# syun88/VLA-from-FastVLM

Measured on AMD Instinct MI355X. Metric: policy steps/sec (img+prompt->action) FastVLM-0.5B bs=64, higher is better.
Workload: dtype bf16; 1 GPU; fastvlm-0.5b select_action: letterbox 336^2->1024^2, FastViT-HD, projector, Qwen2 decoder (text-only, reference-literal: 64-token prompt), last-token pool, action head; batch_per_gpu=64, global_batch=64, seq_len=64, image=336, parallelism=replicas x1 (no collective on the inference path), tower_microbatch=0, stream_overlap=True, llm_precision=split-bf16 (hi+lo) operands, fp32 attention

## Files before the change

### include/fastvla_hip_testops.h

```cpp
#ifndef FASTVLA_HIP_TESTOPS_H
#define FASTVLA_HIP_TESTOPS_H

#include "fastvla_hip.h"

#ifdef __cplusplus
extern "C" {
#endif

enum fv_gemm_epilogue {
  FV_EPI_BIAS = 0,
  FV_EPI_BIAS_GELU = 1,
  FV_EPI_LS_RES = 2,
  FV_EPI_RES_F32 = 3,
  FV_EPI_SWIGLU = 4,
  FV_EPI_F32 = 5,
  FV_EPI_SWIGLU_SPLIT = 7,
  FV_EPI_SWIGLU_F16 = 8,
  FV_EPI_GELU_GRAD = 9,
  FV_EPI_MUL_AUX = 10,
  FV_EPI_F16 = 11,
  FV_EPI_MUL_GELUP = 12
};
int fv_op_gemm(const void* A, int lda, const void* W, int M, int N, int K, const float* bias, const float* scale,
               const void* res, int ldr, void* out, int ldo, int epilogue, fv_stream s);
int fv_op_gemm_f16(const void* A, int lda, const void* W, int M, int N, int K, const float* bias, const void* res, int ldr, void* out,
                   int ldo, int epilogue, void* ws, size_t ws_bytes, fv_stream s);
int fv_op_gemm_lo8(const void* A, int lda, const void* W, const void* W8, int M, int N, int K, const float* bias, const void* res, int ldr, void* out,
                   int ldo, int epilogue, void* ws, size_t ws_bytes, fv_stream s);
int fv_op_lo8_pack(const float* x, void* a_out, int lda, const void* W, void* w8_out, int M, int K, int N, fv_stream s);
int fv_op_gemm_ksplit(const void* A, int lda, const void* W, int M, int N, int K, const float* bias, const void* res, int ldr,
                      void* out, int ldo, int epilogue, fv_stream s);
int fv_op_gemm_tn(const void* A, int lda, const void* W, int ldw, int M, int N, int K, int f16, const float* bias, void* out, int ldo, void* ws,
                  size_t ws_bytes, fv_stream s);
int fv_op_gemm_splitk(const void* A, int lda, const void* W, int M, int N, int K, const float* bias, const void* res, int ldr,
                      void* out, int ldo, int epilogue, int ksplit, void* ws, size_t ws_bytes, fv_stream s);
int fv_op_dwconv(const void* x, const float* w, const float* bias, void* y, int B, int H, int W, int C, int k,
                 int stride, int mult, int gelu, fv_stream s);
int fv_op_stem_conv(const void* pix, const float* w, const float* bias, void* y, int B, int S, int Cout, fv_stream s);
int fv_op_stem_mfma(const void* pix, const void* wp, const float* bias, void* y, int B, int S, int Cout, fv_stream s);
int fv_op_stem_fused(const void* pix, const void* wp, const float* b1, const float* w2, const float* b2, void* y, int B,
                     int S, int Cout, fv_stream s);
int fv_op_stem_fused_images(const void* img, int dtype, int B, int C, int Hin, int Win, float pad_value, int resize_with_padding, const void* wp,
                            const float* b1, const float* w2, const float* b2, void* y, int S, int Cout, fv_stream s);
int fv_op_layernorm_rows(const void* x, const float* w, const float* b, void* y, int rows, int C, float eps,
                         fv_stream s);
int fv_op_attention(const void* q, const void* k, const void* v, int ldq, int ldk, int ldv, void* out, int ldo, int B,
                    int T, int heads, int kv_heads, int D, int causal, const int32_t* lens, float scale, fv_stream s);
int fv_op_rmsnorm(const float* x, const float* w, void* y_bf16, int rows, int H, float eps, fv_stream s);
int fv_op_rope(void* qkv, int ld, int rows, int T, int heads, int kv_heads, int D, float theta, fv_stream s);
int fv_op_attention_bwd(const float* qkv, int ld, const float* dO, float* dqkv, void* out_bf16_scratch, float* stat_scratch, int B, int T,
                        int heads, int kv_heads, int D, const int32_t* lens, float theta, fv_stream s);
int fv_op_rmsnorm_bwd(const float* x, const float* w, const float* dy, const float* dres, float* dx, float* dw, float* scratch, int rows,
                      int H, float eps, fv_stream s);

int fv_op_se_gelu(const void* x, const float* w1, const float* b1, const float* w2, const float* b2, void* y,
                  float* scratch, int B, int P, int C, int R, fv_stream s);

int fv_op_dwconv_mfma(const void* x, const void* ttab, const float* bias, void* y, int B, int H, int W, int C, int k, int gelu,
                      fv_stream s);
int fv_op_dwconv_s2_mfma(const void* x, const void* ttab, const float* bias, void* y, int B, int H, int W, int C, int gelu,
                         fv_stream s);
int fv_op_dwconv_pair(const void* x, const void* t3, const float* b3, const void* t7, const float* b7, void* y1, void* y2, int B,
                      int H, int W, int C, fv_stream s);
int fv_op_convffn(const void* x, const void* w1, const float* b1, const void* w2p, const float* b2, const float* ls,
                  const void* res, void* out, int M, int C, fv_stream s);

int fv_op_convffn32(const void* x, const void* wq, const float* b1, const float* b2, const float* ls, const void* res, void* out,
                    int M, int C, fv_stream s);
int fv_op_convffn32_stash(const void* x, const void* wq, const float* b1, const float* b2, const float* ls, const void* res, void* out,
                          int M, int C, void* stash_y, fv_stream s);
int fv_op_gemm_f16_gelup(const void* A, int lda, const void* W, int M, int N, int K, const void* aux, int ldaux, void* out, int ldo, void* h_out, fv_stream s);
int fv_op_dw_wgrad(const void* x, const void* dy, float* dw, float* db, float* scratch, size_t scratch_floats, int B, int H, int W, int C, int k, int stride, int mult, fv_stream s);
int fv_op_convffn32_split(const void* x, const void* wq, const float* b1, const float* b2, const float* ls, const void* res, void* out,
                          int M, int C, float* part, size_t part_bytes, fv_stream s);

int fv_op_lora_direct_scratch_floats(int R, int rank, int max_cols, size_t* out_floats);
int fv_op_lora_direct(int kind, int part_mask, int rank, int Np, int K, int qd, int kd, const int64_t* a_off, const int64_t* b_off, const void* dY, const void* X,
                      int xkind, int ldx, int lo_off, int R, const float* lora, float* lora_grads, float scale, float* scratch, size_t scratch_floats, fv_stream s);

#ifdef __cplusplus
}
#endif
#endif
```

### vla-from-fastvlm_amd/csrc/engine.hip

```cpp
#include <dlfcn.h>

#include <algorithm>
#include <cmath>
#include <cstdarg>
#include <cstdio>
#include <cstdlib>
#include <cstring>
#include <functional>
#include <map>
#include <string>
#include <vector>

#include "kernels.h"

static thread_local char g_err[768] = "";
static thread_local char* g_err_handle = nullptr;
int fv_fail(int code, const char* fmt, ...) {
  va_list ap;
  va_start(ap, fmt);
  vsnprintf(g_err, sizeof(g_err), fmt, ap);
  va_end(ap);
  if (g_err_handle) memcpy(g_err_handle, g_err, sizeof(g_err));
  return code;
}
// ... 202 lines not shown
    const fv_tensor_desc* t = need(name);
    if (t && count(t) != n) {
      if (rc == FV_OK) rc = fv_fail(FV_ERR_ARG, "tensor '%s' has %zu elements, expected %zu", name.c_str(), count(t), n);
      return nullptr;
    }
    return t;
  }
  bool to_f32(const fv_tensor_desc* t, std::vector<float>& out) {
    const size_t n = count(t), esz = t->dtype == FV_F32 ? 4 : 2;
    const void* src = t->data;
    if (t->device) {
      stage.resize(n * esz);
      if (hipMemcpy(stage.data(), t->data, n * esz, hipMemcpyDeviceToHost) != hipSuccess) {
        if (rc == FV_OK) rc = fv_fail(FV_ERR_HIP, "hipMemcpy (device tensor -> host) failed");
        return false;
      }
      src = stage.data();
    }
    out.resize(n);
    if (t->dtype == FV_F32) memcpy(out.data(), src, n * 4);
    else { const bf16_t* b = static_cast<const bf16_t*>(src); for (size_t i = 0; i < n; ++i) out[i] = host_bf2f(b[i]); }
    return true;
  }
  bool get(const std::string& name, std::vector<float>& out, std::vector<int64_t>* shape = nullptr) {
    const fv_tensor_desc* t = need(name);
    if (!t || !to_f32(t, out)) return false;
    if (shape) shape->assign(t->shape, t->shape + t->ndim);
    return true;
  }
  bool expect(const std::string& name, std::vector<float>& v, size_t n) {
    const fv_tensor_desc* t = need_n(name, n);
    return t && to_f32(t, v);
  }
  void* alloc(size_t bytes) {
    void* p = nullptr;
    if (dev_alloc(h, bytes, &p) != FV_OK) { if (rc == FV_OK) rc = FV_ERR_HIP; return nullptr; }
    return p;
  }
  float* up_f32(const std::vector<float>& v) {
    void* p = alloc(v.size() * 4);
    if (p && hipMemcpy(p, v.data(), v.size() * 4, hipMemcpyHostToDevice) != hipSuccess) { if (rc == FV_OK) rc = fv_fail(FV_ERR_HIP, "hipMemcpy failed"); }
    return static_cast<float*>(p);
  }
  bf16_t* up_bf16(const std::vector<float>& v) {
    std::vector<bf16_t> b(v.size());
    for (size_t i = 0; i < v.size(); ++i) b[i] = host_f2bf(v[i]);
    void* p = alloc(b.size() * 2);
    if (p && hipMemcpy(p, b.data(), b.size() * 2, hipMemcpyHostToDevice) != hipSuccess) { if (rc == FV_OK) rc = fv_fail(FV_ERR_HIP, "hipMemcpy failed"); }
    return static_cast<bf16_t*>(p);
  }
  bool put_rows(const fv_tensor_desc* t, bf16_t* dst, size_t dst_pitch, size_t row_elems, size_t rows, size_t src_pitch) {
    std::vector<bf16_t> tmp;
    const void* src = t->data;
    hipMemcpyKind kind = t->device ? hipMemcpyDeviceToDevice : hipMemcpyHostToDevice;
    if (t->dtype == FV_F32) {
      std::vector<float> v;
      if (!to_f32(t, v)) return false;
      tmp.resize(v.size());
      for (size_t i = 0; i < v.size(); ++i) tmp[i] = host_f2bf(v[i]);
      src = tmp.data();
      kind = hipMemcpyHostToDevice;
    }
    if (hipMemcpy2D(dst, dst_pitch * 2, src, src_pitch * 2, row_elems * 2, rows, kind) != hipSuccess) {
      if (rc == FV_OK) rc = fv_fail(FV_ERR_HIP, "hipMemcpy2D (weight packing) failed");
      return false;
    }
    return true;
  }
  float* vec(const std::string& name, size_t n) { std::vector<float> v; return expect(name, v, n) ? up_f32(v) : nullptr; }
  bf16_t* mat(const std::string& name, size_t n, size_t k) {
    const fv_tensor_desc* t = need_n(name, n * k);
    if (!t) return nullptr;
    bf16_t* p = static_cast<bf16_t*>(alloc(n * k * 2));
    return p && put_rows(t, p, n * k, n * k, 1, n * k) ? p : nullptr;
  }
  float* dw(const std::string& name, int cout, int k, const std::vector<float>* scale = nullptr, int map_w = 0, bf16_t** ttab = nullptr,
            int s2_cin = 0, int s2_map = 0, bf16_t** s2_ttab = nullptr) {
    std::vector<float> v;
    if (!expect(name, v, (size_t)cout * k * k)) return nullptr;
    std::vector<float> o((size_t)cout * k * k);
    for (int c = 0; c < cout; ++c)
      for (int t = 0; t < k * k; ++t) o[(size_t)t * cout + c] = v[(size_t)c * k * k + t] * (scale ? (*scale)[c] : 1.0f);
    if (ttab && fv::dwconv_mfma_supported(map_w, cout, k, 1, 1)) {
      std::vector<float> tt(fv::dwconv_toeplitz_elems(cout, k));
      fv::dwconv_toeplitz_pack(o.data(), tt.data(), cout, k);
      *ttab = up_bf16(tt);
    }
    if (s2_ttab && s2_cin > 0 && cout % s2_cin == 0 && fv::dwconv_s2_mfma_supported(s2_map, s2_map, s2_cin, k, 2, cout / s2_cin)) {
      std::vector<float> tt(fv::dwconv_s2_toeplitz_elems(s2_cin));
      fv::dwconv_s2_toeplitz_pack(o.data(), tt.data(), s2_cin);
      *s2_ttab = up_bf16(tt);
    }
    return up_f32(o);
  }
};

int load_ffn(Loader& L, const std::string& pre, int C, int hidden, float bn_eps, FFN& f, const std::string& ls_name, int map_w) {
  std::vector<float> g, b, m, v;
  if (!L.expect(pre + "conv.bn.weight", g, C) || !L.expect(pre + "conv.bn.bias", b, C) ||
      !L.expect(pre + "conv.bn.running_mean", m, C) || !L.expect(pre + "conv.bn.running_var", v, C))
    return L.rc;
  std::vector<float> sc(C), bias(C);
  for (int c = 0; c < C; ++c) {
    sc[c] = g[c] / std::sqrt(v[c] + bn_eps);
    bias[c] = b[c] - m[c] * sc[c];
  }
  f.dw_w = L.dw(pre + "conv.conv.weight", C, 7, &sc, map_w, &f.dw_t);
  f.dw_b = L.up_f32(bias);
  f.fc1_w = L.mat(pre + "fc1.weight", hidden, C);
  f.fc1_b = L.vec(pre + "fc1.bias", hidden);
  f.fc2_w = L.mat(pre + "fc2.weight", C, hidden);
  if (hidden == 4 * C && fv::convffn_supported(C, 4)) {
    std::vector<float> w2, w2p;
    if (L.expect(pre + "fc2.weight", w2, (size_t)C * hidden)) {
      w2p.resize(w2.size());
      fv::convffn_pack_w2(w2.data(), w2p.data(), C, hidden);
      f.w2p = L.up_bf16(w2p);
      std::vector<float> w1;
      if (fv::convffn32_supported(C, 4) && L.expect(pre + "fc1.weight", w1, (size_t)hidden * C)) {
        std::vector<float> wq((size_t)2 * hidden * C);
        fv::convffn32_pack(w1.data(), w2.data(), wq.data(), C);
        f.w2q = L.up_bf16(wq);
      }
    }
  }
  f.fc2_b = L.vec(pre + "fc2.bias", C);
  f.ls = L.vec(ls_name, C);
  return L.rc;
}

WsPlan plan_ws(const fv_handle* h, int B, int T, int splice) {
  const fv_model_desc& d = h->d;
  WsPlan p{};
  const int mb = (d.tower_microbatch > 0 && d.tower_microbatch < B) ? d.tower_microbatch : B;
  const size_t S = d.image_size;
  size_t act = (S / 2) * (S / 2) * (size_t)d.tower_dims[0];
  size_t hid = 0;
  size_t hw = (S / 4) * (S / 4);
  for (int i = 0; i < d.tower_stages; ++i) {
    const size_t C = d.tower_dims[i];
    act = std::max(act, hw * C);
    hid = std::max(hid, hw * C * d.tower_mlp_ratio);
    if (d.tower_is_attn[i]) hid = std::max(hid, hw * C * 3);
    if (i + 1 < d.tower_stages) {
      hw /= 4;
      act = std::max(act, hw * (size_t)d.tower_dims[i + 1]);
    }
  }
  const size_t P = hw;
  act = std::max(act, P * (size_t)d.tower_out_dim);
  hid = std::max(hid, P * (size_t)d.llm_hidden);
  size_t o = 0;
  auto take = [&](size_t bytes) { size_t r = o; o += align_up(bytes); return r; };
  p.bufA = take(act * mb * 2);
  p.bufB = take(act * mb * 2);
  p.bufH = take(hid * mb * 2);
  p.se = take(((size_t)mb * (2 * d.tower_out_dim + d.tower_se_rd)) * 4);
  p.tower_out = take((size_t)B * P * d.tower_out_dim * 2);
  const size_t rows = (size_t)B * (T + (splice ? P : 0));
  const size_t qkvw = (size_t)(d.llm_heads + 2 * d.llm_kv_heads) * d.llm_head_dim;
  p.x = take(rows * d.llm_hidden * 4);
  p.xn = take(rows * d.llm_hidden * 2);
  p.qkv = take(rows * qkvw * 2);
  p.att = take(rows * (size_t)d.llm_heads * d.llm_head_dim * 2);
  p.act = take(rows * d.llm_inter * 2);
  if (d.llm_precision >= 1) {
    p.xn_lo = take(rows * d.llm_hidden * 2 * 2);
    p.att_lo = take(rows * (size_t)d.llm_heads * d.llm_head_dim * 2 * 2);
    p.act_lo = (d.llm_precision == 1 || d.llm_precision == 3 || d.llm_precision == 5) ? take(rows * d.llm_inter * 2 * 2) : 0;
    p.qkvf = take(rows * qkvw * 4);
    p.guf = 0;
  }
  p.splitk_bytes = rows <= 256 || (rows % 256 != 0 && rows <= 1024) ? (size_t)(rows <= 256 ? 40 : 24) * rows * ((std::max((size_t)d.llm_hidden, qkvw) + 255) / 256 * 256) * 4
                               : rows % 256 == 0 ? (size_t)(rows <= 2048 ? 8 : 4) * rows * ((std::max((size_t)d.llm_hidden, qkvw) + 255) / 256 * 256) * 4 : 0;
  p.splitk = take(p.splitk_bytes);
  p.head_scr = take(fv::head_bwd_scratch_bytes(h->hd, B));
  const int Tseq = T + (splice ? (int)P : 0);
  p.attn_scr_bytes = (d.llm_precision != 0 && Tseq >= fv::FV_ATTN_SPLIT_MIN_T && (d.llm_head_dim == 64 || d.llm_head_dim == 128))
                         ? fv::attention_split_scratch_bytes(B, Tseq, d.llm_kv_heads, d.llm_head_dim) : 0;
  p.attn_scr = take(p.attn_scr_bytes);
  p.total = o;
  return p;
}

int check_ready(fv_handle* h, bool need_ws) {
  if (!h) return fv_fail(FV_ERR_ARG, "null handle");
  if (!h->loaded) return fv_fail(FV_ERR_STATE, "weights not loaded: call fv_load_weights first");
  if (need_ws && !h->ws) return fv_fail(FV_ERR_STATE, "workspace not bound: call fv_bind_workspace first");
  return FV_OK;
}

#define FV_TRY(expr)            \
  do {                          \
    int _rc = (expr);           \
    if (_rc != FV_OK) return _rc; \
  } while (0)

void prof_begin(fv_handle* h, int fam, double flops, double bytes, hipStream_t s, int m = 0, int n = 0, int k = 0, int epi = 0) {
  if (!h->prof.on) return;
  ProfRec r{fam, flops, bytes, m, n, k, epi, h->prof.get(), h->prof.get()};
  if (!r.e0 || !r.e1) return;
  (void)hipEventRecord(r.e0, s);
  h->prof.recs.push_back(r);
}
void prof_end(fv_handle* h, hipStream_t s) {
  if (!h->prof.on || h->prof.recs.empty()) return;
  (void)hipEventRecord(h->prof.recs.back().e1, s);
}
#define FV_P(fam, flops, bytes, call)            \
  do {                                           \
    prof_begin(h, fam, flops, bytes, s);         \
    int _rc = (call);                            \
    prof_end(h, s);                              \
    if (_rc != FV_OK) return _rc;                \
  } while (0)

int gemm_p(fv_handle* h, const fv::GemmArgs& g_in, hipStream_t s) {
  fv::GemmArgs g = g_in;
  if (h->train_depth > 0) g.few_rows = 0;
  const double M = g.M, N = g.N, K = g.K;
  const bool f32o = g.epi == FV_EPI_RES_F32 || g.epi == FV_EPI_F32;
  double bytes = (M * K + N * K) * 2 + M * ((g.epi == FV_EPI_SWIGLU || g.epi == FV_EPI_SWIGLU_F16) ? N / 2 : N) * (f32o ? 4 : 2);
  if (g.epi == FV_EPI_LS_RES) bytes += M * N * 2;
  if (g.epi == FV_EPI_RES_F32) bytes += M * N * 4;
  prof_begin(h, FV_FAM_GEMM, 2.0 * M * N * K, bytes + (g.ksplit ? M * K * 2 : 0), s, g.M, g.N, g.ksplit ? -g.K : g.K, g.epi);
  const int rc = fv::launch_gemm(g, s);
  prof_end(h, s);
  return rc;
}
double dw_flops(int B, int Ho, int Wo, int Cout, int k) { return 2.0 * B * Ho * Wo * Cout * k * k; }

int dw_s1(fv_handle* h, const bf16_t* x, const float* w, const bf16_t* ttab, const float* bias, bf16_t* y, int mb, int H, int C,
          int k, hipStream_t s) {
  if (ttab && !h->no_mfma_dw) return fv::launch_dwconv_mfma(x, ttab, bias, y, mb, H, H, C, k, 0, s);
  return fv::launch_dwconv(x, w, bias, y, mb, H, H, C, k, 1, 1, 0, s);
}

bool ffn_stash_ok(const fv_handle* h, const FFN& f, int M, int C) { return f.w2q && !h->no_ffn32 && fv::convffn32_stash_supported(M, C); }
int fused_ffn(fv_handle* h, const FFN& f, const bf16_t* t, const bf16_t* res, bf16_t* out, int M, int C, int hidden, hipStream_t s, bool ranges = true,
              bf16_t* stash_y = nullptr) {
  if (stash_y) return fv::launch_convffn32(t, f.w2q, f.fc1_b, f.fc2_b, f.ls, res, out, M, C, hidden, s, nullptr, 0, stash_y);
  if (f.w2q && !h->no_ffn32 && (size_t)M * C * 2 < ((size_t)1 << 31))
    return fv::launch_convffn32(t, f.w2q, f.fc1_b, f.fc2_b, f.ls, res, out, M, C, hidden, s, ranges && !h->batch_invariant ? h->ffn_part : nullptr,
                                ranges && !h->batch_invariant && h->ffn_part ? FFN_PART_BYTES : 0);
  return fv::launch_convffn(t, f.fc1_w, f.fc1_b, f.w2p, f.fc2_b, f.ls, res, out, M, C, hidden, s);
}

int run_ffn(fv_handle* h, const FFN& f, bf16_t* x_dw_in, bf16_t* dw_out, bf16_t* hid, bf16_t* res_out, int mb, int H, int W, int C,
            int ratio, hipStream_t s) {
  const int M = mb * H * W;
  FV_P(FV_FAM_DWCONV, dw_flops(mb, H, W, C, 7), 4.0 * M * C, dw_s1(h, x_dw_in, f.dw_w, f.dw_t, f.dw_b, dw_out, mb, H, C, 7, s));
  if (f.w2p && !h->no_fused_ffn) {
    prof_begin(h, FV_FAM_GEMM, 4.0 * M * C * (double)(C * ratio), 6.0 * M * C, s, M, C, C * ratio, 6);
    const int rc = fused_ffn(h, f, dw_out, res_out, res_out, M, C, C * ratio, s);
    prof_end(h, s);
    return rc;
  }
  fv::GemmArgs g1{dw_out, C, f.fc1_w, M, C * ratio, C, f.fc1_b, nullptr, nullptr, 0, hid, C * ratio, FV_EPI_BIAS_GELU};
  FV_TRY(gemm_p(h, g1, s));
  fv::GemmArgs g2{hid, C * ratio, f.fc2_w, M, C, C * ratio, f.fc2_b, f.ls, res_out, C, res_out, C, FV_EPI_LS_RES};
  if (!h->batch_invariant) { g2.splitk_ws = h->ffn_part; g2.splitk_bytes = h->ffn_part ? FFN_PART_BYTES : 0; }
  FV_TRY(gemm_p(h, g2, s));
  return FV_OK;
}

int tap_copy(fv_handle* h, int t, const bf16_t* src, int b0, int mb, size_t per_image, hipStream_t s) {
  if (!h->taps || t >= h->n_taps || !h->taps[t]) return FV_OK;
  bf16_t* dst = static_cast<bf16_t*>(h->taps[t]) + (size_t)b0 * per_image;
  FV_HIP_CHECK(hipMemcpyAsync(dst, src, (size_t)mb * per_image * 2, hipMemcpyDeviceToDevice, s));
  return FV_OK;
}

int unit_tap(fv_handle* h, int u, const bf16_t* src, int b0, int mb, size_t per_image, hipStream_t s) {
  if (!h->utaps || u >= h->n_utaps || !h->utaps[u]) return FV_OK;
  bf16_t* dst = static_cast<bf16_t*>(h->utaps[u]) + (size_t)b0 * per_image;
  FV_HIP_CHECK(hipMemcpyAsync(dst, src, (size_t)mb * per_image * 2, hipMemcpyDeviceToDevice, s));
  return FV_OK;
}

struct UnitInfo { int kind, stage, side, channels; };
std::vector<UnitInfo> tower_units(const fv_model_desc& d) {
  std::vector<UnitInfo> u;
  int H = d.image_size / 4;
  u.push_back({0, 0, H, d.tower_dims[0]});
  for (int i = 0; i < d.tower_stages; ++i) {
    if (d.tower_is_attn[i]) u.push_back({1, i, H, d.tower_dims[i]});
    for (int j = 0; j < d.tower_layers[i]; ++j) u.push_back({2, i, H, d.tower_dims[i]});
    if (i + 1 < d.tower_stages) { H /= 2; u.push_back({3, i, H, d.tower_dims[i + 1]}); }
  }
  return u;
}

int tower_pass(fv_handle* h, const bf16_t* pix, int b0, int mb, bf16_t* tower_out, float* img_tokens, const WsPlan& wp,
               hipStream_t s) {
  const fv_model_desc& d = h->d;
  const Tower& tw = h->tw;
  char* ws = static_cast<char*>(h->ws);
  bf16_t* cur = reinterpret_cast<bf16_t*>(ws + wp.bufA);
  bf16_t* oth = reinterpret_cast<bf16_t*>(ws + wp.bufB);
  bf16_t* hid = reinterpret_cast<bf16_t*>(ws + wp.bufH);
  float* se = reinterpret_cast<float*>(ws + wp.se);
  const int S = d.image_size, C0 = d.tower_dims[0];
  static const bool fuse_stem = !fv_ab_env("FASTVLA_NO_FUSED_STEM");
  if (h->lbsrc) {
    const fv_handle::LbSrc& L = *h->lbsrc;
    if (!(tw.stem0_wp && fv::stem_fused_supported(S, C0))) return fv_fail(FV_ERR_UNSUPPORTED, "fv_vision_forward_images needs the fused stem (first stage width 96)");
    const size_t per = (size_t)L.C * L.Hin * L.Win * (L.dtype == FV_U8 ? 1 : 4);
    FV_P(FV_FAM_STEM, 2.0 * mb * (S / 2) * (S / 2) * 27 * C0 + dw_flops(mb, S / 4, S / 4, C0, 3) + 30.0 * mb * S * S,
         (double)mb * per + (double)mb * (S / 4) * (S / 4) * C0 * 2,
         fv::launch_stem_fused_lb(static_cast<const char*>(L.img) + (size_t)b0 * per, L.dtype, mb, L.C, L.Hin, L.Win, L.pad, L.letterbox, tw.stem0_wp,
                                  tw.stem0_b, tw.stem1_w, tw.stem1_b, oth, S, C0, s));
  } else if (fuse_stem && tw.stem0_wp && fv::stem_fused_supported(S, C0)) {
    FV_P(FV_FAM_STEM, 2.0 * mb * (S / 2) * (S / 2) * 27 * C0 + dw_flops(mb, S / 4, S / 4, C0, 3),
         (double)mb * S * S * 8 + (double)mb * (S / 4) * (S / 4) * C0 * 2,
         fv::launch_stem_fused(pix, tw.stem0_wp, tw.stem0_b, tw.stem1_w, tw.stem1_b, oth, mb, S, C0, s));
  } else {
    FV_P(FV_FAM_STEM, 2.0 * mb * (S / 2) * (S / 2) * 27 * C0, (double)mb * S * S * 8 + (double)mb * (S / 2) * (S / 2) * C0 * 2,
         tw.stem0_wp ? fv::launch_stem_mfma(pix, tw.stem0_wp, tw.stem0_b, cur, mb, S, C0, s)
                     : fv::launch_stem_conv(pix, tw.stem0_w, tw.stem0_b, cur, mb, S, C0, s));
    FV_P(FV_FAM_DWCONV, dw_flops(mb, S / 4, S / 4, C0, 3), (double)mb * (S / 2) * (S / 2) * C0 * 2 * 1.25,
         fv::launch_dwconv(cur, tw.stem1_w, tw.stem1_b, oth, mb, S / 2, S / 2, C0, 3, 2, 1, 1, s));
  }
  int H = S / 4;
  {
    fv::GemmArgs g{oth, C0, tw.stem2_w, mb * H * H, C0, C0, tw.stem2_b, nullptr, nullptr, 0, cur, C0, FV_EPI_BIAS_GELU};
    FV_TRY(gemm_p(h, g, s));
  }
  FV_TRY(tap_copy(h, 0, cur, b0, mb, (size_t)H * H * C0, s));
  int unit = 0;
  FV_TRY(unit_tap(h, unit++, cur, b0, mb, (size_t)H * H * C0, s));
  for (int i = 0; i < d.tower_stages; ++i) {
    const int C = d.tower_dims[i];
    const int M = mb * H * H;
    if (d.tower_is_attn[i]) {
      FV_P(FV_FAM_DWCONV, dw_flops(mb, H, H, C, 7), 4.0 * M * C, dw_s1(h, cur, tw.cpes[i].w, tw.cpes[i].t, tw.cpes[i].b, oth, mb, H, C, 7, s));
      std::swap(cur, oth);
      FV_TRY(unit_tap(h, unit++, cur, b0, mb, (size_t)H * H * C, s));
    }
    for (const Block& b : tw.stages[i]) {
      if (!d.tower_is_attn[i]) {
        static const bool pair_ok = !fv_ab_env("FASTVLA_NO_DW_PAIR");
        if (pair_ok && !h->no_mfma_dw && !h->no_fused_ffn && b.mix_t && b.ffn.dw_t && b.ffn.w2p && fv::dwconv_pair_supported(mb, H, H, C)) {
          FV_P(FV_FAM_DWCONV, dw_flops(mb, H, H, C, 3) + dw_flops(mb, H, H, C, 7), 6.0 * M * C,
               fv::launch_dwconv_pair(cur, b.mix_t, b.mix_b, b.ffn.dw_t, b.ffn.dw_b, oth, hid, mb, H, H, C, s));
          prof_begin(h, FV_FAM_GEMM, 4.0 * M * C * (double)(C * d.tower_mlp_ratio), 6.0 * M * C, s, M, C, C * d.tower_mlp_ratio, 6);
          const int rc = fused_ffn(h, b.ffn, hid, oth, oth, M, C, C * d.tower_mlp_ratio, s);
          prof_end(h, s);
          if (rc != FV_OK) return rc;
        } else {
          FV_P(FV_FAM_DWCONV, dw_flops(mb, H, H, C, 3), 4.0 * M * C, dw_s1(h, cur, b.mix_w, b.mix_t, b.mix_b, oth, mb, H, C, 3, s));
          FV_TRY(run_ffn(h, b.ffn, oth, cur, hid, oth, mb, H, H, C, d.tower_mlp_ratio, s));
        }
        std::swap(cur, oth);
      } else {
        FV_P(FV_FAM_NORM, 8.0 * M * C, 4.0 * M * C, fv::launch_layernorm_rows(cur, b.ln_w, b.ln_b, oth, M, C, d.ln_eps, s));
        fv::GemmArgs gq{oth, C, b.qkv_w, M, 3 * C, C, nullptr, nullptr, nullptr, 0, hid, 3 * C, FV_EPI_BIAS};
        FV_TRY(gemm_p(h, gq, s));
        const int nh = C / d.tower_head_dim;
        FV_P(FV_FAM_ATTN, 4.0 * mb * (double)(H * H) * (H * H) * C, 8.0 * M * C,
             fv::launch_attention(hid, hid + C, hid + 2 * C, 3 * C, 3 * C, 3 * C, oth, C, mb, H * H, nh, nh,
                                  d.tower_head_dim, 0, nullptr, 0, 1.0f / std::sqrt((float)d.tower_head_dim), s));
        fv::GemmArgs gp{oth, C, b.proj_w, M, C, C, b.proj_b, b.ls1, cur, C, cur, C, FV_EPI_LS_RES};
        FV_TRY(gemm_p(h, gp, s));
        FV_TRY(run_ffn(h, b.ffn, cur, oth, hid, cur, mb, H, H, C, d.tower_mlp_ratio, s));
      }
      FV_TRY(unit_tap(h, unit++, cur, b0, mb, (size_t)H * H * C, s));
    }
    FV_TRY(tap_copy(h, 1 + i, cur, b0, mb, (size_t)H * H * C, s));
    if (i + 1 < d.tower_stages) {
      const int C2 = d.tower_dims[i + 1];
      FV_P(FV_FAM_DWCONV, dw_flops(mb, H / 2, H / 2, C2, 7), 2.0 * M * C + 2.0 * (M / 4) * C2,
           (tw.downs[i].lk_t && !h->no_mfma_dw)
               ? fv::launch_dwconv_s2_mfma(cur, tw.downs[i].lk_t, tw.downs[i].lk_b, oth, mb, H, H, C, 1, s)
               : fv::launch_dwconv(cur, tw.downs[i].lk_w, tw.downs[i].lk_b, oth, mb, H, H, C, 7, 2, C2 / C, 1, s));
      H /= 2;
      fv::GemmArgs g{oth, C2, tw.downs[i].pw_w, mb * H * H, C2, C2, tw.downs[i].pw_b, nullptr, nullptr, 0, cur, C2, FV_EPI_BIAS_GELU};
      FV_TRY(gemm_p(h, g, s));
      FV_TRY(unit_tap(h, unit++, cur, b0, mb, (size_t)H * H * C2, s));
    }
  }
  const int CL = d.tower_dims[d.tower_stages - 1], CO = d.tower_out_dim, P = H * H;
  FV_P(FV_FAM_DWCONV, dw_flops(mb, H, H, CO, 3), 2.0 * mb * P * (CL + CO), fv::launch_dwconv(cur, tw.exp_w, tw.exp_b, oth, mb, H, H, CL, 3, 1, CO / CL, 0, s));
  FV_P(FV_FAM_ELT, 20.0 * mb * P * CO, 6.0 * mb * P * CO, fv::launch_se_gelu(oth, tw.se_w1, tw.se_b1, tw.se_w2, tw.se_b2, tower_out, se, mb, P, CO, d.tower_se_rd, s));
  fv::GemmArgs p0{tower_out, CO, tw.pj0_w, mb * P, d.llm_hidden, CO, tw.pj0_b, nullptr, nullptr, 0, hid, d.llm_hidden, FV_EPI_BIAS_GELU};
  if (!h->batch_invariant) { p0.splitk_ws = h->ffn_part; p0.splitk_bytes = h->ffn_part ? FFN_PART_BYTES : 0; }
  FV_TRY(gemm_p(h, p0, s));
  fv::GemmArgs p2{hid, d.llm_hidden, tw.pj2_w, mb * P, d.llm_hidden, d.llm_hidden, tw.pj2_b, nullptr, nullptr, 0, img_tokens, d.llm_hidden, FV_EPI_F32};
  FV_TRY(gemm_p(h, p2, s));
  return FV_OK;
}


enum DecMode { DEC_FULL = 0, DEC_PREFIX = 1, DEC_SUFFIX = 2 };
int decoder_layers_split(fv_handle* h, const WsPlan& wp, int B, int Tq, const int32_t* lens, int len_add, float* kv, int Np, int mode,
                         hipStream_t s) {
  const fv_model_desc& d = h->d;
  char* ws = static_cast<char*>(h->ws);
  float* x = reinterpret_cast<float*>(ws + wp.x);
  bf16_t* xn = reinterpret_cast<bf16_t*>(ws + wp.xn);
  bf16_t* act = reinterpret_cast<bf16_t*>(ws + wp.act);
  const int rows = B * Tq, Hd = d.llm_hidden, D = d.llm_head_dim;
  const int qd = d.llm_heads * D, kd = d.llm_kv_heads * D, qkvw = qd + 2 * kd;
  const int Tt = mode == DEC_SUFFIX ? Np + Tq : Tq;
  const float att_scale = 1.0f / std::sqrt((float)D);
  {
    bf16_t* xs = reinterpret_cast<bf16_t*>(ws + wp.xn_lo);
    bf16_t* as = reinterpret_cast<bf16_t*>(ws + wp.att_lo);
    bf16_t* cs = reinterpret_cast<bf16_t*>(ws + wp.act_lo);
    float* qkvf = reinterpret_cast<float*>(ws + wp.qkvf);
    const int I = d.llm_inter, I2 = 2 * I;
    const size_t kv_layer = (size_t)B * Np * 2 * kd;
    for (size_t li = 0; li < h->dec.layers.size(); ++li) {
      const DecLayer& L = h->dec.layers[li];
      const int lo8 = d.llm_precision == 5, KS = lo8 ? 2 : 1;
      if (li == 0) FV_P(FV_FAM_NORM, 4.0 * rows * Hd, 8.0 * rows * Hd, fv::launch_rmsnorm(x, L.ln1, xs, xs + Hd, 2 * Hd, rows, Hd, d.rms_eps, s, 0, nullptr, lo8));
      fv::GemmArgs q1{xs, 2 * Hd, L.qkv_w, rows, qkvw, Hd, L.qkv_b, nullptr, nullptr, 0, qkvf, qkvw, FV_EPI_F32, KS};
      q1.W8 = L.qkv_w8;
      q1.splitk_ws = wp.splitk_bytes ? reinterpret_cast<float*>(ws + wp.splitk) : nullptr;
      q1.splitk_bytes = wp.splitk_bytes;
      FV_TRY(gemm_p(h, q1, s));
      if (mode == DEC_PREFIX) {
        FV_HIP_CHECK(hipMemcpy2DAsync(kv + li * kv_layer, (size_t)2 * kd * 4, qkvf + qd, (size_t)qkvw * 4, (size_t)2 * kd * 4, (size_t)rows,
                                      hipMemcpyDeviceToDevice, s));
        if (li + 1 == h->dec.layers.size()) break;
      }
      FV_P(FV_FAM_ATTN, 2.0 * B * (double)Tq * Tt * qd + 3.0 * rows * (qd + kd), 4.0 * rows * (qkvw + qd),
           fv::launch_attention_f32(qkvf, qkvw, as, as + qd, 2 * qd, B, Tt, d.llm_heads, d.llm_kv_heads, D, lens, len_add, att_scale, s, h->rope,
                                    mode == DEC_SUFFIX ? kv + li * kv_layer : nullptr, 2 * kd, mode == DEC_SUFFIX ? Np : 0, nullptr, lo8,
                                    wp.attn_scr_bytes && mode != DEC_SUFFIX ? ws + wp.attn_scr : nullptr));
      fv::GemmArgs o1{as, 2 * qd, L.o_w, rows, Hd, qd, nullptr, nullptr, x, Hd, x, Hd, FV_EPI_RES_F32, KS};
      o1.W8 = L.o_w8;
      o1.splitk_ws = q1.splitk_ws;
      o1.splitk_bytes = wp.splitk_bytes;
      const bool ln2_fused = d.llm_precision == 1 || d.llm_precision == 5;
      if (ln2_fused) { o1.norm_w = L.ln2; o1.norm_y = xs; o1.norm_ylo = xs + Hd; o1.norm_ld = 2 * Hd; o1.norm_eps = d.rms_eps; }
      FV_TRY(gemm_p(h, o1, s));
      fv::GemmArgs d1{cs, I2, L.down_w, rows, Hd, I, nullptr, nullptr, x, Hd, x, Hd, FV_EPI_RES_F32, KS};
      d1.W8 = L.down_w8;
      if (d.llm_precision == 2) {
        FV_P(FV_FAM_NORM, 4.0 * rows * Hd, 6.0 * rows * Hd, fv::launch_rmsnorm(x, L.ln2, xn, nullptr, Hd, rows, Hd, d.rms_eps, s, 1, h->f16_flags));
        fv::GemmArgs g1{xn, Hd, L.gu_w, rows, I2, Hd, nullptr, nullptr, nullptr, 0, act, I, FV_EPI_SWIGLU_F16, 0};
        g1.f16 = 1; g1.sat = h->f16_flags;
        FV_TRY(gemm_p(h, g1, s));
        d1 = fv::GemmArgs{act, I, L.down_w, rows, Hd, I, nullptr, nullptr, x, Hd, x, Hd, FV_EPI_RES_F32, 0};
        d1.f16 = 1;
      } else if (d.llm_precision == 3) {
        FV_P(FV_FAM_NORM, 4.0 * rows * Hd, 6.0 * rows * Hd, fv::launch_rmsnorm(x, L.ln2, xn, nullptr, Hd, rows, Hd, d.rms_eps, s, 1, h->f16_flags));
        fv::GemmArgs g1{xn, Hd, L.gu_w, rows, I2, Hd, nullptr, nullptr, nullptr, 0, cs, I2, FV_EPI_SWIGLU_SPLIT, 0};
        g1.f16 = 1;
        FV_TRY(gemm_p(h, g1, s));
      } else if (d.llm_precision == 4) {
        FV_P(FV_FAM_NORM, 4.0 * rows * Hd, 8.0 * rows * Hd, fv::launch_rmsnorm(x, L.ln2, xs, xs + Hd, 2 * Hd, rows, Hd, d.rms_eps, s));
        fv::GemmArgs g1{xs, 2 * Hd, L.gu_w, rows, I2, Hd, nullptr, nullptr, nullptr, 0, act, I, FV_EPI_SWIGLU_F16, 1};
        g1.sat = h->f16_flags;
        FV_TRY(gemm_p(h, g1, s));
        d1 = fv::GemmArgs{act, I, L.down_w, rows, Hd, I, nullptr, nullptr, x, Hd, x, Hd, FV_EPI_RES_F32, 0};
        d1.f16 = 1;
      } else {
        fv::GemmArgs g1{xs, 2 * Hd, L.gu_w, rows, I2, Hd, nullptr, nullptr, nullptr, 0, cs, I2, FV_EPI_SWIGLU_SPLIT, KS};
        g1.W8 = L.gu_w8;
        g1.splitk_ws = q1.splitk_ws; g1.splitk_bytes = wp.splitk_bytes;
        FV_TRY(gemm_p(h, g1, s));
      }
      d1.splitk_ws = wp.splitk_bytes ? reinterpret_cast<float*>(ws + wp.splitk) : nullptr;
      d1.splitk_bytes = wp.splitk_bytes;
      if (li + 1 < h->dec.layers.size()) {
        d1.norm_w = h->dec.layers[li + 1].ln1; d1.norm_y = xs; d1.norm_ylo = xs + Hd; d1.norm_ld = 2 * Hd; d1.norm_eps = d.rms_eps;
      }
      FV_TRY(gemm_p(h, d1, s));
    }
  }
  return FV_OK;
}

}

extern "C" {

const char* fv_version(void) { return "fastvla_hip 0.1 (gfx950)"; }
const char* fv_last_error(fv_handle* h) { return h ? h->err : g_err; }

int fv_create(const fv_model_desc* desc, int device, fv_handle** out) {
  if (!desc || !out) return fv_fail(FV_ERR_ARG, "fv_create: null argument");
  const fv_model_desc& d = *desc;
  if (d.tower_stages < 1 || d.tower_stages > FV_MAX_STAGES) return fv_fail(FV_ERR_ARG, "tower_stages out of range");
  if (d.image_size <= 0 || d.image_size % (4 << (d.tower_stages - 1)))
    return fv_fail(FV_ERR_ARG, "image_size %d must be a positive multiple of %d", d.image_size, 4 << (d.tower_stages - 1));
  for (int i = 0; i < d.tower_stages; ++i) {
    if (d.tower_dims[i] % 8 || d.tower_dims[i] <= 0 || d.tower_layers[i] < 0) return fv_fail(FV_ERR_ARG, "tower dims must be positive multiples of 8");
    if (d.tower_is_attn[i] && d.tower_dims[i] % d.tower_head_dim) return fv_fail(FV_ERR_ARG, "attention stage dim %% head_dim != 0");
    if (i > 0 && d.tower_dims[i] != 2 * d.tower_dims[i - 1] && d.tower_dims[i] != d.tower_dims[i - 1]) return fv_fail(FV_ERR_UNSUPPORTED, "stage dims must double or stay (grouped 7x7 multiplier 1 or 2)");
  }
  if (d.tower_head_dim != 32 && d.tower_head_dim != 64 && d.tower_head_dim != 128) return fv_fail(FV_ERR_UNSUPPORTED, "tower head_dim must be 32/64/128");
  if (d.llm_head_dim != 32 && d.llm_head_dim != 64 && d.llm_head_dim != 128) return fv_fail(FV_ERR_UNSUPPORTED, "llm head_dim must be 32/64/128");
  if (d.llm_hidden % 8 || d.llm_inter % 8 || d.llm_heads % d.llm_kv_heads) return fv_fail(FV_ERR_ARG, "llm dims must be multiples of 8 and heads %% kv_heads == 0");
  if (d.tower_out_dim != 2 * d.tower_dims[d.tower_stages - 1] && d.tower_out_dim != d.tower_dims[d.tower_stages - 1]) return fv_fail(FV_ERR_UNSUPPORTED, "tower_out_dim must be 1x or 2x the last stage dim");
  if (d.llm_precision < 0 || d.llm_precision > 5)
    return fv_fail(FV_ERR_ARG, "llm_precision must be 0 (bf16), 1 (split-bf16), 2 (split-bf16 qkv/o + fp16 gate/up/down) or 5 (bf16 hi + fp8 lo)");
#ifndef FASTVLA_AB_SWITCHES
  if (d.llm_precision == 3 || d.llm_precision == 4)
    return fv_fail(FV_ERR_UNSUPPORTED, "llm_precision = %d is a measurement mode of the tools build (make AB=1); the product ships 0, 1, 2 and 5", d.llm_precision);
#endif
  if (d.llm_precision == 5 && (d.llm_hidden % 128 || d.llm_inter % 128 || (d.llm_heads * d.llm_head_dim) % 128))
    return fv_fail(FV_ERR_UNSUPPORTED, "llm_precision = 5 (hi + lo8 operands) needs hidden, inter and heads * head_dim to be multiples of 128");
  if (d.state_dim <= 0 || d.action_dim <= 0 || d.hidden_dim <= 0 || d.fusion_dim <= 0) return fv_fail(FV_ERR_ARG, "head dims must be positive");
  FV_HIP_CHECK(hipSetDevice(device));
  fv_handle* h = new fv_handle();
  h->d = d;
  h->device = device;
  h->hd = fv::HeadDims{d.llm_hidden, d.state_dim, d.action_dim, d.hidden_dim, d.fusion_dim};
  if (const char* e = fv_ab_env("FASTVLA_NO_FUSED_FFN")) h->no_fused_ffn = e[0] == '1';
  if (const char* e = fv_ab_env("FASTVLA_NO_MFMA_DW")) h->no_mfma_dw = e[0] == '1';
  if (const char* e = fv_ab_env("FASTVLA_NO_FFN32")) h->no_ffn32 = e[0] == '1';
  const int P = (d.image_size >> (d.tower_stages + 1)) * (d.image_size >> (d.tower_stages + 1));
  h->rope_rows = d.max_text_tokens + P + 8;
  std::vector<float> cs((size_t)h->rope_rows * d.llm_head_dim);
  fv::rope_table_host(cs.data(), h->rope_rows, d.llm_head_dim, d.rope_theta);
  void* p = nullptr;
  int rc = dev_alloc(h, cs.size() * 4, &p);
  if (rc == FV_OK && hipMemcpy(p, cs.data(), cs.size() * 4, hipMemcpyHostToDevice) != hipSuccess) rc = fv_fail(FV_ERR_HIP, "rope table upload failed");
  h->rope = static_cast<float2*>(p);
  if (rc == FV_OK) { rc = dev_alloc(h, fv::adamw_scratch_bytes(), &p); h->norm_scratch = static_cast<float*>(p); }
  if (rc == FV_OK) {
    rc = dev_alloc(h, 256, &p);
    h->f16_flags = static_cast<unsigned*>(p);
    if (rc == FV_OK && hipMemset(p, 0, 256) != hipSuccess) rc = fv_fail(FV_ERR_HIP, "fp16 flag words: memset failed");
    h->lb_vmax = h->f16_flags + 32;
  }
  if (rc == FV_OK) { rc = dev_alloc(h, FFN_PART_BYTES, &p); h->ffn_part = static_cast<float*>(p); }
  if (rc != FV_OK) { fv_destroy(h); return rc; }
  *out = h;
  return FV_OK;
}

void fv_destroy(fv_handle* h) {
  if (!h) return;
  (void)hipSetDevice(h->device);
  for (void* p : h->allocs) (void)hipFree(p);
  for (hipEvent_t e : h->prof.pool) (void)hipEventDestroy(e);
  delete h;
}

static int load_impl(fv_handle* h, Loader& L);

int fv_load_weights(fv_handle* h, const fv_tensor_desc* tensors, int n) {
  HandleScope _hs(h);
  if (!h || !tensors || n <= 0) return fv_fail(FV_ERR_ARG, "fv_load_weights: null argument");
  if (h->loaded) return fv_fail(FV_ERR_STATE, "weights already loaded");
  Loader L{h};
  for (int i = 0; i < n; ++i) {
    if (!tensors[i].name || !tensors[i].data || tensors[i].ndim < 1 || tensors[i].ndim > 4) return fv_fail(FV_ERR_ARG, "tensor %d: bad descriptor", i);
    L.idx[tensors[i].name] = &tensors[i];
  }
  return load_impl(h, L);
}

int fv_load_weights_cb(fv_handle* h, fv_tensor_provider provider, void* user) {
  HandleScope _hs(h);
  if (!h || !provider) return fv_fail(FV_ERR_ARG, "fv_load_weights_cb: null argument");
  if (h->loaded) return fv_fail(FV_ERR_STATE, "weights already loaded");
  Loader L{h};
  L.prov = provider;
  L.user = user;
  return load_impl(h, L);
}

static int load_impl(fv_handle* h, Loader& L) {
  FV_HIP_CHECK(hipSetDevice(h->device));
  const fv_model_desc& d = h->d;
  Tower& tw = h->tw;
  const std::string vt = VT;
  const int C0 = d.tower_dims[0];
  {
    std::vector<float> v;
    if (L.expect(vt + "patch_embed.0.reparam_conv.weight", v, (size_t)C0 * 27)) {
      std::vector<float> o((size_t)27 * C0);
      for (int co = 0; co < C0; ++co)
        for (int ci = 0; ci < 3; ++ci)
          for (int t = 0; t < 9; ++t) o[(size_t)(t * 3 + ci) * C0 + co] = v[((size_t)co * 3 + ci) * 9 + t];
      tw.stem0_w = L.up_f32(o);
      if (C0 % 16 == 0 && C0 <= 128) {
        std::vector<float> wp((size_t)C0 * 64);
        fv::stem_mfma_pack(o.data(), wp.data(), C0);
        tw.stem0_wp = L.up_bf16(wp);
      }
    }
    tw.stem0_b = L.vec(vt + "patch_embed.0.reparam_conv.bias", C0);
    tw.stem1_w = L.dw(vt + "patch_embed.1.reparam_conv.weight", C0, 3);
    tw.stem1_b = L.vec(vt + "patch_embed.1.reparam_conv.bias", C0);
    tw.stem2_w = L.mat(vt + "patch_embed.2.reparam_conv.weight", C0, C0);
    tw.stem2_b = L.vec(vt + "patch_embed.2.reparam_conv.bias", C0);
  }
  tw.stages.resize(d.tower_stages);
  tw.downs.resize(d.tower_stages);
  tw.cpes.resize(d.tower_stages);
  int idx = 0;
  for (int i = 0; i < d.tower_stages && L.rc == FV_OK; ++i) {
    const int C = d.tower_dims[i];
    const int map_w = d.image_size >> (2 + i);
    if (d.tower_is_attn[i]) {
      const std::string pre = vt + "network." + std::to_string(idx++) + ".";
      tw.cpes[i].w = L.dw(pre + "reparam_conv.weight", C, 7, nullptr, map_w, &tw.cpes[i].t);
      tw.cpes[i].b = L.vec(pre + "reparam_conv.bias", C);
    }
    const int sidx = idx++;
    tw.stages[i].resize(d.tower_layers[i]);
    for (int j = 0; j < d.tower_layers[i] && L.rc == FV_OK; ++j) {
      const std::string pre = vt + "network." + std::to_string(sidx) + "." + std::to_string(j) + ".";
      Block& b = tw.stages[i][j];
      if (d.tower_is_attn[i]) {
        b.ln_w = L.vec(pre + "norm.weight", C);
        b.ln_b = L.vec(pre + "norm.bias", C);
        b.qkv_w = L.mat(pre + "token_mixer.qkv.weight", 3 * (size_t)C, C);
        b.proj_w = L.mat(pre + "token_mixer.proj.weight", C, C);
        b.proj_b = L.vec(pre + "token_mixer.proj.bias", C);
        b.ls1 = L.vec(pre + "layer_scale_1", C);
        load_ffn(L, pre + "convffn.", C, C * d.tower_mlp_ratio, d.bn_eps, b.ffn, pre + "layer_scale_2", map_w);
      } else {
        b.mix_w = L.dw(pre + "token_mixer.reparam_conv.weight", C, 3, nullptr, map_w, &b.mix_t);
        b.mix_b = L.vec(pre + "token_mixer.reparam_conv.bias", C);
        load_ffn(L, pre + "convffn.", C, C * d.tower_mlp_ratio, d.bn_eps, b.ffn, pre + "layer_scale", map_w);
      }
    }
    if (i + 1 < d.tower_stages) {
      const int C2 = d.tower_dims[i + 1];
      const std::string pre = vt + "network." + std::to_string(idx++) + ".proj.";
      tw.downs[i].lk_w = L.dw(pre + "0.lkb_reparam.weight", C2, 7, nullptr, 0, nullptr, C, map_w, &tw.downs[i].lk_t);
// ... 525 lines not shown
```

### vla-from-fastvlm_amd/csrc/kernels.h

```cpp
#pragma once
#include <hip/hip_runtime.h>
#include <stdint.h>

#include "../../include/fastvla_hip.h"
#include "../../include/fastvla_hip_testops.h"
#include "common.h"

namespace fv {

struct GemmArgs {
  const bf16_t* A; int lda;
  const bf16_t* W;
  int M, N, K;
  const float* bias;
  const float* scale;
  const void* res; int ldr;
  void* out; int ldo;
  int epi;
  int ksplit = 0;
  int f16 = 0;
  float* splitk_ws = nullptr;
  size_t splitk_bytes = 0;
  int lo_off = 0;
  int no_tail = 0;
  int few_rows = 1;
  const float* norm_w = nullptr; bf16_t* norm_y = nullptr; bf16_t* norm_ylo = nullptr; int norm_ld = 0; float norm_eps = 0.f;
  const void* W8 = nullptr;
  unsigned* sat = nullptr;
  void* stash = nullptr;
  int stash_f16 = 0;
  int tn = 0, ldw = 0;
};
int launch_gemm(const GemmArgs& a, hipStream_t s);

bool convffn_supported(int C, int ratio);
void convffn_pack_w2(const float* w2, float* out, int C, int hidden);
int launch_convffn(const bf16_t* x, const bf16_t* w1, const float* b1, const bf16_t* w2p, const float* b2, const float* ls,
                   const bf16_t* res, bf16_t* out, int M, int C, int hidden, hipStream_t s);

bool convffn32_supported(int C, int ratio);
void convffn32_pack(const float* w1, const float* w2, float* out, int C);
int launch_convffn32(const bf16_t* x, const bf16_t* wq, const float* b1, const float* b2, const float* ls,
                     const bf16_t* res, bf16_t* out, int M, int C, int hidden, hipStream_t s, float* part = nullptr, size_t part_bytes = 0,
                     bf16_t* stash_y = nullptr);
bool convffn32_stash_supported(int M, int C);

int launch_letterbox(const void* img, int dtype, int B, int C, int Hin, int Win, int S, float pad_value, int letterbox,
                     bf16_t* pix, hipStream_t s);
int launch_letterbox_norm(const void* img, int dtype, int B, int C, int Hin, int Win, int S, float pad_value, int letterbox, const float* mean3,
                          const float* std3, int range_heuristic, unsigned* vmax_scratch, bf16_t* pix, hipStream_t s);
int launch_stem_conv(const bf16_t* pix, const float* w, const float* bias, bf16_t* y, int B, int S, int Cout,
                     hipStream_t s);
void stem_mfma_pack(const float* w27, float* out, int Cout);
int launch_stem_mfma(const bf16_t* pix, const bf16_t* wp, const float* bias, bf16_t* y, int B, int S, int Cout, hipStream_t s);
bool stem_fused_supported(int S, int C0);
int launch_stem_fused(const bf16_t* pix, const bf16_t* wp, const float* b1, const float* w2, const float* b2, bf16_t* y, int B,
                      int S, int C0, hipStream_t s);
int launch_stem_fused_lb(const void* img, int dtype, int B, int C, int Hin, int Win, float pad_value, int letterbox, const bf16_t* wp,
                         const float* b1, const float* w2, const float* b2, bf16_t* y, int S, int C0, hipStream_t s);
int launch_dwconv(const bf16_t* x, const float* w, const float* bias, bf16_t* y, int B, int H, int W, int C, int k,
                  int stride, int mult, int gelu, hipStream_t s);
bool dwconv_mfma_supported(int W, int C, int k, int stride, int mult);
size_t dwconv_toeplitz_elems(int C, int k);
void dwconv_toeplitz_pack(const float* w_tapmajor, float* out, int C, int k);
size_t dwconv_s2_toeplitz_elems(int C);
void dwconv_s2_toeplitz_pack(const float* w_tapmajor, float* out, int C);
bool dwconv_s2_mfma_supported(int H, int W, int C, int k, int stride, int mult);
int launch_dwconv_s2_mfma(const bf16_t* x, const bf16_t* ttab, const float* bias, bf16_t* y, int B, int H, int W, int C, int gelu,
                          hipStream_t s);
bool dwconv_pair_supported(int B, int H, int W, int C);
int launch_dwconv_pair(const bf16_t* x, const bf16_t* t3, const float* b3, const bf16_t* t7, const float* b7, bf16_t* y1, bf16_t* y2,
                       int B, int H, int W, int C, hipStream_t s);
int launch_dwconv_mfma(const bf16_t* x, const bf16_t* ttab, const float* bias, bf16_t* y, int B, int H, int W, int C, int k,
                       int gelu, hipStream_t s);
int launch_layernorm_rows(const bf16_t* x, const float* w, const float* b, bf16_t* y, int rows, int C, float eps,
                          hipStream_t s);
int launch_se_gelu(const bf16_t* x, const float* w1, const float* b1, const float* w2, const float* b2, bf16_t* y,
                   float* scratch, int B, int P, int C, int R, hipStream_t s);
int launch_attention(const bf16_t* q, const bf16_t* k, const bf16_t* v, int ldq, int ldk, int ldv, bf16_t* out,
                     int ldo, int B, int T, int heads, int kv_heads, int D, int causal, const int32_t* lens,
                     int len_add, float scale, hipStream_t s);

int launch_embed_gather(const int32_t* ids, const bf16_t* table, const float* img_tokens, float* x, int B, int T,
                        int Ni, int H, int vocab, hipStream_t s);
int launch_rmsnorm(const float* x, const float* w, bf16_t* y, bf16_t* y_lo, int ldy, int rows, int H, float eps, hipStream_t s,
                   int f16 = 0, unsigned* sat = nullptr,
                   int lo8 = 0);
int launch_bf16_to_f16(bf16_t* p, size_t n, float scale, hipStream_t s, unsigned* maxbits = nullptr);
int launch_bf16_to_w8(const bf16_t* w, void* w8, size_t rows, int K, hipStream_t s, unsigned* maxbits = nullptr);
int launch_rope_f32(float* qkv, const float2* table, int ld, int rows, int T, int heads, int kv_heads, int D, hipStream_t s);
int launch_attention_f32(float* qkv, int ld, bf16_t* out_hi, bf16_t* out_lo, int ldo, int B, int T, int heads,
                         int kv_heads, int D, const int32_t* lens, int len_add, float scale, hipStream_t s, const float2* rope = nullptr,
                         const float* pre = nullptr, int ldp = 0, int Np = 0,
                         float* lse = nullptr,
                         int lo8 = 0,
                         void* split_scratch = nullptr);
constexpr int FV_ATTN_SPLIT_MIN_T = 128;
int launch_rope(bf16_t* qkv, const float2* table, int ld, int rows, int T, int heads, int kv_heads, int D,
                hipStream_t s);
void rope_table_host(float* cos_sin_pairs, int T, int D, float theta);
int launch_pool_norm(const float* x, const int32_t* lens, const float* w, float* pooled, int B, int Ttot, int Ni,
                     int H, float eps, int mode, hipStream_t s);

constexpr int RMS_BWD_RPW = 4;
constexpr int COLSUM_CHUNKS = 64;
int launch_split_rows(const float* in, int ldi, bf16_t* out, int ldo, int lo_off, long R, int C, hipStream_t s);
int launch_lo8_rows(const float* in, int ldi, bf16_t* out, int ldo, long R, int C, hipStream_t s);
int launch_bf16_to_f32(const bf16_t* in, float* out, size_t n, hipStream_t s);
int launch_transpose_to_bf16(const void* in, int in_bf16, int ldi, bf16_t* out, int ldo, int lo_off, int R, int Rp, int C, hipStream_t s);
int launch_transpose_to_f16(const void* in, int in_kind, int ldi, int lo_in, bf16_t* out, int ldo, int R, int Rp, int C, unsigned* sat, hipStream_t s,
                            bf16_t* rows_out = nullptr, int ldro = 0);
int launch_rows_to_f16(const void* in, int in_kind, int ldi, int lo_in, bf16_t* out, int ldo, long R, int C, unsigned* sat, hipStream_t s,
                       long Rp = 0);
int launch_swiglu_bwd(float* gu, const float* dact, long rows, int I, hipStream_t s, bf16_t* out_split = nullptr);
int launch_swiglu_bwd_rows(const void* gu, int gu_f16, const float* dact, long rows, long Rp, int I, bf16_t* dgu_rows, bf16_t* act_rows, unsigned* sat, hipStream_t s);
int launch_swiglu_bwd_f16(const void* gu, int gu_f16, const float* dact, int rows, int Rp, int I, bf16_t* out_rows, bf16_t* outT, unsigned* sat, hipStream_t s,
                          bf16_t* actT = nullptr);
int launch_gelu_fwd(const float* pre, bf16_t* out, int ldo, int lo_off, long R, int C, hipStream_t s);
int launch_gelu_bwd(float* dh, const float* pre, size_t n, hipStream_t s);
size_t rmsnorm_bwd_scratch_floats(long rows, int H);
int launch_colsum(const float* in, int ld, long R, int C, float* out, float* scratch, hipStream_t s);
int launch_rmsnorm_bwd(const float* x, const float* w, const float* dy, const float* dres, float* dx, float* dw, float* scratch, long rows, int H,
                       float eps, hipStream_t s);
int launch_pool_rows(float* stream, float* compact, const int32_t* lens, int B, int Tt, int Ni, int H, int scatter, hipStream_t s);
int launch_image_rows(const float* stream, float* compact, int B, int Tt, int Ni, int H, hipStream_t s);
int launch_embed_bwd(const int32_t* ids, const int32_t* lens, const float* dx, float* dE, int B, int T, int Ni, int H, int vocab, hipStream_t s);
int launch_attention_bwd(const float* qkv, int ld, const bf16_t* o_hi, const bf16_t* o_lo, int ldo, const float* dO, int lddo, const float* lse,
                         float* delta, float* dqkv, int B, int T, int heads, int kv_heads, int D, const int32_t* lens, int len_add, float scale,
                         const float2* rope, hipStream_t s, float* part = nullptr,
                         void* split_scratch = nullptr);

struct CommitDesc {
  long long src_off;
  void* dst;
  void* dstT16;
  void* dstTb;
  int rows, cols;
  int is_mat;
  int tile0;
  void* dst16;
  float scale16;
};
int launch_commit(const CommitDesc* desc_dev, int ndesc, int ntiles, const float* flat, int f16_transposes, unsigned* sat, hipStream_t s);

constexpr int LORA_STRIP_ROWS = 128;
struct LoraMat {
  long long w_off;
  long long a_off, b_off;
  int out, in;
  int row0, blk;
  int strip0;
  long long part_off;
  long long m_off, n_off;
};
struct LoraCommitDesc {
  CommitDesc c;
  int kind;
  int qd, kd;
  int mat[3];
  int band0;
};
int launch_lora_project(const LoraMat* mats_dev, int m0, int m1, int strip_begin, int nstrips, int max_in, const float* grads_full, const float* lora,
                        float* lora_grads, float* scratch, int rank, float scale, hipStream_t s, const float* master = nullptr, const float* norms = nullptr);
int launch_lora_commit(const LoraCommitDesc* desc_dev, int ndesc, int ntiles, const LoraMat* mats_dev, const float* flat, const float* lora, int rank, float scale,
                       int f16_transposes, unsigned* sat, hipStream_t s, const float* norms = nullptr);
int launch_lora_merge(const LoraCommitDesc* desc_dev, int ndesc, int ntiles, const LoraMat* mats_dev, float* flat, const float* lora, int rank, float scale,
                      hipStream_t s, const float* norms = nullptr);
int launch_lora_norms(const LoraCommitDesc* desc_dev, int ndesc, int nbands, const LoraMat* mats_dev, const float* flat, const float* lora, int rank, float scale,
                      float* norms, float* mag, hipStream_t s);

struct LoraDirectPack {
  int kind;
  int nm, r, NCp;
  int Np, K;
  int qd, kd;
  int slot_of_part[3];
  long long a_off[3], b_off[3];
};
size_t lora_direct_scratch_floats(long R, int rank, int max_cols);
int launch_lora_direct(const LoraDirectPack& pk, const bf16_t* dY, const bf16_t* X, int xkind, int ldx, int lo_off, int R, const float* lora, float* lgrads,
                       float scale, float* scratch, size_t scratch_floats, hipStream_t s);

size_t dw_bwd_scratch_floats(int B, int Ho, int Wo, int Co, int k);
int launch_dw_dgrad(const bf16_t* dy, const float* w, const bf16_t* res, bf16_t* dx, int B, int Hi, int Wi, int Ci, int k, int stride, int mult, unsigned* sat,
                    hipStream_t s, int round_w = 0);
bool dw_dgrad_mfma_supported(int H, int W, int C, int k);
int launch_dw_dgrad_mfma(const bf16_t* dy, const bf16_t* ttab16, const bf16_t* res, bf16_t* dx, int B, int H, int W, int C, int k, hipStream_t s);
int launch_dw_wgrad(const bf16_t* x, const bf16_t* dy, float* dw, float* db, float* scratch, int B, int Hi, int Wi, int Ci, int k, int stride, int mult,
                    hipStream_t s);
constexpr int TOWER_COLSUM_CHUNKS = 512;
int launch_colsum16(const bf16_t* in, int ld, long R, int C, float* out, float* scratch, hipStream_t s);
int launch_mul16(const bf16_t* a, const bf16_t* b, bf16_t* out, size_t n, unsigned* sat, hipStream_t s);
int launch_gelu_grad_mul(const bf16_t* dh, const bf16_t* pre, bf16_t* out, size_t n, unsigned* sat, hipStream_t s);
int launch_f16_to_f32(const bf16_t* in, float* out, size_t n, float scale, hipStream_t s);
int launch_scale_to_f16(const float* in, bf16_t* out, size_t n, float scale, unsigned* sat, hipStream_t s);
int launch_rescale_to_f16(const float* in, bf16_t* out, size_t n, float target, unsigned* bits, float* sc, unsigned* sat, hipStream_t s);
int launch_unscale_dev(float* p, size_t n, const float* sc, hipStream_t s);
int launch_ones_col(bf16_t* out, int ld, int C, long R, hipStream_t s);
int launch_ls_grads(const float* dWraw, const float* dbraw, const bf16_t* W, const float* bias, const float* ls, float* dW, float* db, float* dls, int C, int Kd,
                    hipStream_t s);
size_t ln_bwd_scratch_floats(long rows, int C);
int launch_ln_bwd(const bf16_t* x, const bf16_t* dy, const float* w, const bf16_t* res, bf16_t* dx, float* dw, float* db, float* scratch, long rows, int C,
                  float eps, unsigned* sat, hipStream_t s);
int launch_tower_attn_bwd(const bf16_t* qkv, int ld, const bf16_t* dO, int lddo, bf16_t* dqkv, int ldd, float* stats, int B, int T, int heads, float scale,
                          hipStream_t s);
int launch_se_bwd(const bf16_t* e, const bf16_t* dout, const float* se, const float* w1, const float* w2, bf16_t* de, float* dW1, float* db1, float* dW2,
                  float* db2, float* tmp, int B, int P, int C, int R, unsigned* sat, hipStream_t s);
size_t stem0_wgrad_scratch_floats(int B, int S, int C0);
int launch_stem0_wgrad(const bf16_t* pix, const float* w, const float* bias, const bf16_t* dh0, float* dw, float* db, float* scratch, int B, int S, int C0,
                       hipStream_t s, int round_w = 0);
int launch_stem_im2col16(const bf16_t* pix, bf16_t* P, int B, int S, hipStream_t s);
struct TowerCommitOp {
  long long src_off, src2_off, n;
  void* dst;
  const int* idx; const float* coef;
  int kind, rows, cols, blk0;
};
int launch_tower_commit(const TowerCommitOp* ops_dev, int nops, int nblocks, const float* flat, unsigned* sat, hipStream_t s);

size_t attention_split_scratch_bytes(int B, int T, int kv_heads, int D);
int launch_attention_split_fwd(const float* qkv, int ld, bf16_t* out_hi, bf16_t* out_lo, int ldo, int B, int T, int heads, int kv_heads, int D,
                               const int32_t* lens, int len_add, float scale, const float2* rope, float* lse, void* scratch, hipStream_t s);
int launch_attention_split_bwd(const float* qkv, int ld, const bf16_t* o_hi, const bf16_t* o_lo, int ldo, const float* dO, int lddo, const float* lse,
                               float* delta, float* dqkv, int B, int T, int heads, int kv_heads, int D, const int32_t* lens, int len_add, float scale,
                               const float2* rope, hipStream_t s, float* part, long pstride, void* scratch);

struct HeadDims { int feat, ds, da, hid, fus; };
struct HeadOffsets { int64_t o[13]; };
HeadOffsets head_offsets(const HeadDims& d);
size_t head_saved_bytes(const HeadDims& d, int B);
struct HeadIoNorm { const float *state_mean, *state_istd, *action_mean, *action_std; };
int launch_head_forward(const HeadDims& d, const float* P, const float* pooled, const float* states, int B,
                        int training, float drop_p, uint64_t seed, uint64_t offset, float* actions, float* saved,
                        hipStream_t s, const HeadIoNorm* io = nullptr);
int launch_head_backward(const HeadDims& d, const float* P, const float* grad_actions, const float* actions,
                         const float* targets, int B, float drop_p, const float* saved, float* loss, float* G,
                         float* scratch, hipStream_t s, float* d_pooled = nullptr, float loss_scale = 1.0f);
size_t head_bwd_scratch_bytes(const HeadDims& d, int B);
size_t adamw_scratch_bytes();
int launch_axpy(float* y, const float* x, int64_t n, const float* scale_dev, hipStream_t s);
int launch_adamw_clip(float* p, const float* g, float* m, float* v, int64_t n, const fv_adamw_hparams& hp,
                      int64_t step, float* norm_scratch, float* grad_norm_out, hipStream_t s);

}
```

### vla-from-fastvlm_amd/csrc/ops_api.hip

```cpp
#include <cmath>
#include <vector>

#include "kernels.h"

extern "C" {

int fv_op_gemm(const void* A, int lda, const void* W, int M, int N, int K, const float* bias, const float* scale,
               const void* res, int ldr, void* out, int ldo, int epilogue, fv_stream s) {
  fv::GemmArgs g{static_cast<const bf16_t*>(A), lda, static_cast<const bf16_t*>(W), M, N, K, bias, scale, res, ldr, out, ldo, epilogue};
  return fv::launch_gemm(g, static_cast<hipStream_t>(s));
}
int fv_op_gemm_ksplit(const void* A, int lda, const void* W, int M, int N, int K, const float* bias, const void* res, int ldr,
                      void* out, int ldo, int epilogue, fv_stream s) {
  fv::GemmArgs g{static_cast<const bf16_t*>(A), lda, static_cast<const bf16_t*>(W), M, N, K, bias, nullptr, res, ldr, out, ldo, epilogue};
  g.ksplit = true;
  return fv::launch_gemm(g, static_cast<hipStream_t>(s));
}
int fv_op_gemm_splitk(const void* A, int lda, const void* W, int M, int N, int K, const float* bias, const void* res, int ldr,
                      void* out, int ldo, int epilogue, int ksplit, void* ws, size_t ws_bytes, fv_stream s) {
  fv::GemmArgs g{static_cast<const bf16_t*>(A), lda, static_cast<const bf16_t*>(W), M, N, K, bias, nullptr, res, ldr, out, ldo, epilogue};
  g.ksplit = ksplit != 0;
  g.splitk_ws = static_cast<float*>(ws);
  g.splitk_bytes = ws_bytes;
  return fv::launch_gemm(g, static_cast<hipStream_t>(s));
}

int fv_op_gemm_tn(const void* A, int lda, const void* W, int ldw, int M, int N, int K, int f16, const float* bias, void* out, int ldo, void* ws,
                  size_t ws_bytes, fv_stream s) {
  fv::GemmArgs g{static_cast<const bf16_t*>(A), lda, static_cast<const bf16_t*>(W), M, N, K, bias, nullptr, nullptr, 0, out, ldo, FV_EPI_F32};
  g.tn = 1; g.ldw = ldw; g.f16 = f16 != 0;
  g.splitk_ws = static_cast<float*>(ws);
  g.splitk_bytes = ws_bytes;
  return fv::launch_gemm(g, static_cast<hipStream_t>(s));
}

int fv_op_gemm_lo8(const void* A, int lda, const void* W, const void* W8, int M, int N, int K, const float* bias, const void* res, int ldr, void* out,
                   int ldo, int epilogue, void* ws, size_t ws_bytes, fv_stream s) {
  fv::GemmArgs g{static_cast<const bf16_t*>(A), lda, static_cast<const bf16_t*>(W), M, N, K, bias, nullptr, res, ldr, out, ldo, epilogue};
  g.ksplit = 2;
  g.W8 = W8;
  g.splitk_ws = static_cast<float*>(ws);
  g.splitk_bytes = ws_bytes;
  return fv::launch_gemm(g, static_cast<hipStream_t>(s));
}
int fv_op_lo8_pack(const float* x, void* a_out, int lda, const void* W, void* w8_out, int M, int K, int N, fv_stream s) {
  int rc = FV_OK;
  if (x && a_out) {
    rc = fv::launch_split_rows(x, K, static_cast<bf16_t*>(a_out), lda, 0, M, K, static_cast<hipStream_t>(s));
    if (rc == FV_OK) rc = fv::launch_lo8_rows(x, K, static_cast<bf16_t*>(a_out), lda, M, K, static_cast<hipStream_t>(s));
  }
  if (rc == FV_OK && W && w8_out) rc = fv::launch_bf16_to_w8(static_cast<const bf16_t*>(W), w8_out, (size_t)N, K, static_cast<hipStream_t>(s));
  return rc;
}

int fv_op_gemm_f16(const void* A, int lda, const void* W, int M, int N, int K, const float* bias, const void* res, int ldr, void* out,
                   int ldo, int epilogue, void* ws, size_t ws_bytes, fv_stream s) {
  fv::GemmArgs g{static_cast<const bf16_t*>(A), lda, static_cast<const bf16_t*>(W), M, N, K, bias, nullptr, res, ldr, out, ldo, epilogue};
  g.f16 = 1;
  g.splitk_ws = static_cast<float*>(ws);
  g.splitk_bytes = ws_bytes;
  return fv::launch_gemm(g, static_cast<hipStream_t>(s));
}

int fv_op_dwconv(const void* x, const float* w, const float* bias, void* y, int B, int H, int W, int C, int k,
                 int stride, int mult, int gelu, fv_stream s) {
  return fv::launch_dwconv(static_cast<const bf16_t*>(x), w, bias, static_cast<bf16_t*>(y), B, H, W, C, k, stride, mult, gelu, static_cast<hipStream_t>(s));
}

int fv_op_stem_conv(const void* pix, const float* w, const float* bias, void* y, int B, int S, int Cout, fv_stream s) {
  return fv::launch_stem_conv(static_cast<const bf16_t*>(pix), w, bias, static_cast<bf16_t*>(y), B, S, Cout, static_cast<hipStream_t>(s));
}

int fv_op_stem_mfma(const void* pix, const void* wp, const float* bias, void* y, int B, int S, int Cout, fv_stream s) {
  return fv::launch_stem_mfma(static_cast<const bf16_t*>(pix), static_cast<const bf16_t*>(wp), bias, static_cast<bf16_t*>(y), B, S, Cout, static_cast<hipStream_t>(s));
}
int fv_op_stem_fused(const void* pix, const void* wp, const float* b1, const float* w2, const float* b2, void* y, int B, int S, int Cout,
                     fv_stream s) {
  return fv::launch_stem_fused(static_cast<const bf16_t*>(pix), static_cast<const bf16_t*>(wp), b1, w2, b2, static_cast<bf16_t*>(y), B, S, Cout,
                               static_cast<hipStream_t>(s));
}

int fv_op_stem_fused_images(const void* img, int dtype, int B, int C, int Hin, int Win, float pad_value, int resize_with_padding, const void* wp,
                            const float* b1, const float* w2, const float* b2, void* y, int S, int Cout, fv_stream s) {
  return fv::launch_stem_fused_lb(img, dtype, B, C, Hin, Win, pad_value, resize_with_padding, static_cast<const bf16_t*>(wp), b1, w2, b2,
                                  static_cast<bf16_t*>(y), S, Cout, static_cast<hipStream_t>(s));
}

int fv_op_layernorm_rows(const void* x, const float* w, const float* b, void* y, int rows, int C, float eps, fv_stream s) {
  return fv::launch_layernorm_rows(static_cast<const bf16_t*>(x), w, b, static_cast<bf16_t*>(y), rows, C, eps, static_cast<hipStream_t>(s));
}

int fv_op_attention(const void* q, const void* k, const void* v, int ldq, int ldk, int ldv, void* out, int ldo, int B,
                    int T, int heads, int kv_heads, int D, int causal, const int32_t* lens, float scale, fv_stream s) {
  return fv::launch_attention(static_cast<const bf16_t*>(q), static_cast<const bf16_t*>(k), static_cast<const bf16_t*>(v), ldq, ldk,
                              ldv, static_cast<bf16_t*>(out), ldo, B, T, heads, kv_heads, D, causal, lens, 0, scale, static_cast<hipStream_t>(s));
}

int fv_op_rmsnorm(const float* x, const float* w, void* y_bf16, int rows, int H, float eps, fv_stream s) {
  return fv::launch_rmsnorm(x, w, static_cast<bf16_t*>(y_bf16), nullptr, H, rows, H, eps, static_cast<hipStream_t>(s));
}

int fv_op_rope(void* qkv, int ld, int rows, int T, int heads, int kv_heads, int D, float theta, fv_stream s) {
  if (T <= 0 || D <= 0 || D % 16) return fv_fail(FV_ERR_ARG, "rope: bad T/D");
  std::vector<float> cs((size_t)T * D);
  fv::rope_table_host(cs.data(), T, D, theta);
  float2* tab = nullptr;
  FV_HIP_CHECK(hipMalloc(reinterpret_cast<void**>(&tab), cs.size() * 4));
  hipError_t e = hipMemcpy(tab, cs.data(), cs.size() * 4, hipMemcpyHostToDevice);
  int rc = e == hipSuccess ? fv::launch_rope(static_cast<bf16_t*>(qkv), tab, ld, rows, T, heads, kv_heads, D, static_cast<hipStream_t>(s))
                           : fv_hip_fail(e, "hipMemcpy(rope table)");
  (void)hipStreamSynchronize(static_cast<hipStream_t>(s));
  (void)hipFree(tab);
  return rc;
}

int fv_op_attention_bwd(const float* qkv, int ld, const float* dO, float* dqkv, void* out_bf16_scratch, float* stat_scratch, int B, int T,
                        int heads, int kv_heads, int D, const int32_t* lens, float theta, fv_stream st) {
  if (!qkv || !dO || !dqkv || !out_bf16_scratch || !stat_scratch) return fv_fail(FV_ERR_ARG, "attention_bwd: null pointer");
  if (T <= 0 || (D != 64 && D != 128)) return fv_fail(FV_ERR_UNSUPPORTED, "attention_bwd: head_dim must be 64 or 128");
  hipStream_t s = static_cast<hipStream_t>(st);
  std::vector<float> cs((size_t)T * D);
  fv::rope_table_host(cs.data(), T, D, theta);
  float2* tab = nullptr;
  FV_HIP_CHECK(hipMalloc(reinterpret_cast<void**>(&tab), cs.size() * 4));
  hipError_t e = hipMemcpy(tab, cs.data(), cs.size() * 4, hipMemcpyHostToDevice);
  int rc = e == hipSuccess ? FV_OK : fv_hip_fail(e, "hipMemcpy(rope table)");
  const int qd = heads * D;
  bf16_t* o = static_cast<bf16_t*>(out_bf16_scratch);
  float* lse = stat_scratch;
  float* delta = stat_scratch + (size_t)B * heads * T;
  const float scale = 1.0f / sqrtf((float)D);
  void* scr = nullptr;
  if (rc == FV_OK) { e = hipMalloc(&scr, fv::attention_split_scratch_bytes(B, T, kv_heads, D)); if (e != hipSuccess) rc = fv_hip_fail(e, "hipMalloc(attention scratch)"); }
  if (rc == FV_OK) rc = fv::launch_attention_f32(const_cast<float*>(qkv), ld, o, o + qd, 2 * qd, B, T, heads, kv_heads, D, lens, 0, scale, s, tab, nullptr, 0, 0, lse, 0, scr);
  if (rc == FV_OK) rc = fv::launch_attention_bwd(qkv, ld, o, o + qd, 2 * qd, dO, qd, lse, delta, dqkv, B, T, heads, kv_heads, D, lens, 0, scale, tab, s, nullptr, scr);
  (void)hipStreamSynchronize(s);
  (void)hipFree(tab);
  if (scr) (void)hipFree(scr);
  return rc;
}

int fv_op_rmsnorm_bwd(const float* x, const float* w, const float* dy, const float* dres, float* dx, float* dw, float* scratch, int rows,
                      int H, float eps, fv_stream s) {
  return fv::launch_rmsnorm_bwd(x, w, dy, dres, dx, dw, scratch, rows, H, eps, static_cast<hipStream_t>(s));
}

int fv_op_se_gelu(const void* x, const float* w1, const float* b1, const float* w2, const float* b2, void* y,
                  float* scratch, int B, int P, int C, int R, fv_stream s) {
  return fv::launch_se_gelu(static_cast<const bf16_t*>(x), w1, b1, w2, b2, static_cast<bf16_t*>(y), scratch, B, P, C, R, static_cast<hipStream_t>(s));
}

int fv_op_dwconv_mfma(const void* x, const void* ttab, const float* bias, void* y, int B, int H, int W, int C, int k, int gelu,
                      fv_stream s) {
  return fv::launch_dwconv_mfma(static_cast<const bf16_t*>(x), static_cast<const bf16_t*>(ttab), bias, static_cast<bf16_t*>(y), B, H, W, C, k,
                                gelu, static_cast<hipStream_t>(s));
}
int fv_op_dwconv_s2_mfma(const void* x, const void* ttab, const float* bias, void* y, int B, int H, int W, int C, int gelu, fv_stream s) {
  return fv::launch_dwconv_s2_mfma(static_cast<const bf16_t*>(x), static_cast<const bf16_t*>(ttab), bias, static_cast<bf16_t*>(y), B, H, W, C,
                                   gelu, static_cast<hipStream_t>(s));
}
int fv_op_dwconv_pair(const void* x, const void* t3, const float* b3, const void* t7, const float* b7, void* y1, void* y2, int B,
                      int H, int W, int C, fv_stream s) {
  return fv::launch_dwconv_pair(static_cast<const bf16_t*>(x), static_cast<const bf16_t*>(t3), b3, static_cast<const bf16_t*>(t7), b7,
                                static_cast<bf16_t*>(y1), static_cast<bf16_t*>(y2), B, H, W, C, static_cast<hipStream_t>(s));
}

int fv_op_convffn(const void* x, const void* w1, const float* b1, const void* w2p, const float* b2, const float* ls,
                  const void* res, void* out, int M, int C, fv_stream s) {
  return fv::launch_convffn(static_cast<const bf16_t*>(x), static_cast<const bf16_t*>(w1), b1, static_cast<const bf16_t*>(w2p), b2, ls,
                            static_cast<const bf16_t*>(res), static_cast<bf16_t*>(out), M, C, 4 * C, static_cast<hipStream_t>(s));
}

int fv_op_convffn32(const void* x, const void* wq, const float* b1, const float* b2, const float* ls, const void* res, void* out,
                    int M, int C, fv_stream s) {
  return fv::launch_convffn32(static_cast<const bf16_t*>(x), static_cast<const bf16_t*>(wq), b1, b2, ls, static_cast<const bf16_t*>(res),
                              static_cast<bf16_t*>(out), M, C, 4 * C, static_cast<hipStream_t>(s));
}

int fv_op_convffn32_stash(const void* x, const void* wq, const float* b1, const float* b2, const float* ls, const void* res, void* out,
                          int M, int C, void* stash_y, fv_stream s) {
  if (!stash_y) return fv_fail(FV_ERR_ARG, "fv_op_convffn32_stash: null stash");
  return fv::launch_convffn32(static_cast<const bf16_t*>(x), static_cast<const bf16_t*>(wq), b1, b2, ls, static_cast<const bf16_t*>(res),
                              static_cast<bf16_t*>(out), M, C, 4 * C, static_cast<hipStream_t>(s), nullptr, 0, static_cast<bf16_t*>(stash_y));
}
int fv_op_gemm_f16_gelup(const void* A, int lda, const void* W, int M, int N, int K, const void* aux, int ldaux, void* out, int ldo, void* h_out, fv_stream s) {
  fv::GemmArgs g{static_cast<const bf16_t*>(A), lda, static_cast<const bf16_t*>(W), M, N, K, nullptr, nullptr, aux, ldaux, out, ldo, FV_EPI_MUL_GELUP};
  g.f16 = 1;
  g.stash = h_out;
  return fv::launch_gemm(g, static_cast<hipStream_t>(s));
}

int fv_op_dw_wgrad(const void* x, const void* dy, float* dw, float* db, float* scratch, size_t scratch_floats, int B, int H, int W, int C, int k, int stride, int mult, fv_stream s) {
  const int pad = k / 2, Ho = (H + 2 * pad - k) / stride + 1, Wo = (W + 2 * pad - k) / stride + 1;
  if (scratch_floats < fv::dw_bwd_scratch_floats(B, Ho, Wo, C * mult, k)) return fv_fail(FV_ERR_ARG, "fv_op_dw_wgrad: scratch too small (%zu floats needed)", fv::dw_bwd_scratch_floats(B, Ho, Wo, C * mult, k));
  return fv::launch_dw_wgrad(static_cast<const bf16_t*>(x), static_cast<const bf16_t*>(dy), dw, db, scratch, B, H, W, C, k, stride, mult, static_cast<hipStream_t>(s));
}

int fv_op_convffn32_split(const void* x, const void* wq, const float* b1, const float* b2, const float* ls, const void* res, void* out,
                          int M, int C, float* part, size_t part_bytes, fv_stream s) {
  return fv::launch_convffn32(static_cast<const bf16_t*>(x), static_cast<const bf16_t*>(wq), b1, b2, ls, static_cast<const bf16_t*>(res),
                              static_cast<bf16_t*>(out), M, C, 4 * C, static_cast<hipStream_t>(s), part, part_bytes);
}

int fv_op_lora_direct_scratch_floats(int R, int rank, int max_cols, size_t* out_floats) {
  if (!out_floats || R <= 0 || rank < 1 || rank > 64 || max_cols <= 0) return fv_fail(FV_ERR_ARG, "fv_op_lora_direct_scratch_floats: bad arguments");
  *out_floats = fv::lora_direct_scratch_floats(R, rank, max_cols);
  return FV_OK;
}
int fv_op_lora_direct(int kind, int part_mask, int rank, int Np, int K, int qd, int kd, const int64_t* a_off, const int64_t* b_off, const void* dY, const void* X,
                      int xkind, int ldx, int lo_off, int R, const float* lora, float* lora_grads, float scale, float* scratch, size_t scratch_floats, fv_stream s) {
  if (!a_off || !b_off) return fv_fail(FV_ERR_ARG, "fv_op_lora_direct: null offsets");
  const int nparts = kind == 1 ? 3 : (kind == 2 ? 2 : 1);
  if (kind < 0 || kind > 2 || part_mask <= 0 || part_mask >= (1 << nparts)) return fv_fail(FV_ERR_ARG, "fv_op_lora_direct: kind %d, part mask 0x%x", kind, part_mask);
  fv::LoraDirectPack pk{};
  pk.kind = kind; pk.r = rank; pk.Np = Np; pk.K = K; pk.qd = qd; pk.kd = kd;
  for (int p = 0; p < 3; ++p) {
    pk.slot_of_part[p] = -1;
    if (p < nparts && (part_mask >> p & 1)) { pk.slot_of_part[p] = pk.nm; pk.a_off[pk.nm] = a_off[p]; pk.b_off[pk.nm] = b_off[p]; ++pk.nm; }
  }
  pk.NCp = (pk.nm * rank + 31) / 32 * 32;
  return fv::launch_lora_direct(pk, static_cast<const bf16_t*>(dY), static_cast<const bf16_t*>(X), xkind, ldx, lo_off, R, lora, lora_grads, scale, scratch,
                                scratch_floats, static_cast<hipStream_t>(s));
}

}
```

### vla-from-fastvlm_amd/csrc/tower_kernels.hip

```cpp
#include "kernels.h"
#include <cstdlib>

namespace fv {
namespace {

struct LbParams {
  const void* img; bf16_t* pix; int dtype, B, C, Hin, Win, S, rh, rw, pt, pl; float pad, sh, sw;
};

__device__ __forceinline__ float lb_fetch(const LbParams& p, size_t plane, int y, int x) {
  const size_t i = plane + (size_t)y * p.Win + x;
  return p.dtype == FV_U8 ? (float)static_cast<const uint8_t*>(p.img)[i] : static_cast<const float*>(p.img)[i];
}

__device__ __forceinline__ float lb_lerp(float a, float b, float w) {
#pragma clang fp contract(off)
  return (1.0f - w) * a + w * b;
}
__device__ __forceinline__ float lb_src(int d, float scale) {
#pragma clang fp contract(off)
  return fmaxf(((float)d + 0.5f) * scale - 0.5f, 0.0f);
}
__device__ __forceinline__ float lb_frac(float s, int i) {
#pragma clang fp contract(off)
  return s - (float)i;
}

__device__ __forceinline__ uint2 lb_pixel(const LbParams& p, int b, int y, int x) {
  float v[3] = {p.pad, p.pad, p.pad};
  const int dx = x - p.pl, dy = y - p.pt;
  if (dx >= 0 && dx < p.rw && dy >= 0 && dy < p.rh) {
    const float sx = lb_src(dx, p.sw);
    const int x0 = min((int)sx, p.Win - 1), x1 = min(x0 + 1, p.Win - 1);
    const float wx = lb_frac(sx, x0);
    const float sy = lb_src(dy, p.sh);
    const int y0 = min((int)sy, p.Hin - 1), y1 = min(y0 + 1, p.Hin - 1);
    const float wy = lb_frac(sy, y0);
    const int nc = p.C >= 3 ? 3 : 1;
    for (int c = 0; c < nc; ++c) {
      const size_t plane = ((size_t)b * p.C + c) * p.Hin * p.Win;
      const float t0 = lb_lerp(lb_fetch(p, plane, y0, x0), lb_fetch(p, plane, y0, x1), wx);
      const float t1 = lb_lerp(lb_fetch(p, plane, y1, x0), lb_fetch(p, plane, y1, x1), wx);
      v[c] = lb_lerp(t0, t1, wy);
    }
    if (nc == 1) v[1] = v[2] = v[0];
  }
  uint2 o;
  o.x = pack_bf2(v[0], v[1]);
  o.y = pack_bf2(v[2], 0.0f);
  return o;
}

constexpr int LB_R = 4;
struct LbNorm { float mean[3], std[3]; unsigned* vmax; int heuristic; };
__device__ __forceinline__ unsigned lb_ord(float f) { const unsigned u = __float_as_uint(f); return (u & 0x80000000u) ? ~u : (u | 0x80000000u); }
__device__ __forceinline__ float lb_unord(unsigned k) { return __uint_as_float((k & 0x80000000u) ? (k & 0x7fffffffu) : ~k); }
template <int MODE>
__global__ __launch_bounds__(256) void letterbox_kernel(LbParams p, LbNorm nrm) {
  bool by255 = false;
  if constexpr (MODE == 2) by255 = nrm.heuristic && lb_unord(*nrm.vmax) > 1.5f;
  float vmax = -INFINITY;
  const int x = blockIdx.x * 256 + threadIdx.x, yb = blockIdx.y * LB_R, b = blockIdx.z;
  if (MODE != 1 && x >= p.S) return;
  const int dx = x - p.pl;
  const bool xin = dx >= 0 && dx < p.rw;
  const float sx = lb_src(dx, p.sw);
  const int x0 = min((int)sx, p.Win - 1), x1 = min(x0 + 1, p.Win - 1);
  const float wx = lb_frac(sx, x0);
  const int nc = p.C >= 3 ? 3 : 1;
  float t0[3] = {0.f, 0.f, 0.f}, t1[3] = {0.f, 0.f, 0.f};
  int have = -1;
#pragma unroll
  for (int r = 0; r < LB_R; ++r) {
    const int y = yb + r;
    if (y >= p.S || x >= p.S) break;
    float v[3] = {p.pad, p.pad, p.pad};
    const int dy = y - p.pt;
    if (xin && dy >= 0 && dy < p.rh) {
      const float sy = lb_src(dy, p.sh);
      const int y0 = min((int)sy, p.Hin - 1), y1 = min(y0 + 1, p.Hin - 1);
      const float wy = lb_frac(sy, y0);
      if (y0 != have) {
        have = y0;
        for (int c = 0; c < nc; ++c) {
          const size_t plane = ((size_t)b * p.C + c) * p.Hin * p.Win;
          const float p00 = lb_fetch(p, plane, y0, x0), p01 = lb_fetch(p, plane, y0, x1);
          const float p10 = lb_fetch(p, plane, y1, x0), p11 = lb_fetch(p, plane, y1, x1);
          t0[c] = lb_lerp(p00, p01, wx);
          t1[c] = lb_lerp(p10, p11, wx);
        }
      }
      for (int c = 0; c < nc; ++c) v[c] = lb_lerp(t0[c], t1[c], wy);
      if (nc == 1) v[1] = v[2] = v[0];
    }
    if constexpr (MODE == 1) { vmax = fmaxf(vmax, fmaxf(v[0], fmaxf(v[1], v[2]))); continue; }
    if constexpr (MODE == 2) {
#pragma unroll
      for (int c = 0; c < 3; ++c) {
        float t = v[c];
        if (by255) t = __fdiv_rn(t, 255.0f);
        v[c] = __fdiv_rn(__fsub_rn(t, nrm.mean[c]), nrm.std[c]);
      }
    }
    uint2 o;
    o.x = pack_bf2(v[0], v[1]);
    o.y = pack_bf2(v[2], 0.0f);
    *reinterpret_cast<uint2*>(p.pix + (((size_t)b * p.S + y) * p.S + x) * 4) = o;
  }
  if constexpr (MODE == 1) {
#pragma unroll
    for (int off = 32; off > 0; off >>= 1) vmax = fmaxf(vmax, __shfl_xor(vmax, off, 64));
    if ((threadIdx.x & 63) == 0 && vmax > -INFINITY) atomicMax(nrm.vmax, lb_ord(vmax));
  }
}

__global__ __launch_bounds__(256) void stem_conv_kernel(const bf16_t* __restrict__ pix, const float* __restrict__ w,
                                                         const float* __restrict__ bias, bf16_t* __restrict__ y, int B,
                                                         int S, int Cout) {
  extern __shared__ __attribute__((aligned(16))) float sw[];
  for (int i = threadIdx.x; i < 27 * Cout; i += 256) sw[i] = w[i];
  __syncthreads();
  const int So = S >> 1, G = Cout >> 3, WQ = (So + 3) >> 2;
  const int per_block = 256 / G;
  const int g = threadIdx.x % G, ql = threadIdx.x / G;
  if (ql >= per_block) return;
  long q = (long)blockIdx.x * per_block + ql;
  const int xq = (int)(q % WQ); q /= WQ;
  const int oy = (int)(q % So);
  const int b = (int)(q / So);
  if (b >= B) return;
  const int ox0 = xq * 4, co0 = g * 8;
  float acc[4][8];
#pragma unroll
  for (int r = 0; r < 4; ++r)
#pragma unroll
    for (int e = 0; e < 8; ++e) acc[r][e] = bias[co0 + e];
#pragma unroll
  for (int ky = 0; ky < 3; ++ky) {
    const int iy = oy * 2 - 1 + ky;
    if (iy < 0 || iy >= S) continue;
    float xin[9][3];
#pragma unroll
    for (int c = 0; c < 9; ++c) {
      const int ix = ox0 * 2 - 1 + c;
      if (ix >= 0 && ix < S) {
        const uint2 u = *reinterpret_cast<const uint2*>(pix + (((size_t)b * S + iy) * S + ix) * 4);
        xin[c][0] = bf_lo(u.x); xin[c][1] = bf_hi(u.x); xin[c][2] = bf_lo(u.y);
      } else {
        xin[c][0] = xin[c][1] = xin[c][2] = 0.0f;
      }
    }
#pragma unroll
    for (int kx = 0; kx < 3; ++kx)
#pragma unroll
      for (int ci = 0; ci < 3; ++ci) {
        const float* wp = sw + ((ky * 3 + kx) * 3 + ci) * Cout + co0;
        const float4 w0 = *reinterpret_cast<const float4*>(wp), w1 = *reinterpret_cast<const float4*>(wp + 4);
        const float wv[8] = {w0.x, w0.y, w0.z, w0.w, w1.x, w1.y, w1.z, w1.w};
#pragma unroll
        for (int r = 0; r < 4; ++r)
#pragma unroll
          for (int e = 0; e < 8; ++e) acc[r][e] += xin[2 * r + kx][ci] * wv[e];
      }
  }
#pragma unroll
  for (int r = 0; r < 4; ++r) {
    if (ox0 + r >= So) break;
#pragma unroll
    for (int e = 0; e < 8; ++e) acc[r][e] = gelu_f(acc[r][e]);
    *reinterpret_cast<uint4*>(y + (((size_t)b * So + oy) * So + ox0 + r) * Cout + co0) = pack8(acc[r]);
  }
}

template <int TPW>
__global__ __launch_bounds__(256) void stem_mfma_kernel(const bf16_t* __restrict__ pix, const bf16_t* __restrict__ wp,
                                                         const float* __restrict__ bias, bf16_t* __restrict__ y, int B,
                                                         int S, int Cout, long ntiles) {
  const int lane = threadIdx.x & 63, fr = lane & 15, fg = lane >> 4;
  const int So = S >> 1, tiles_per_row = (So + 15) >> 4;
  const int NTn = Cout >> 4;
  bf16x8 wf[8][2];
#pragma unroll
  for (int nt = 0; nt < 8; ++nt)
#pragma unroll
    for (int ks = 0; ks < 2; ++ks)
      wf[nt][ks] = nt < NTn ? __builtin_bit_cast(bf16x8, *reinterpret_cast<const uint4*>(wp + ((size_t)(nt * 16 + fr) * 64 + ks * 32 + fg * 8)))
                            : __builtin_bit_cast(bf16x8, make_uint4(0, 0, 0, 0));
  const long wave = (long)blockIdx.x * 4 + (threadIdx.x >> 6);
  for (int t = 0; t < TPW; ++t) {
    const long tile = wave * TPW + t;
    if (tile >= ntiles) break;
    const int tx = (int)(tile % tiles_per_row);
    const int oy = (int)((tile / tiles_per_row) % So);
    const long b = tile / ((long)tiles_per_row * So);
    const int ox = tx * 16 + fr;
    bf16x8 xf[2];
#pragma unroll
    for (int ks = 0; ks < 2; ++ks) {
      const int ky = 2 * ks + (fg >> 1), pp = fg & 1;
      const int iy = 2 * oy - 1 + ky, ix = 2 * ox - 1 + 2 * pp;
      uint2 lo = make_uint2(0, 0), hi = make_uint2(0, 0);
      if (ky < 3 && iy >= 0 && iy < S && ox < So) {
        const bf16_t* rp = pix + (((size_t)b * S + iy) * S) * 4;
        if (ix >= 0 && ix < S) lo = *reinterpret_cast<const uint2*>(rp + (size_t)ix * 4);
        if (ix + 1 >= 0 && ix + 1 < S) hi = *reinterpret_cast<const uint2*>(rp + (size_t)(ix + 1) * 4);
      }
      xf[ks] = __builtin_bit_cast(bf16x8, make_uint4(lo.x, lo.y, hi.x, hi.y));
    }
#pragma unroll
    for (int nt = 0; nt < 8; ++nt) {
      if (nt >= NTn) break;
      f32x4 acc = f32x4{0.f, 0.f, 0.f, 0.f};
      acc = __builtin_amdgcn_mfma_f32_16x16x32_bf16(wf[nt][0], xf[0], acc, 0, 0, 0);
      acc = __builtin_amdgcn_mfma_f32_16x16x32_bf16(wf[nt][1], xf[1], acc, 0, 0, 0);
      if (ox < So) {
        const float4 bv = *reinterpret_cast<const float4*>(bias + nt * 16 + fg * 4);
        uint2 o;
        o.x = pack_bf2(gelu_f(acc[0] + bv.x), gelu_f(acc[1] + bv.y));
        o.y = pack_bf2(gelu_f(acc[2] + bv.z), gelu_f(acc[3] + bv.w));
        *reinterpret_cast<uint2*>(y + (((size_t)b * So + oy) * So + ox) * Cout + nt * 16 + fg * 4) = o;
      }
    }
  }
}

template <int K, int S, int MULT>
__global__ __launch_bounds__(256) void dwconv_kernel(const bf16_t* __restrict__ x, const float* __restrict__ w,
                                                      const float* __restrict__ bias, bf16_t* __restrict__ y, int B,
                                                      int H, int W, int C, int Ho, int Wo, int gelu, int GS,
                                                      int nslices, long nquads) {
  constexpr int R = 4, NCOL = (R - 1) * S + K, CI = 8 / MULT, PAD = K / 2;
  __shared__ __attribute__((aligned(16))) float sw[K * K * 16 * 8];
  const int Cout = C * MULT, WQ = (Wo + R - 1) / R;
  const int slice = blockIdx.x % nslices;
  const long qblock = blockIdx.x / nslices;
  const int sc = GS * 8;
  for (int i = threadIdx.x; i < K * K * sc; i += 256) sw[i] = w[(size_t)(i / sc) * Cout + slice * sc + (i % sc)];
  __syncthreads();
  const int qpb = 256 / GS;
  const int g = threadIdx.x % GS, ql = threadIdx.x / GS;
  long q = qblock * qpb + ql;
  if (ql >= qpb || q >= nquads) return;
  const int xq = (int)(q % WQ); q /= WQ;
  const int oy = (int)(q % Ho);
  const long b = q / Ho;
  const int ox0 = xq * R, co0 = slice * sc + g * 8, ci0 = co0 / MULT;
  float acc[R][8];
  {
    const float4 b0 = *reinterpret_cast<const float4*>(bias + co0), b1 = *reinterpret_cast<const float4*>(bias + co0 + 4);
#pragma unroll
    for (int r = 0; r < R; ++r) {
      acc[r][0] = b0.x; acc[r][1] = b0.y; acc[r][2] = b0.z; acc[r][3] = b0.w;
      acc[r][4] = b1.x; acc[r][5] = b1.y; acc[r][6] = b1.z; acc[r][7] = b1.w;
    }
  }
#pragma unroll 1
  for (int ky = 0; ky < K; ++ky) {
    const int iy = oy * S - PAD + ky;
    if (iy < 0 || iy >= H) continue;
    float wr[K][8];
#pragma unroll
    for (int kx = 0; kx < K; ++kx) {
      const float* wp = sw + (ky * K + kx) * sc + g * 8;
      const float4 w0 = *reinterpret_cast<const float4*>(wp), w1 = *reinterpret_cast<const float4*>(wp + 4);
      wr[kx][0] = w0.x; wr[kx][1] = w0.y; wr[kx][2] = w0.z; wr[kx][3] = w0.w;
      wr[kx][4] = w1.x; wr[kx][5] = w1.y; wr[kx][6] = w1.z; wr[kx][7] = w1.w;
    }
    const bf16_t* rowp = x + ((size_t)b * H + iy) * W * C + ci0;
#pragma unroll
    for (int c = 0; c < NCOL; ++c) {
      const int ix = ox0 * S - PAD + c;
      const bool ok = ix >= 0 && ix < W;
      float xv[CI];
      if (MULT == 1) {
        const uint4 u = ok ? *reinterpret_cast<const uint4*>(rowp + (size_t)ix * C) : make_uint4(0, 0, 0, 0);
        unpack8(u, xv);
      } else {
        const uint2 u = ok ? *reinterpret_cast<const uint2*>(rowp + (size_t)ix * C) : make_uint2(0, 0);
        xv[0] = bf_lo(u.x); xv[1] = bf_hi(u.x); xv[2] = bf_lo(u.y); xv[3] = bf_hi(u.y);
      }
#pragma unroll
      for (int r = 0; r < R; ++r) {
        const int kx = c - r * S;
        if (kx >= 0 && kx < K) {
#pragma unroll
          for (int e = 0; e < 8; ++e) acc[r][e] += xv[e / MULT] * wr[kx][e];
        }
      }
    }
  }
#pragma unroll
  for (int r = 0; r < R; ++r) {
    if (ox0 + r >= Wo) break;
    if (gelu) {
#pragma unroll
      for (int e = 0; e < 8; ++e) acc[r][e] = gelu_f(acc[r][e]);
    }
    *reinterpret_cast<uint4*>(y + (((size_t)b * Ho + oy) * Wo + ox0 + r) * Cout + co0) = pack8(acc[r]);
  }
}

template <int K>
__global__ __launch_bounds__(256, 3) void dwconv_tile_kernel(const bf16_t* __restrict__ x, const float* __restrict__ w,
                                                           const float* __restrict__ bias, bf16_t* __restrict__ y,
                                                           int H, int W, int C, int gelu, int tiles_x, int tiles_y,
                                                           int nslices) {
  constexpr int TH = 8, TW = 32, CS = 32, PAD = K / 2, IH = TH + K - 1, IW = TW + K - 1;
  constexpr int ROWB = IW * 64 + ((IW + 3) / 4) * 64;
  __shared__ __attribute__((aligned(16))) char smem[IH * ROWB + K * K * CS * 4];
  float* sw = reinterpret_cast<float*>(smem + IH * ROWB);
  const int tid = threadIdx.x;
  int bid = blockIdx.x;
  const int slice = bid % nslices; bid /= nslices;
  const int tx = bid % tiles_x; bid /= tiles_x;
  const int tyb = bid % tiles_y;
  const long b = bid / tiles_y;
  const int c0 = slice * CS;
  for (int i = tid; i < K * K * CS; i += 256) sw[i] = w[(size_t)(i / CS) * C + c0 + (i % CS)];
  for (int i = tid; i < IH * IW * 4; i += 256) {
    const int chunk = i & 3, pc = i >> 2;
    const int col = pc % IW, row = pc / IW;
    const int iy = tyb * TH - PAD + row, ix = tx * TW - PAD + col;
    uint4 v = make_uint4(0, 0, 0, 0);
    if (iy >= 0 && iy < H && ix >= 0 && ix < W) v = *reinterpret_cast<const uint4*>(x + (((size_t)b * H + iy) * W + ix) * C + c0 + chunk * 8);
    *reinterpret_cast<uint4*>(smem + row * ROWB + col * 64 + (col >> 2) * 64 + chunk * 16) = v;
  }
  __syncthreads();
  const int g = tid & 3, qx = (tid >> 2) & 7, r_ = tid >> 5;
  const int oy = tyb * TH + r_, ox0 = tx * TW + qx * 4;
  float acc[4][8];
  {
    const float4 b0 = *reinterpret_cast<const float4*>(bias + c0 + g * 8), b1 = *reinterpret_cast<const float4*>(bias + c0 + g * 8 + 4);
#pragma unroll
    for (int r = 0; r < 4; ++r) {
      acc[r][0] = b0.x; acc[r][1] = b0.y; acc[r][2] = b0.z; acc[r][3] = b0.w;
      acc[r][4] = b1.x; acc[r][5] = b1.y; acc[r][6] = b1.z; acc[r][7] = b1.w;
    }
  }
#pragma unroll 1
  for (int ky = 0; ky < K; ++ky) {
    float wr[K][8];
#pragma unroll
    for (int kx = 0; kx < K; ++kx) {
      const float* wp = sw + (ky * K + kx) * CS + g * 8;
      const float4 w0 = *reinterpret_cast<const float4*>(wp), w1 = *reinterpret_cast<const float4*>(wp + 4);
      wr[kx][0] = w0.x; wr[kx][1] = w0.y; wr[kx][2] = w0.z; wr[kx][3] = w0.w;
      wr[kx][4] = w1.x; wr[kx][5] = w1.y; wr[kx][6] = w1.z; wr[kx][7] = w1.w;
    }
    const char* rowp = smem + (r_ + ky) * ROWB + g * 16;
#pragma unroll
    for (int c = 0; c < K + 3; ++c) {
      const int col = qx * 4 + c;
      float xv[8];
      unpack8(*reinterpret_cast<const uint4*>(rowp + col * 64 + (col >> 2) * 64), xv);
#pragma unroll
      for (int r = 0; r < 4; ++r) {
        const int kx = c - r;
        if (kx >= 0 && kx < K) {
#pragma unroll
          for (int e = 0; e < 8; ++e) acc[r][e] += xv[e] * wr[kx][e];
        }
      }
    }
  }
  if (oy >= H) return;
#pragma unroll
  for (int r = 0; r < 4; ++r) {
    if (ox0 + r >= W) break;
    if (gelu) {
#pragma unroll
      for (int e = 0; e < 8; ++e) acc[r][e] = gelu_f(acc[r][e]);
    }
    *reinterpret_cast<uint4*>(y + (((size_t)b * H + oy) * W + ox0 + r) * C + c0 + g * 8) = pack8(acc[r]);
  }
}

constexpr int SF_C = 96, SF_TR = 4, SF_TC = 32, SF_R1 = 2 * SF_TR + 1, SF_C1 = 2 * SF_TC + 1;
constexpr int SF_NSEG = (SF_R1 * SF_C1 + 15) / 16;
constexpr int SF_PS = SF_C * 2 + 16;
constexpr int SF_S1 = SF_R1 * SF_C1 * SF_PS;
constexpr int SF_PR = 4 * SF_TR + 3, SF_PCH = (4 * SF_TC + 4) / 2;
constexpr int SF_PATCH = SF_PR * SF_PCH * 16 + 16;
constexpr int SF_LDS = SF_S1 + 10 * SF_C * 4 + SF_PATCH;
constexpr int SF_PLD = (SF_PR * SF_PCH + 511) / 512;
template <bool LB>
__global__ __launch_bounds__(512, 1) void stem_fused_kernel(const bf16_t* __restrict__ pix, const bf16_t* __restrict__ wp,
                                                             const float* __restrict__ b1, const float* __restrict__ w2,
                                                             const float* __restrict__ b2, bf16_t* __restrict__ y, int B, int S,
                                                             long ntiles, LbParams lb) {
  extern __shared__ __attribute__((aligned(16))) char sf_smem[];
  char* s1 = sf_smem;
  float* sw2 = reinterpret_cast<float*>(sf_smem + SF_S1);
  char* spx = sf_smem + SF_S1 + 10 * SF_C * 4;
  const int tid = threadIdx.x, lane = tid & 63, wid = tid >> 6, fr = lane & 15, fg = lane >> 4;
  const int S1 = S >> 1, S2 = S >> 2;
  const int tiles_x = (S2 + SF_TC - 1) / SF_TC, tiles_y = (S2 + SF_TR - 1) / SF_TR;
  for (int i = tid; i < 10 * SF_C; i += 512) sw2[i] = i < 9 * SF_C ? w2[i] : b2[i - 9 * SF_C];
  bf16x8 wf[6][2];
#pragma unroll
  for (int nt = 0; nt < 6; ++nt)
#pragma unroll
    for (int ks = 0; ks < 2; ++ks)
      wf[nt][ks] = __builtin_bit_cast(bf16x8, *reinterpret_cast<const uint4*>(wp + ((size_t)(nt * 16 + fr) * 64 + ks * 32 + fg * 8)));
  float4 bv1[6];
#pragma unroll
  for (int nt = 0; nt < 6; ++nt) bv1[nt] = *reinterpret_cast<const float4*>(b1 + nt * 16 + fg * 4);

  uint4 pre[SF_PLD];
  auto patch_fetch = [&](unsigned tile) {
    const unsigned r_ = tile / (unsigned)tiles_x;
    const int tx = (int)(tile - r_ * (unsigned)tiles_x), ty = (int)(r_ % (unsigned)tiles_y);
    const long b = r_ / (unsigned)tiles_y;
    const int iy0 = 4 * ty * SF_TR - 3, ix0 = 4 * tx * SF_TC - 4;
#pragma unroll
    for (int j = 0; j < SF_PLD; ++j) {
      const int c = tid + 512 * j, r = c / SF_PCH, cc = c % SF_PCH;
      const int iy = iy0 + r, ix = ix0 + 2 * cc;
      const bool in_ = c < SF_PR * SF_PCH && iy >= 0 && iy < S && ix >= 0 && ix < S;
      if constexpr (LB) {
        pre[j] = make_uint4(0, 0, 0, 0);
        if (in_) {
          const uint2 p0 = lb_pixel(lb, (int)b, iy, ix), p1 = lb_pixel(lb, (int)b, iy, ix + 1);
          pre[j] = make_uint4(p0.x, p0.y, p1.x, p1.y);
        }
      } else {
        pre[j] = in_ ? *reinterpret_cast<const uint4*>(pix + (((size_t)b * S + iy) * S + ix) * 4) : make_uint4(0, 0, 0, 0);
      }
    }
  };
  auto patch_store = [&]() {
#pragma unroll
    for (int j = 0; j < SF_PLD; ++j) {
      const int c = tid + 512 * j;
      if (c < SF_PR * SF_PCH) *reinterpret_cast<uint4*>(spx + c * 16) = pre[j];
    }
  };
  if (tid == 0) *reinterpret_cast<uint4*>(spx + SF_PR * SF_PCH * 16) = make_uint4(0, 0, 0, 0);
  if ((long)blockIdx.x < ntiles) { patch_fetch(blockIdx.x); patch_store(); }

  for (unsigned tile = blockIdx.x; tile < (unsigned)ntiles; tile += gridDim.x) {
    const unsigned r_ = tile / (unsigned)tiles_x;
    const int tx = (int)(tile - r_ * (unsigned)tiles_x), ty = (int)(r_ % (unsigned)tiles_y);
    const long b = r_ / (unsigned)tiles_y;
    const int y1_0 = 2 * ty * SF_TR - 1, x1_0 = 2 * tx * SF_TC - 1;
    __syncthreads();
#define SF_FETCH(SEG, XF, LIVE)                                                                                  \
  {                                                                                                              \
    const int f_ = min((SEG) * 16 + fr, SF_R1 * SF_C1 - 1), r1_ = f_ / SF_C1, cs_ = f_ - r1_ * SF_C1;            \
    const int oy_ = y1_0 + r1_, ox_ = x1_0 + cs_;                                                                \
    LIVE = oy_ >= 0 && oy_ < S1 && ox_ >= 0 && ox_ < S1;                                                         \
    const char* pp_ = spx + ((2 * r1_ + (fg >> 1)) * SF_PCH * 2 + 2 * cs_ + 2 * (fg & 1) + 1) * 8;               \
    const uint2 l0_ = *reinterpret_cast<const uint2*>(pp_), h0_ = *reinterpret_cast<const uint2*>(pp_ + 8);      \
    uint2 l1_ = make_uint2(0, 0), h1_ = make_uint2(0, 0);                                                        \
    if (fg < 2) {                                                                                                \
      l1_ = *reinterpret_cast<const uint2*>(pp_ + 2 * SF_PCH * 16);                                              \
      h1_ = *reinterpret_cast<const uint2*>(pp_ + 2 * SF_PCH * 16 + 8);                                          \
    }                                                                                                            \
    XF[0] = __builtin_bit_cast(bf16x8, make_uint4(l0_.x, l0_.y, h0_.x, h0_.y));                                  \
    XF[1] = __builtin_bit_cast(bf16x8, make_uint4(l1_.x, l1_.y, h1_.x, h1_.y));                                  \
  }
    bf16x8 xf[2], xn[2];
    bool live, live_n;
    SF_FETCH(wid, xf, live)
    for (int seg = wid; seg < SF_NSEG; seg += 8) {
      SF_FETCH(seg + 8, xn, live_n)
      const int f = seg * 16 + fr;
      char* dst = s1 + f * SF_PS + fg * 8;
      f32x4 acc[6];
#pragma unroll
      for (int nt = 0; nt < 6; ++nt) {
        acc[nt] = __builtin_amdgcn_mfma_f32_16x16x32_bf16(wf[nt][0], xf[0], f32x4{0.f, 0.f, 0.f, 0.f}, 0, 0, 0);
        acc[nt] = __builtin_amdgcn_mfma_f32_16x16x32_bf16(wf[nt][1], xf[1], acc[nt], 0, 0, 0);
      }
#pragma unroll
      for (int np = 0; np < 3; ++np) {
        const int n0 = 2 * np, n1 = 2 * np + 1;
        f32x2 g[4] = {{acc[n0][0] + bv1[n0].x, acc[n0][1] + bv1[n0].y}, {acc[n0][2] + bv1[n0].z, acc[n0][3] + bv1[n0].w},
                      {acc[n1][0] + bv1[n1].x, acc[n1][1] + bv1[n1].y}, {acc[n1][2] + bv1[n1].z, acc[n1][3] + bv1[n1].w}};
        gelu2_n<4>(g);
        uint2 o0, o1;
        o0.x = live ? pack_bf2(g[0].x, g[0].y) : 0u;
        o0.y = live ? pack_bf2(g[1].x, g[1].y) : 0u;
        o1.x = live ? pack_bf2(g[2].x, g[2].y) : 0u;
        o1.y = live ? pack_bf2(g[3].x, g[3].y) : 0u;
        if (f < SF_R1 * SF_C1) {
          *reinterpret_cast<uint2*>(dst + n0 * 32) = o0;
          *reinterpret_cast<uint2*>(dst + n1 * 32) = o1;
        }
      }
      xf[0] = xn[0]; xf[1] = xn[1]; live = live_n;
    }
#undef SF_FETCH
    __syncthreads();
    const unsigned tile_n = tile + gridDim.x;
    if (tile_n < (unsigned)ntiles) patch_fetch(tile_n);
#pragma unroll 1
    for (int it = 0; it < SF_TR * SF_TC * (SF_C / 8) / 512; ++it) {
      const int item = tid + 512 * it;
      const int cg = item % (SF_C / 8), p = item / (SF_C / 8), pr = p / SF_TC, pc = p % SF_TC;
      float acc[8];
      {
        const float4 a0 = *reinterpret_cast<const float4*>(sw2 + 9 * SF_C + cg * 8), a1 = *reinterpret_cast<const float4*>(sw2 + 9 * SF_C + cg * 8 + 4);
        acc[0] = a0.x; acc[1] = a0.y; acc[2] = a0.z; acc[3] = a0.w; acc[4] = a1.x; acc[5] = a1.y; acc[6] = a1.z; acc[7] = a1.w;
      }
#pragma unroll
      for (int ky = 0; ky < 3; ++ky)
#pragma unroll
        for (int kx = 0; kx < 3; ++kx) {
          float xv[8];
          unpack8(*reinterpret_cast<const uint4*>(s1 + ((2 * pr + ky) * SF_C1 + 2 * pc + kx) * SF_PS + cg * 16), xv);
          const float* wt = sw2 + (ky * 3 + kx) * SF_C + cg * 8;
          const float4 w0 = *reinterpret_cast<const float4*>(wt), w1 = *reinterpret_cast<const float4*>(wt + 4);
          acc[0] += xv[0] * w0.x; acc[1] += xv[1] * w0.y; acc[2] += xv[2] * w0.z; acc[3] += xv[3] * w0.w;
          acc[4] += xv[4] * w1.x; acc[5] += xv[5] * w1.y; acc[6] += xv[6] * w1.z; acc[7] += xv[7] * w1.w;
        }
      f32x2 g[4] = {{acc[0], acc[1]}, {acc[2], acc[3]}, {acc[4], acc[5]}, {acc[6], acc[7]}};
      gelu2_n<4>(g);
      const int oy = ty * SF_TR + pr, ox = tx * SF_TC + pc;
      if (oy < S2 && ox < S2) {
        uint4 o;
        o.x = pack_bf2(g[0].x, g[0].y); o.y = pack_bf2(g[1].x, g[1].y); o.z = pack_bf2(g[2].x, g[2].y); o.w = pack_bf2(g[3].x, g[3].y);
        *reinterpret_cast<uint4*>(y + (((size_t)b * S2 + oy) * S2 + ox) * SF_C + cg * 8) = o;
      }
    }
    if (tile_n < (unsigned)ntiles) patch_store();
  }
}

typedef __attribute__((ext_vector_type(4))) short s16x4;

template <int K, int TH>
__global__ __launch_bounds__(256, TH == 8 ? 3 : 2) void dwconv_mfma_kernel(const bf16_t* __restrict__ x, const bf16_t* __restrict__ ttab,
                                                              const float* __restrict__ bias, bf16_t* __restrict__ y,
                                                              int H, int W, int C, int gelu, int tiles_x, int tiles_y,
                                                              int nslices) {
  constexpr int TW = 32, NP = TH / 8, PAD = K / 2, IH = TH + K - 1, IW = TW + K - 1;
  constexpr int NQ = (IW + 3) / 4, NM = (K + 3 + 3) / 4;
  constexpr int RS = NQ * 256 + 64;
  constexpr int T_BYTES = 2 * K * NM * 512, X_BYTES = IH * RS;
  __shared__ __attribute__((aligned(16))) char smem[X_BYTES];
  char* sX = smem;

  const int tid = threadIdx.x, lane = tid & 63, wid = tid >> 6;
#ifdef DW_NO_XCD
  int bid = blockIdx.x;
#else
  int bid = xcd_remap(blockIdx.x, gridDim.x);
#endif
  const int slice = bid % nslices; bid /= nslices;
  const int tx = bid % tiles_x; bid /= tiles_x;
  const int tyb = bid % tiles_y;
  const long b = bid / tiles_y;
  const int c0 = slice * 32;
  const int gg = wid & 1, rg = wid >> 1;
  const int bch = lane >> 2, jr = lane & 3;

  s16x4 afr[K][NM];
  {
    const char* tsrc = reinterpret_cast<const char*>(ttab) + (size_t)slice * T_BYTES + (size_t)gg * K * NM * 512 + lane * 8;
#pragma unroll
    for (int ky = 0; ky < K; ++ky)
#pragma unroll
      for (int m = 0; m < NM; ++m) afr[ky][m] = __builtin_bit_cast(s16x4, *reinterpret_cast<const uint2*>(tsrc + (ky * NM + m) * 512));
  }
  constexpr int NTASK = IH * NQ * 4, TPT = (NTASK + 255) / 256;
  uint4 px[TPT][4];
#pragma unroll
  for (int tt = 0; tt < TPT; ++tt) {
    const int task = tid + 256 * tt;
    const int cg = task & 3, quad = (task >> 2) % NQ, row = (task >> 2) / NQ;
    const int iy = tyb * TH - PAD + row, ix0 = tx * TW - PAD + quad * 4;
#pragma unroll
    for (int j = 0; j < 4; ++j) {
      const int ix = ix0 + j;
      px[tt][j] = (task < NTASK && iy >= 0 && iy < H && ix >= 0 && ix < W && quad * 4 + j < IW)
                      ? *reinterpret_cast<const uint4*>(x + (((size_t)b * H + iy) * W + ix) * C + c0 + cg * 8)
                      : make_uint4(0, 0, 0, 0);
    }
  }
#pragma unroll
  for (int tt = 0; tt < TPT; ++tt) {
    const int task = tid + 256 * tt;
    if (task < NTASK) {
      const int cg = task & 3, quad = (task >> 2) % NQ, row = (task >> 2) / NQ;
      const uint32_t d[4][4] = {{px[tt][0].x, px[tt][0].y, px[tt][0].z, px[tt][0].w}, {px[tt][1].x, px[tt][1].y, px[tt][1].z, px[tt][1].w},
                                {px[tt][2].x, px[tt][2].y, px[tt][2].z, px[tt][2].w}, {px[tt][3].x, px[tt][3].y, px[tt][3].z, px[tt][3].w}};
      const uint32_t dst = (uint32_t)(row * RS + quad * 256 + cg * 64) | (uint32_t)((((quad & 3) << 1) | (cg >> 1)) << 3);
#pragma unroll
      for (int dd = 0; dd < 4; ++dd) {
        uint2 ev, od;
        ev.x = __builtin_amdgcn_perm(d[1][dd], d[0][dd], 0x05040100u);
        ev.y = __builtin_amdgcn_perm(d[3][dd], d[2][dd], 0x05040100u);
        od.x = __builtin_amdgcn_perm(d[1][dd], d[0][dd], 0x07060302u);
        od.y = __builtin_amdgcn_perm(d[3][dd], d[2][dd], 0x07060302u);
        *reinterpret_cast<uint2*>(sX + (dst ^ (uint32_t)((2 * dd) * 8))) = ev;
        *reinterpret_cast<uint2*>(sX + (dst ^ (uint32_t)((2 * dd + 1) * 8))) = od;
      }
    }
  }
  __syncthreads();

  const char* lrow[4];
#pragma unroll
  for (int v = 0; v < 4; ++v) lrow[v] = sX + (rg * 4 * NP + jr) * RS + (((gg * 16 + bch) ^ ((v << 1) | gg)) << 3);
  f32x4 acc[NP][8];
#pragma unroll
  for (int pp = 0; pp < NP; ++pp)
#pragma unroll
    for (int q = 0; q < 8; ++q) acc[pp][q] = f32x4{0.f, 0.f, 0.f, 0.f};
#pragma unroll
  for (int pp = 0; pp < NP; ++pp)
#pragma unroll
    for (int ky = 0; ky < K; ++ky) {
      s16x4 xq[NQ];
#pragma unroll
      for (int t = 0; t < NQ; ++t)
        xq[t] = __builtin_bit_cast(s16x4, *reinterpret_cast<const uint2*>(lrow[t & 3] + (pp * 4 + ky) * RS + t * 256));
#pragma unroll
      for (int q = 0; q < 8; ++q)
#pragma unroll
        for (int m = 0; m < NM; ++m)
#ifdef DW_ABL_MFMA
          if (q + m < NQ && m == 0) acc[pp][q] = __builtin_amdgcn_mfma_f32_4x4x4bf16_1k(afr[ky][m], xq[q + m], acc[pp][q], 0, 0, 0);
#else
          if (q + m < NQ) acc[pp][q] = __builtin_amdgcn_mfma_f32_4x4x4bf16_1k(afr[ky][m], xq[q + m], acc[pp][q], 0, 0, 0);
#endif
    }
  __syncthreads();

  {
    const float bv = bias[c0 + gg * 16 + bch];
#pragma unroll
    for (int pp = 0; pp < NP; ++pp)
#pragma unroll
      for (int q = 0; q < 8; ++q) {
        float v[4];
#pragma unroll
        for (int i = 0; i < 4; ++i) {
          v[i] = acc[pp][q][i] + bv;
          if (gelu) v[i] = gelu_f(v[i]);
        }
        uint2 u;
        u.x = pack_bf2(v[0], v[1]);
        u.y = pack_bf2(v[2], v[3]);
        *reinterpret_cast<uint2*>(const_cast<char*>(lrow[q & 3]) + pp * 4 * RS + q * 256) = u;
      }
  }
  __syncthreads();
#pragma unroll
  for (int ot = 0; ot < NP; ++ot) {
    const int task = tid + 256 * ot;
    const int cg = task & 3, quad = (task >> 2) & 7, row = task >> 5;
    const uint32_t src = (uint32_t)(row * RS + quad * 256 + cg * 64) | (uint32_t)((((quad & 3) << 1) | (cg >> 1)) << 3);
    uint2 r[8];
#pragma unroll
    for (int e = 0; e < 8; ++e) r[e] = *reinterpret_cast<const uint2*>(sX + (src ^ (uint32_t)(e * 8)));
    const int oy = tyb * TH + row, ox0 = tx * TW + quad * 4;
    if (oy < H) {
      bf16_t* yp = y + (((size_t)b * H + oy) * W + ox0) * C + c0 + cg * 8;
#pragma unroll
      for (int j = 0; j < 4; ++j) {
        if (ox0 + j < W) {
          uint4 o;
          const uint32_t sel = (j & 1) ? 0x07060302u : 0x05040100u;
#define FV_PX(A, B) __builtin_amdgcn_perm((j & 2) ? r[B].y : r[B].x, (j & 2) ? r[A].y : r[A].x, sel)
          o.x = FV_PX(0, 1); o.y = FV_PX(2, 3); o.z = FV_PX(4, 5); o.w = FV_PX(6, 7);
#undef FV_PX
          *reinterpret_cast<uint4*>(yp + (size_t)j * C) = o;
        }
      }
    }
  }
}

__global__ __launch_bounds__(256, 2) void dwconv_s2_mfma_kernel(const bf16_t* __restrict__ x, const bf16_t* __restrict__ ttab,
                                                                 const float* __restrict__ bias, bf16_t* __restrict__ y, int H,
                                                                 int W, int C, int Ho, int Wo, int gelu, int tiles_x, int tiles_y,
                                                                 int nslices, int nimg) {
  constexpr int K = 7, TH = 8, TW = 16, PAD = 3, IH = 2 * TH + K - 2, IW = 2 * TW + K - 2;
  constexpr int NQ = (IW + 3) / 4, NM = 4;
  constexpr int RS = NQ * 256 + 64;
  constexpr int X_BYTES = IH * RS;
  constexpr int OC = 512 + 16;
  static_assert(TH * 4 * OC <= X_BYTES, "the output tile reuses the halo tile's LDS");
  __shared__ __attribute__((aligned(16))) char smem[X_BYTES];
  char* sX = smem;
  const int tid = threadIdx.x, lane = tid & 63, wid = tid >> 6;
  const int xcd = blockIdx.x & 7, lb = blockIdx.x >> 3;
  const int slice = lb % nslices, chain = lb / nslices, chains = (int)(gridDim.x >> 3) / nslices;
  const int ntiles = nimg * tiles_x * tiles_y;
  const int tpx = (ntiles + 7) >> 3, t_end = min((xcd + 1) * tpx, ntiles), per_slice = chains;
  const int c0 = slice * 32;
  const int gg = wid & 1, eo = wid >> 1;
  const int bch = lane >> 2, jr = lane & 3;

  s16x4 afr[K][NM];
  {
    const char* tsrc = reinterpret_cast<const char*>(ttab) + (size_t)(slice * 2 + gg) * (2 * K * NM * 512) + (size_t)eo * (K * NM * 512) + lane * 8;
#pragma unroll
    for (int ky = 0; ky < K; ++ky)
#pragma unroll
      for (int m = 0; m < NM; ++m) afr[ky][m] = __builtin_bit_cast(s16x4, *reinterpret_cast<const uint2*>(tsrc + (ky * NM + m) * 512));
  }
  constexpr int NTASK = IH * NQ * 4, TPT = (NTASK + 255) / 256;
  uint4 px[TPT][4];
  int trow[TPT], tcol[TPT], toff[TPT];
  uint32_t tdst[TPT];
#pragma unroll
  for (int tt = 0; tt < TPT; ++tt) {
    const int task = min(tid + 256 * tt, NTASK - 1);
    const int cg = task & 3, quad = (task >> 2) % NQ, row = (task >> 2) / NQ;
    trow[tt] = row;
    tcol[tt] = quad * 4;
    toff[tt] = (row * W + quad * 4) * C + cg * 8;
    tdst[tt] = (uint32_t)(row * RS + quad * 256 + cg * 64) | (uint32_t)((((quad & 3) << 1) | (cg >> 1)) << 3);
  }
  auto fetch = [&](int tx, int tyb, int b) {
    const int iy0 = 2 * tyb * TH - PAD, ix0 = 2 * tx * TW - PAD;
    const bf16_t* org = x + ((long)b * H * W + (long)iy0 * W + ix0) * C + c0;
#pragma unroll
    for (int tt = 0; tt < TPT; ++tt) {
      const bool rok = (unsigned)(iy0 + trow[tt]) < (unsigned)H;
#pragma unroll
      for (int j = 0; j < 4; ++j)
        px[tt][j] = (rok && (unsigned)(ix0 + tcol[tt] + j) < (unsigned)W) ? *reinterpret_cast<const uint4*>(org + toff[tt] + j * C)
                                                                         : make_uint4(0, 0, 0, 0);
    }
  };
  auto decode = [&](int tile, int& tx, int& tyb, int& b) {
    const unsigned t = (unsigned)tile, r = t / (unsigned)tiles_x;
    tx = (int)(t - r * (unsigned)tiles_x);
    b = (int)(r / (unsigned)tiles_y);
    tyb = (int)(r - (unsigned)b * (unsigned)tiles_y);
  };
  int tile = xcd * tpx + chain, tx = 0, tyb = 0, b = 0, txn = 0, tybn = 0, bn = 0;
  if (tile < t_end) { decode(tile, tx, tyb, b); fetch(tx, tyb, b); }
  for (; tile < t_end; tile += per_slice) {
#pragma unroll
  for (int tt = 0; tt < TPT; ++tt) {
    if (tid + 256 * tt < NTASK) {
      const uint32_t d[4][4] = {{px[tt][0].x, px[tt][0].y, px[tt][0].z, px[tt][0].w}, {px[tt][1].x, px[tt][1].y, px[tt][1].z, px[tt][1].w},
                                {px[tt][2].x, px[tt][2].y, px[tt][2].z, px[tt][2].w}, {px[tt][3].x, px[tt][3].y, px[tt][3].z, px[tt][3].w}};
      const uint32_t dst = tdst[tt];
#pragma unroll
      for (int dd = 0; dd < 4; ++dd) {
        uint2 ev, od;
        ev.x = __builtin_amdgcn_perm(d[1][dd], d[0][dd], 0x05040100u);
        ev.y = __builtin_amdgcn_perm(d[3][dd], d[2][dd], 0x05040100u);
        od.x = __builtin_amdgcn_perm(d[1][dd], d[0][dd], 0x07060302u);
        od.y = __builtin_amdgcn_perm(d[3][dd], d[2][dd], 0x07060302u);
        *reinterpret_cast<uint2*>(sX + (dst ^ (uint32_t)((2 * dd) * 8))) = ev;
        *reinterpret_cast<uint2*>(sX + (dst ^ (uint32_t)((2 * dd + 1) * 8))) = od;
      }
    }
  }
  __syncthreads();
  if (tile + per_slice < t_end) { decode(tile + per_slice, txn, tybn, bn); fetch(txn, tybn, bn); }

  const char* lrow[4];
#pragma unroll
  for (int v = 0; v < 4; ++v) lrow[v] = sX + (2 * jr) * RS + (((gg * 16 + bch) ^ ((v << 1) | gg)) << 3);
  f32x4 acc[2][4];
#pragma unroll
  for (int rg = 0; rg < 2; ++rg)
#pragma unroll
    for (int q = 0; q < 4; ++q) acc[rg][q] = f32x4{0.f, 0.f, 0.f, 0.f};
#pragma unroll
  for (int ky = 0; ky < K; ++ky)
#pragma unroll
    for (int rg = 0; rg < 2; ++rg) {
      s16x4 xq[NQ];
#pragma unroll
      for (int t = 0; t < NQ; ++t) xq[t] = __builtin_bit_cast(s16x4, *reinterpret_cast<const uint2*>(lrow[t & 3] + (rg * 8 + ky) * RS + t * 256));
#pragma unroll
      for (int m = 0; m < NM; ++m)
#pragma unroll
        for (int q = 0; q < 4; ++q) acc[rg][q] = __builtin_amdgcn_mfma_f32_4x4x4bf16_1k(afr[ky][m], xq[2 * q + m], acc[rg][q], 0, 0, 0);
    }
  __syncthreads();

  {
    const int co = 2 * (gg * 16 + bch) + eo, sig = (jr >> 1) & 1;
    const float bv = bias[2 * c0 + co];
#pragma unroll
    for (int rg = 0; rg < 2; ++rg)
#pragma unroll
      for (int q = 0; q < 4; ++q) {
        f32x2 g[2] = {{acc[rg][q][0] + bv, acc[rg][q][1] + bv}, {acc[rg][q][2] + bv, acc[rg][q][3] + bv}};
        if (gelu) gelu2_n<2>(g);
        uint2 u;
        u.x = pack_bf2(g[0].x, g[0].y);
        u.y = pack_bf2(g[1].x, g[1].y);
        *reinterpret_cast<uint2*>(sX + ((rg * 4 + jr) * 4 + q) * OC + ((co ^ sig) << 3)) = u;
      }
  }
  __syncthreads();
  {
    const int cg = tid & 7, quad = (tid >> 3) & 3, row = tid >> 5;
    const int sig = (row >> 1) & 1;
    uint2 r[8];
#pragma unroll
    for (int e = 0; e < 8; ++e) r[e] = *reinterpret_cast<const uint2*>(sX + (row * 4 + quad) * OC + (((cg * 8 + e) ^ sig) << 3));
    const int oy = tyb * TH + row, ox0 = tx * TW + quad * 4;
    if (oy < Ho) {
      bf16_t* yp = y + (((size_t)b * Ho + oy) * Wo + ox0) * (2 * C) + 2 * c0 + cg * 8;
#pragma unroll
      for (int j = 0; j < 4; ++j) {
        if (ox0 + j < Wo) {
          uint4 o;
          const uint32_t sel = (j & 1) ? 0x07060302u : 0x05040100u;
#define FV_PX(A, B) __builtin_amdgcn_perm((j & 2) ? r[B].y : r[B].x, (j & 2) ? r[A].y : r[A].x, sel)
          o.x = FV_PX(0, 1); o.y = FV_PX(2, 3); o.z = FV_PX(4, 5); o.w = FV_PX(6, 7);
#undef FV_PX
          *reinterpret_cast<uint4*>(yp + (size_t)j * (2 * C)) = o;
        }
      }
    }
  }
  __syncthreads();
  tx = txn; tyb = tybn; b = bn;
  }
}

#ifndef DW_MARCH_OCC
#define DW_MARCH_OCC 2
#endif
typedef __attribute__((ext_vector_type(4))) _Float16 f16x4_t;
template <int K, bool GRAD = false>
// ... 554 lines not shown
    }
  }
  const float rstd = rsqrtf(wave_sum(q) / (float)C + eps);
#pragma unroll
  for (int i = 0; i < 4; ++i) {
    const int ch = lane + 64 * i;
    if (ch < nch) {
      float o[8];
#pragma unroll
      for (int e = 0; e < 8; ++e) o[e] = (v[i][e] - mean) * rstd * w[ch * 8 + e] + bb[ch * 8 + e];
      *reinterpret_cast<uint4*>(y + row * C + ch * 8) = pack8(o);
    }
  }
}

__global__ __launch_bounds__(256) void se_pool_kernel(const bf16_t* __restrict__ x, float* __restrict__ pooled, int P,
                                                       int C) {
  __shared__ float part[16][16][8];
  const int cgl = threadIdx.x & 15, pr = threadIdx.x >> 4;
  const int ch = blockIdx.x * 16 + cgl, b = blockIdx.y;
  float a[8] = {0, 0, 0, 0, 0, 0, 0, 0};
  if (ch < (C >> 3)) {
    for (int p = pr; p < P; p += 16) {
      float v[8];
      unpack8(*reinterpret_cast<const uint4*>(x + ((size_t)b * P + p) * C + ch * 8), v);
#pragma unroll
      for (int e = 0; e < 8; ++e) a[e] += v[e];
    }
  }
#pragma unroll
  for (int e = 0; e < 8; ++e) part[pr][cgl][e] = a[e];
  __syncthreads();
  if (threadIdx.x < 128) {
    const int c = threadIdx.x >> 3, e = threadIdx.x & 7, chn = blockIdx.x * 16 + c;
    if (chn < (C >> 3)) {
      float t = 0.f;
#pragma unroll
      for (int q = 0; q < 16; ++q) t += part[q][c][e];
      pooled[(size_t)b * C + chn * 8 + e] = t / (float)P;
    }
  }
}

__global__ __launch_bounds__(256) void se_fc_kernel(const float* __restrict__ x, const float* __restrict__ W,
                                                     const float* __restrict__ bias, float* __restrict__ y, int N,
                                                     int K, int act) {
  const int lane = threadIdx.x & 63;
  const int n = blockIdx.x * 4 + (threadIdx.x >> 6), b = blockIdx.y;
  if (n >= N) return;
  float s = 0.f;
  for (int k = lane; k < K; k += 64) s += x[(size_t)b * K + k] * W[(size_t)n * K + k];
  s = wave_sum(s) + bias[n];
  if (lane == 0) y[(size_t)b * N + n] = act == 0 ? fmaxf(s, 0.f) : sigmoid_f(s);
}

__global__ __launch_bounds__(256) void se_apply_gelu_kernel(const bf16_t* __restrict__ x, const float* __restrict__ sc,
                                                             bf16_t* __restrict__ y, int P, int C, long total_chunks) {
  const long i = (long)blockIdx.x * 256 + threadIdx.x;
  if (i >= total_chunks) return;
  const int nch = C >> 3;
  const int ch = (int)(i % nch);
  const long b = i / ((long)nch * P);
  float v[8];
  unpack8(*reinterpret_cast<const uint4*>(x + i * 8), v);
  const float* s = sc + b * C + ch * 8;
#pragma unroll
  for (int e = 0; e < 8; ++e) v[e] = gelu_f(v[e] * s[e]);
  *reinterpret_cast<uint4*>(y + i * 8) = pack8(v);
}

}

#ifndef FV_TRY_RC
#define FV_TRY_RC(expr) do { const int rc_ = (expr); if (rc_ != FV_OK) return rc_; } while (0)
#endif
namespace {
int lb_params(const void* img, int dtype, int B, int C, int Hin, int Win, int S, float pad_value, int letterbox, bf16_t* pix, LbParams& p) {
  if (B <= 0 || Hin <= 0 || Win <= 0 || S <= 0) return fv_fail(FV_ERR_ARG, "letterbox: empty shape");
  if (C != 1 && C != 3 && C != 4) return fv_fail(FV_ERR_ARG, "letterbox: C must be 1, 3 or 4 (got %d)", C);
  if (dtype != FV_F32 && dtype != FV_U8) return fv_fail(FV_ERR_ARG, "letterbox: dtype must be f32 or u8");
  p.img = img; p.pix = pix; p.dtype = dtype; p.B = B; p.C = C; p.Hin = Hin; p.Win = Win; p.S = S; p.pad = pad_value;
  if (letterbox) {
    const double ratio = ((double)Win / S > (double)Hin / S) ? (double)Win / S : (double)Hin / S;
    p.rh = (int)((double)Hin / ratio);
    p.rw = (int)((double)Win / ratio);
    if (p.rh > S || p.rw > S || p.rh < 1 || p.rw < 1) return fv_fail(FV_ERR_ARG, "letterbox: degenerate resize %dx%d", p.rh, p.rw);
  } else {
    p.rh = S; p.rw = S;
  }
  p.pt = S - p.rh; p.pl = S - p.rw;
  p.sh = (float)Hin / (float)p.rh;
  p.sw = (float)Win / (float)p.rw;
  return FV_OK;
}
}

int launch_letterbox(const void* img, int dtype, int B, int C, int Hin, int Win, int S, float pad_value, int letterbox,
                     bf16_t* pix, hipStream_t s) {
  if (!img || !pix) return fv_fail(FV_ERR_ARG, "letterbox: null pointer");
  LbParams p;
  FV_TRY_RC(lb_params(img, dtype, B, C, Hin, Win, S, pad_value, letterbox, pix, p));
  hipLaunchKernelGGL(letterbox_kernel<0>, dim3((S + 255) / 256, (S + LB_R - 1) / LB_R, B), dim3(256), 0, s, p, LbNorm{});
  FV_HIP_CHECK(hipGetLastError());
  return FV_OK;
}

int launch_letterbox_norm(const void* img, int dtype, int B, int C, int Hin, int Win, int S, float pad_value, int letterbox, const float* mean3,
                          const float* std3, int range_heuristic, unsigned* vmax_scratch, bf16_t* pix, hipStream_t s) {
  if (!img || !pix || !mean3 || !std3 || (range_heuristic && !vmax_scratch)) return fv_fail(FV_ERR_ARG, "letterbox_norm: null pointer");
  LbParams p;
  FV_TRY_RC(lb_params(img, dtype, B, C, Hin, Win, S, pad_value, letterbox, pix, p));
  LbNorm n{};
  for (int c = 0; c < 3; ++c) {
    if (!(std3[c] != 0.0f)) return fv_fail(FV_ERR_ARG, "letterbox_norm: std[%d] must be non-zero", c);
    n.mean[c] = mean3[c]; n.std[c] = std3[c];
  }
  n.vmax = vmax_scratch; n.heuristic = range_heuristic ? 1 : 0;
  const dim3 grid((S + 255) / 256, (S + LB_R - 1) / LB_R, B);
  if (range_heuristic) {
    FV_HIP_CHECK(hipMemsetAsync(vmax_scratch, 0, 4, s));
    hipLaunchKernelGGL(letterbox_kernel<1>, grid, dim3(256), 0, s, p, n);
  }
  hipLaunchKernelGGL(letterbox_kernel<2>, grid, dim3(256), 0, s, p, n);
  FV_HIP_CHECK(hipGetLastError());
  return FV_OK;
}

int launch_stem_conv(const bf16_t* pix, const float* w, const float* bias, bf16_t* y, int B, int S, int Cout,
                     hipStream_t s) {
  if (!pix || !w || !bias || !y) return fv_fail(FV_ERR_ARG, "stem_conv: null pointer");
  if (B <= 0 || S < 2 || (S & 1) || Cout % 8 || Cout < 8 || Cout > 2048) return fv_fail(FV_ERR_ARG, "stem_conv: bad shape S=%d Cout=%d", S, Cout);
  const int So = S / 2, G = Cout / 8, WQ = (So + 3) / 4, per_block = 256 / G;
  const long quads = (long)B * So * WQ;
  const long blocks = (quads + per_block - 1) / per_block;
  hipLaunchKernelGGL(stem_conv_kernel, dim3((unsigned)blocks), dim3(256), 27 * Cout * sizeof(float), s, pix, w, bias, y, B, S, Cout);
  FV_HIP_CHECK(hipGetLastError());
  return FV_OK;
}

void stem_mfma_pack(const float* w27, float* out, int Cout) {
  for (int co = 0; co < Cout; ++co)
    for (int ks = 0; ks < 2; ++ks)
      for (int g = 0; g < 4; ++g)
        for (int e = 0; e < 8; ++e) {
          const int ky = 2 * ks + (g >> 1), kx = 2 * (g & 1) + (e >> 2), ch = e & 3;
          out[(size_t)co * 64 + ks * 32 + g * 8 + e] = (ky < 3 && kx < 3 && ch < 3) ? w27[(size_t)((ky * 3 + kx) * 3 + ch) * Cout + co] : 0.0f;
        }
}

int launch_stem_mfma(const bf16_t* pix, const bf16_t* wp, const float* bias, bf16_t* y, int B, int S, int Cout, hipStream_t s) {
  if (!pix || !wp || !bias || !y) return fv_fail(FV_ERR_ARG, "stem_mfma: null pointer");
  if (B <= 0 || S < 2 || (S & 1) || Cout % 16 || Cout > 128) return fv_fail(FV_ERR_UNSUPPORTED, "stem_mfma: bad shape S=%d Cout=%d", S, Cout);
  const int So = S / 2;
  const long ntiles = (long)B * So * ((So + 15) / 16);
  constexpr int TPW = 8;
  const long blocks = (ntiles + 4 * TPW - 1) / (4 * TPW);
  hipLaunchKernelGGL(stem_mfma_kernel<TPW>, dim3((unsigned)blocks), dim3(256), 0, s, pix, wp, bias, y, B, S, Cout, ntiles);
  FV_HIP_CHECK(hipGetLastError());
  return FV_OK;
}

int launch_dwconv(const bf16_t* x, const float* w, const float* bias, bf16_t* y, int B, int H, int W, int C, int k,
                  int stride, int mult, int gelu, hipStream_t s) {
  if (!x || !w || !bias || !y) return fv_fail(FV_ERR_ARG, "dwconv: null pointer");
  if (B <= 0 || H <= 0 || W <= 0 || C <= 0 || (C * mult) % 8) return fv_fail(FV_ERR_ARG, "dwconv: bad shape C=%d mult=%d", C, mult);
  const int pad = k / 2;
  const int Ho = (H + 2 * pad - k) / stride + 1, Wo = (W + 2 * pad - k) / stride + 1;
  if (stride == 1 && mult == 1 && (k == 3 || k == 7) && W >= 32 && C % 32 == 0) {
    const int tiles_x = (W + 31) / 32, tiles_y = (H + 7) / 8, nsl = C / 32;
    const long nblk = (long)B * tiles_x * tiles_y * nsl;
    if (nblk > 0x7fffffffL) return fv_fail(FV_ERR_ARG, "dwconv: grid too large");
    if (k == 7) hipLaunchKernelGGL(dwconv_tile_kernel<7>, dim3((unsigned)nblk), dim3(256), 0, s, x, w, bias, y, H, W, C, gelu, tiles_x, tiles_y, nsl);
    else hipLaunchKernelGGL(dwconv_tile_kernel<3>, dim3((unsigned)nblk), dim3(256), 0, s, x, w, bias, y, H, W, C, gelu, tiles_x, tiles_y, nsl);
    FV_HIP_CHECK(hipGetLastError());
    return FV_OK;
  }
  const int G = C * mult / 8, WQ = (Wo + 3) / 4;
  int GS = 1;
  for (int d = 1; d <= 16; ++d)
    if (G % d == 0) GS = d;
  const int nslices = G / GS, qpb = 256 / GS;
  const long nquads = (long)B * Ho * WQ;
  const long blocks = (nquads + qpb - 1) / qpb * nslices;
  if (blocks > 0x7fffffffL) return fv_fail(FV_ERR_ARG, "dwconv: grid too large");
  const dim3 grid((unsigned)blocks);
#define FV_DW(K_, S_, M_)                                                                                        \
  if (k == K_ && stride == S_ && mult == M_) {                                                                   \
    hipLaunchKernelGGL((dwconv_kernel<K_, S_, M_>), grid, dim3(256), 0, s, x, w, bias, y, B, H, W, C, Ho, Wo, gelu, \
                       GS, nslices, nquads);                                                                     \
    FV_HIP_CHECK(hipGetLastError());                                                                             \
    return FV_OK;                                                                                                \
  }
  FV_DW(3, 1, 1) FV_DW(7, 1, 1) FV_DW(3, 2, 1) FV_DW(7, 2, 2) FV_DW(3, 1, 2)
#undef FV_DW
  return fv_fail(FV_ERR_UNSUPPORTED, "dwconv: unsupported k=%d stride=%d mult=%d", k, stride, mult);
}

size_t dwconv_toeplitz_elems(int C, int k) { return (size_t)(C / 16) * k * ((k + 6) / 4) * 256; }
void dwconv_toeplitz_pack(const float* w_tapmajor, float* out, int C, int k) {
  const int NM = (k + 6) / 4;
  for (int g = 0; g < C / 16; ++g)
    for (int ky = 0; ky < k; ++ky)
      for (int m = 0; m < NM; ++m)
        for (int bch = 0; bch < 16; ++bch)
          for (int i = 0; i < 4; ++i)
            for (int kk = 0; kk < 4; ++kk) {
              const int kx = 4 * m + kk - i;
              out[((((size_t)(g * k + ky) * NM + m) * 16 + bch) * 4 + i) * 4 + kk] =
                  (kx >= 0 && kx < k) ? w_tapmajor[(size_t)(ky * k + kx) * C + g * 16 + bch] : 0.0f;
            }
}
size_t dwconv_s2_toeplitz_elems(int C) { return (size_t)(C / 16) * 2 * 7 * 4 * 256; }
void dwconv_s2_toeplitz_pack(const float* w_tapmajor, float* out, int C) {
  for (int g = 0; g < C / 16; ++g)
    for (int e = 0; e < 2; ++e)
      for (int ky = 0; ky < 7; ++ky)
        for (int m = 0; m < 4; ++m)
          for (int bch = 0; bch < 16; ++bch)
            for (int i = 0; i < 4; ++i)
              for (int kk = 0; kk < 4; ++kk) {
                const int kx = 4 * m + kk - 2 * i;
                out[(((((size_t)(g * 2 + e) * 7 + ky) * 4 + m) * 16 + bch) * 4 + i) * 4 + kk] =
                    (kx >= 0 && kx < 7) ? w_tapmajor[(size_t)(ky * 7 + kx) * (2 * C) + 2 * (g * 16 + bch) + e] : 0.0f;
              }
}
bool dwconv_s2_mfma_supported(int H, int W, int C, int k, int stride, int mult) {
  return k == 7 && stride == 2 && mult == 2 && C % 32 == 0 && H % 2 == 0 && W % 2 == 0 && W >= 16;
}
int launch_dwconv_s2_mfma(const bf16_t* x, const bf16_t* ttab, const float* bias, bf16_t* y, int B, int H, int W, int C, int gelu,
                          hipStream_t s) {
  if (!x || !ttab || !bias || !y) return fv_fail(FV_ERR_ARG, "dwconv_s2_mfma: null pointer");
  if (B <= 0 || H <= 0 || !dwconv_s2_mfma_supported(H, W, C, 7, 2, 2)) return fv_fail(FV_ERR_UNSUPPORTED, "dwconv_s2_mfma: unsupported shape H=%d W=%d C=%d", H, W, C);
  const int Ho = H / 2, Wo = W / 2;
  const int tiles_x = (Wo + 15) / 16, tiles_y = (Ho + 7) / 8, nsl = C / 32;
  const long nblk = (long)B * tiles_x * tiles_y * nsl;
  if (nblk > 0x7fffffffL) return fv_fail(FV_ERR_ARG, "dwconv_s2_mfma: grid too large");
  static int cus = 0;
  if (!cus) {
    int dev = 0;
    hipDeviceProp_t prop;
    cus = (hipGetDevice(&dev) == hipSuccess && hipGetDeviceProperties(&prop, dev) == hipSuccess && prop.multiProcessorCount > 0) ? prop.multiProcessorCount : 256;
  }
  const long tiles = nblk / nsl, tpx = (tiles + 7) / 8;
  long chains = (2L * cus / 8) / nsl;
  if (chains < 1) chains = 1;
  if (chains > tpx) chains = tpx;
  hipLaunchKernelGGL(dwconv_s2_mfma_kernel, dim3((unsigned)(8 * chains * nsl)), dim3(256), 0, s, x, ttab, bias, y, H, W, C, Ho, Wo, gelu, tiles_x, tiles_y, nsl, B);
  FV_HIP_CHECK(hipGetLastError());
  return FV_OK;
}

bool dwconv_mfma_supported(int W, int C, int k, int stride, int mult) {
  return stride == 1 && mult == 1 && (k == 3 || k == 7) && W >= 16 && C % 32 == 0;
}

int launch_dwconv_mfma(const bf16_t* x, const bf16_t* ttab, const float* bias, bf16_t* y, int B, int H, int W, int C, int k,
                       int gelu, hipStream_t s) {
  if (!x || !ttab || !bias || !y) return fv_fail(FV_ERR_ARG, "dwconv_mfma: null pointer");
  if (B <= 0 || H <= 0 || !dwconv_mfma_supported(W, C, k, 1, 1)) return fv_fail(FV_ERR_UNSUPPORTED, "dwconv_mfma: unsupported shape W=%d C=%d k=%d", W, C, k);
#ifndef DW_TH7
#define DW_TH7 8
#endif
  const int th = (k == 7 && H >= 32) ? DW_TH7 : 8;
  const int tiles_x = (W + 31) / 32, tiles_y = (H + th - 1) / th, nsl = C / 32;
  const long nblk = (long)B * tiles_x * tiles_y * nsl;
  if (nblk > 0x7fffffffL) return fv_fail(FV_ERR_ARG, "dwconv_mfma: grid too large");
#ifndef DW_NO_MARCH
  if (k == 7 && H >= 16) {
    const long nstrips = (long)B * tiles_x * nsl;
    hipLaunchKernelGGL((dwconv_march_kernel<7>), dim3((unsigned)nstrips), dim3(256), 0, s, x, ttab, bias, y, H, W, C, gelu, tiles_x, nsl);
    FV_HIP_CHECK(hipGetLastError());
    return FV_OK;
  }
#ifdef DW_MARCH3
  if (k == 3 && H >= 16) {
    const long nstrips = (long)B * tiles_x * nsl;
    hipLaunchKernelGGL((dwconv_march_kernel<3>), dim3((unsigned)nstrips), dim3(256), 0, s, x, ttab, bias, y, H, W, C, gelu, tiles_x, nsl);
    FV_HIP_CHECK(hipGetLastError());
    return FV_OK;
  }
#endif
#endif
  if (k == 7 && th == 16) hipLaunchKernelGGL((dwconv_mfma_kernel<7, 16>), dim3((unsigned)nblk), dim3(256), 0, s, x, ttab, bias, y, H, W, C, gelu, tiles_x, tiles_y, nsl);
  else if (k == 7) hipLaunchKernelGGL((dwconv_mfma_kernel<7, 8>), dim3((unsigned)nblk), dim3(256), 0, s, x, ttab, bias, y, H, W, C, gelu, tiles_x, tiles_y, nsl);
  else hipLaunchKernelGGL((dwconv_mfma_kernel<3, 8>), dim3((unsigned)nblk), dim3(256), 0, s, x, ttab, bias, y, H, W, C, gelu, tiles_x, tiles_y, nsl);
  FV_HIP_CHECK(hipGetLastError());
  return FV_OK;
}

bool dw_dgrad_mfma_supported(int H, int W, int C, int k) { return dwconv_mfma_supported(W, C, k, 1, 1) && H >= 16; }
int launch_dw_dgrad_mfma(const bf16_t* dy, const bf16_t* ttab16, const bf16_t* res, bf16_t* dx, int B, int H, int W, int C, int k, hipStream_t s) {
  if (!dy || !ttab16 || !dx) return fv_fail(FV_ERR_ARG, "dw_dgrad_mfma: null pointer");
  if (B <= 0 || !dw_dgrad_mfma_supported(H, W, C, k)) return fv_fail(FV_ERR_UNSUPPORTED, "dw_dgrad_mfma: unsupported shape H=%d W=%d C=%d k=%d", H, W, C, k);
  const int tiles_x = (W + 31) / 32, nsl = C / 32;
  const long nstrips = (long)B * tiles_x * nsl;
  if (nstrips > 0x7fffffffL) return fv_fail(FV_ERR_ARG, "dw_dgrad_mfma: grid too large");
  if (k == 7) hipLaunchKernelGGL((dwconv_march_kernel<7, true>), dim3((unsigned)nstrips), dim3(256), 0, s, dy, ttab16, static_cast<const float*>(nullptr), dx, H, W, C, 0, tiles_x, nsl, res);
  else hipLaunchKernelGGL((dwconv_march_kernel<3, true>), dim3((unsigned)nstrips), dim3(256), 0, s, dy, ttab16, static_cast<const float*>(nullptr), dx, H, W, C, 0, tiles_x, nsl, res);
  FV_HIP_CHECK(hipGetLastError());
  return FV_OK;
}

bool stem_fused_supported(int S, int C0) { return C0 == SF_C && S >= 8 && S % 4 == 0; }
int launch_stem_fused(const bf16_t* pix, const bf16_t* wp, const float* b1, const float* w2, const float* b2, bf16_t* y, int B,
                      int S, int C0, hipStream_t s) {
  if (!pix || !wp || !b1 || !w2 || !b2 || !y) return fv_fail(FV_ERR_ARG, "stem_fused: null pointer");
  if (B <= 0 || !stem_fused_supported(S, C0)) return fv_fail(FV_ERR_UNSUPPORTED, "stem_fused: bad shape S=%d C0=%d", S, C0);
  static bool attr_set = false;
  if (!attr_set) {
    FV_HIP_CHECK(hipFuncSetAttribute(reinterpret_cast<const void*>(&stem_fused_kernel<false>), hipFuncAttributeMaxDynamicSharedMemorySize, SF_LDS));
    attr_set = true;
  }
  const int S2 = S / 4;
  const long ntiles = (long)B * ((S2 + SF_TC - 1) / SF_TC) * ((S2 + SF_TR - 1) / SF_TR);
  if (ntiles > 0x3fffffffL) return fv_fail(FV_ERR_ARG, "stem_fused: too many tiles");
  int dev = 0, cus = 256;
  hipDeviceProp_t prop;
  if (hipGetDevice(&dev) == hipSuccess && hipGetDeviceProperties(&prop, dev) == hipSuccess && prop.multiProcessorCount > 0) cus = prop.multiProcessorCount;
  const long blocks = ntiles < cus ? ntiles : cus;
  hipLaunchKernelGGL(stem_fused_kernel<false>, dim3((unsigned)blocks), dim3(512), SF_LDS, s, pix, wp, b1, w2, b2, y, B, S, ntiles, LbParams{});
  FV_HIP_CHECK(hipGetLastError());
  return FV_OK;
}

int launch_stem_fused_lb(const void* img, int dtype, int B, int C, int Hin, int Win, float pad_value, int letterbox, const bf16_t* wp,
                         const float* b1, const float* w2, const float* b2, bf16_t* y, int S, int C0, hipStream_t s) {
  if (!img || !wp || !b1 || !w2 || !b2 || !y) return fv_fail(FV_ERR_ARG, "stem_fused_lb: null pointer");
  if (B <= 0 || !stem_fused_supported(S, C0)) return fv_fail(FV_ERR_UNSUPPORTED, "stem_fused_lb: bad shape S=%d C0=%d", S, C0);
  LbParams p;
  FV_TRY_RC(lb_params(img, dtype, B, C, Hin, Win, S, pad_value, letterbox, nullptr, p));
  static bool attr_set = false;
  if (!attr_set) {
    FV_HIP_CHECK(hipFuncSetAttribute(reinterpret_cast<const void*>(&stem_fused_kernel<true>), hipFuncAttributeMaxDynamicSharedMemorySize, SF_LDS));
    attr_set = true;
  }
  const int S2 = S / 4;
  const long ntiles = (long)B * ((S2 + SF_TC - 1) / SF_TC) * ((S2 + SF_TR - 1) / SF_TR);
  if (ntiles > 0x3fffffffL) return fv_fail(FV_ERR_ARG, "stem_fused_lb: too many tiles");
  int dev = 0, cus = 256;
  hipDeviceProp_t prop;
  if (hipGetDevice(&dev) == hipSuccess && hipGetDeviceProperties(&prop, dev) == hipSuccess && prop.multiProcessorCount > 0) cus = prop.multiProcessorCount;
  const long blocks = ntiles < cus ? ntiles : cus;
  hipLaunchKernelGGL(stem_fused_kernel<true>, dim3((unsigned)blocks), dim3(512), SF_LDS, s, nullptr, wp, b1, w2, b2, y, B, S, ntiles, p);
  FV_HIP_CHECK(hipGetLastError());
  return FV_OK;
}

bool dwconv_pair_supported(int B, int H, int W, int C) {
  return H >= 16 && W >= 32 && C % 32 == 0 && ((long)B * H + 16) * W * C * 2 <= 0x7FFFFFF0L;
}
int launch_dwconv_pair(const bf16_t* x, const bf16_t* t3, const float* b3, const bf16_t* t7, const float* b7, bf16_t* y1, bf16_t* y2,
                       int B, int H, int W, int C, hipStream_t s) {
  if (!x || !t3 || !b3 || !t7 || !b7 || !y1 || !y2) return fv_fail(FV_ERR_ARG, "dwconv_pair: null pointer");
  if (B <= 0 || !dwconv_pair_supported(B, H, W, C)) return fv_fail(FV_ERR_UNSUPPORTED, "dwconv_pair: unsupported shape H=%d W=%d C=%d", H, W, C);
  if (x == y1 || x == y2 || y1 == y2) return fv_fail(FV_ERR_ARG, "dwconv_pair: buffers must be distinct");
  static bool attr_set = false;
  if (!attr_set) {
    FV_HIP_CHECK(hipFuncSetAttribute(reinterpret_cast<const void*>(&dwpair_march_kernel<32, 32>), hipFuncAttributeMaxDynamicSharedMemorySize, DpGeo<32, 32>::LDS));
    FV_HIP_CHECK(hipFuncSetAttribute(reinterpret_cast<const void*>(&dwpair_march_kernel<64, 16>), hipFuncAttributeMaxDynamicSharedMemorySize, DpGeo<64, 16>::LDS));
    FV_HIP_CHECK(hipFuncSetAttribute(reinterpret_cast<const void*>(&dwpair_march_kernel<32, 16>), hipFuncAttributeMaxDynamicSharedMemorySize, DpGeo<32, 16>::LDS));
#if DP_DEFAULT_GEO == 3
    FV_HIP_CHECK(hipFuncSetAttribute(reinterpret_cast<const void*>(&dwpair_march_kernel<64, 8>), hipFuncAttributeMaxDynamicSharedMemorySize, DpGeo<64, 8>::LDS));
#endif
    attr_set = true;
  }
  int geo = DP_DEFAULT_GEO;
  if ((geo == 1 || geo == 3) && C % 64) geo = 0;
  const int chb = (geo == 1 || geo == 3) ? 64 : 32, tw = geo == 0 ? 32 : geo == 3 ? 8 : 16;
  const int tiles_x = (W + tw - 1) / tw, nsl = C / chb;
  long nstrips = (long)B * tiles_x * nsl;
  if (nstrips > 0x7fffffffL) return fv_fail(FV_ERR_ARG, "dwconv_pair: grid too large");
  int nseg = 1;
  if (nstrips < 256) {
    const int ng = (H + 7) / 8;
    nseg = (int)((512 + nstrips - 1) / nstrips);
    if (nseg > ng / 2) nseg = ng / 2;
    if (nseg < 1) nseg = 1;
  }
  nstrips *= nseg;
#if DP_DEFAULT_GEO == 3
  if (geo == 3)
    hipLaunchKernelGGL((dwpair_march_kernel<64, 8>), dim3((unsigned)nstrips), dim3(256), (DpGeo<64, 8>::LDS), s, x, t3, b3, t7, b7, y1, y2, H, W, C, tiles_x, nsl, nseg);
  else
#endif
  if (geo == 1)
    hipLaunchKernelGGL((dwpair_march_kernel<64, 16>), dim3((unsigned)nstrips), dim3(256), (DpGeo<64, 16>::LDS), s, x, t3, b3, t7, b7, y1, y2, H, W, C, tiles_x, nsl, nseg);
  else if (geo == 2)
    hipLaunchKernelGGL((dwpair_march_kernel<32, 16>), dim3((unsigned)nstrips), dim3(256), (DpGeo<32, 16>::LDS), s, x, t3, b3, t7, b7, y1, y2, H, W, C, tiles_x, nsl, nseg);
  else
    hipLaunchKernelGGL((dwpair_march_kernel<32, 32>), dim3((unsigned)nstrips), dim3(256), (DpGeo<32, 32>::LDS), s, x, t3, b3, t7, b7, y1, y2, H, W, C, tiles_x, nsl, nseg);
  FV_HIP_CHECK(hipGetLastError());
  return FV_OK;
}

int launch_layernorm_rows(const bf16_t* x, const float* w, const float* b, bf16_t* y, int rows, int C, float eps,
                          hipStream_t s) {
  if (!x || !w || !b || !y) return fv_fail(FV_ERR_ARG, "layernorm_rows: null pointer");
  if (rows <= 0 || C % 8 || C > 2048 || C <= 0) return fv_fail(FV_ERR_ARG, "layernorm_rows: bad shape rows=%d C=%d", rows, C);
  hipLaunchKernelGGL(layernorm_rows_kernel, dim3((rows + 3) / 4), dim3(256), 0, s, x, w, b, y, rows, C, eps);
  FV_HIP_CHECK(hipGetLastError());
  return FV_OK;
}

int launch_se_gelu(const bf16_t* x, const float* w1, const float* b1, const float* w2, const float* b2, bf16_t* y,
                   float* scratch, int B, int P, int C, int R, hipStream_t s) {
  if (!x || !w1 || !b1 || !w2 || !b2 || !y || !scratch) return fv_fail(FV_ERR_ARG, "se_gelu: null pointer");
  if (B <= 0 || P <= 0 || C % 8 || R <= 0) return fv_fail(FV_ERR_ARG, "se_gelu: bad shape");
  float* pooled = scratch;
  float* hid = pooled + (size_t)B * C;
  float* sc = hid + (size_t)B * R;
  hipLaunchKernelGGL(se_pool_kernel, dim3((C / 8 + 15) / 16, B), dim3(256), 0, s, x, pooled, P, C);
  hipLaunchKernelGGL(se_fc_kernel, dim3((R + 3) / 4, B), dim3(256), 0, s, pooled, w1, b1, hid, R, C, 0);
  hipLaunchKernelGGL(se_fc_kernel, dim3((C + 3) / 4, B), dim3(256), 0, s, hid, w2, b2, sc, C, R, 1);
  const long chunks = (long)B * P * (C / 8);
  hipLaunchKernelGGL(se_apply_gelu_kernel, dim3((unsigned)((chunks + 255) / 256)), dim3(256), 0, s, x, sc, y, P, C, chunks);
  FV_HIP_CHECK(hipGetLastError());
  return FV_OK;
}

}

#ifdef DP_STAMPS
extern "C" int fv_dbg_dp_stamps(unsigned long long* out) { return (int)hipMemcpyFromSymbol(out, HIP_SYMBOL(fv::g_dp_stamps), 512 * 16 * 8); }
#endif
```

### vla-from-fastvlm_amd/fastvla_hip/_lib.py

```python
from __future__ import annotations

import ctypes as C
import os
from pathlib import Path

FV_MAX_STAGES = 8
FV_F32, FV_BF16, FV_U8, FV_I32 = 0, 1, 2, 3
EPI_BIAS, EPI_BIAS_GELU, EPI_LS_RES, EPI_RES_F32, EPI_SWIGLU, EPI_F32 = range(6)
EPI_SWIGLU_SPLIT = 7
EPI_SWIGLU_F16 = 8


class FastVLAHipError(RuntimeError):
    status = 0


class ModelDesc(C.Structure):
    _fields_ = [
        ("llm_hidden", C.c_int32), ("llm_layers", C.c_int32), ("llm_heads", C.c_int32), ("llm_kv_heads", C.c_int32),
        ("llm_head_dim", C.c_int32), ("llm_inter", C.c_int32), ("llm_vocab", C.c_int32),
        ("rope_theta", C.c_float), ("rms_eps", C.c_float),
        ("tower_stages", C.c_int32),
        ("tower_layers", C.c_int32 * FV_MAX_STAGES), ("tower_dims", C.c_int32 * FV_MAX_STAGES),
        ("tower_is_attn", C.c_int32 * FV_MAX_STAGES),
        ("tower_mlp_ratio", C.c_int32), ("tower_head_dim", C.c_int32), ("tower_se_rd", C.c_int32),
        ("tower_out_dim", C.c_int32),
        ("ln_eps", C.c_float), ("bn_eps", C.c_float),
        ("image_size", C.c_int32),
        ("state_dim", C.c_int32), ("action_dim", C.c_int32), ("hidden_dim", C.c_int32), ("fusion_dim", C.c_int32),
        ("max_batch", C.c_int32), ("max_text_tokens", C.c_int32), ("tower_microbatch", C.c_int32),
        ("llm_precision", C.c_int32),
    ]


class TensorDesc(C.Structure):
    _fields_ = [("name", C.c_char_p), ("data", C.c_void_p), ("dtype", C.c_int32), ("ndim", C.c_int32),
                ("shape", C.c_int64 * 4), ("device", C.c_int32), ("reserved", C.c_int32)]


class RcclId(C.Structure):
    _fields_ = [("internal", C.c_char * 128)]


TENSOR_PROVIDER = C.CFUNCTYPE(C.c_int, C.c_void_p, C.c_char_p, C.POINTER(TensorDesc))


class AdamWHParams(C.Structure):
    _fields_ = [("lr", C.c_float), ("beta1", C.c_float), ("beta2", C.c_float), ("eps", C.c_float),
                ("weight_decay", C.c_float), ("max_grad_norm", C.c_float), ("grad_scale", C.c_float)]


class ProfileEntry(C.Structure):
    _fields_ = [("ms", C.c_double), ("flops", C.c_double), ("bytes", C.c_double), ("launches", C.c_int64)]


class GemmProfile(C.Structure):
    _fields_ = [("m", C.c_int32), ("n", C.c_int32), ("k", C.c_int32), ("epi", C.c_int32), ("ms", C.c_double),
                ("launches", C.c_int64)]


class TrainTensor(C.Structure):
    _fields_ = [("name", C.c_char * 104), ("offset", C.c_int64), ("numel", C.c_int64), ("rows", C.c_int32), ("cols", C.c_int32),
                ("bucket", C.c_int32), ("packing", C.c_int32)]


BUCKET_CB = C.CFUNCTYPE(None, C.c_void_p, C.c_int, C.c_int64, C.c_int64)

FAMILIES = ("gemm", "dwconv", "stem", "attention", "norm", "elementwise", "head")

_vp, _i, _f, _u64, _i64 = C.c_void_p, C.c_int, C.c_float, C.c_uint64, C.c_int64

SIGNATURES = {
    "fv_create": (_i, [C.POINTER(ModelDesc), _i, C.POINTER(_vp)]),
    "fv_load_weights": (_i, [_vp, C.POINTER(TensorDesc), _i]),
    "fv_load_weights_cb": (_i, [_vp, TENSOR_PROVIDER, _vp]),
    "fv_destroy": (None, [_vp]),
    "fv_last_error": (C.c_char_p, [_vp]),
    "fv_version": (C.c_char_p, []),
    "fv_workspace_bytes": (_i, [_vp, _i, _i, _i, C.POINTER(C.c_size_t)]),
    "fv_bind_workspace": (_i, [_vp, _vp, C.c_size_t]),
    "fv_preprocess": (_i, [_vp, _vp, _i, _i, _i, _i, _i, _f, _i, _vp, _vp]),
    "fv_preprocess_normalized": (_i, [_vp, _vp, _i, _i, _i, _i, _i, _f, _i, _vp, _vp, _i, _vp, _vp]),
    "fv_vision_forward": (_i, [_vp, _vp, _i, _vp, _vp, _vp]),
    "fv_vision_forward_images": (_i, [_vp, _vp, _i, _i, _i, _i, _i, _f, _i, _vp, _vp, _vp]),
    "fv_vision_forward_taps": (_i, [_vp, _vp, _i, _vp, _vp, C.POINTER(_vp), _i, _vp]),
    "fv_vision_unit_info": (_i, [_vp, _i, C.POINTER(C.c_int32), C.POINTER(C.c_int32), C.POINTER(C.c_int32), C.POINTER(C.c_int32)]),
    "fv_vision_forward_unit_taps": (_i, [_vp, _vp, _i, _vp, _vp, C.POINTER(_vp), _i, _vp]),
    "fv_llm_forward_pooled": (_i, [_vp, _vp, _vp, _vp, _i, _i, _i, _i, _vp, _vp]),
    "fv_llm_fp16_saturations": (_i, [_vp, C.POINTER(_u64), _i]),
    "fv_set_batch_invariant": (_i, [_vp, _i]),
    "fv_llm_prefix_bytes": (_i, [_vp, _i, _i, C.POINTER(C.c_size_t)]),
    "fv_llm_prefix": (_i, [_vp, _vp, _i, _i, _vp, _vp]),
    "fv_llm_forward_pooled_prefixed": (_i, [_vp, _vp, _vp, _vp, _i, _i, _i, _i, _vp, _vp]),
    "fv_head_layout": (_i, [_vp, C.POINTER(_i64 * 13)]),
    "fv_head_saved_bytes": (_i, [_vp, _i, C.POINTER(C.c_size_t)]),
    "fv_head_forward": (_i, [_vp, _vp, _vp, _vp, _i, _i, _f, _u64, _u64, _vp, _vp, _vp]),
    "fv_head_set_io_norm": (_i, [_vp, _vp, _vp, _vp, _vp, _f]),
    "fv_head_mse_backward": (_i, [_vp, _vp, _vp, _vp, _i, _f, _vp, _vp, _vp, _vp]),
    "fv_head_backward": (_i, [_vp, _vp, _vp, _i, _f, _vp, _vp, _vp]),
    "fv_grad_accumulate": (_i, [_vp, _vp, _vp, _i64, _vp]),
    "fv_grad_scale": (_i, [_vp, _vp, _i64, _vp, _vp]),
    "fv_comm_unique_id": (_i, [_vp, C.POINTER(RcclId)]),
    "fv_comm_init": (_i, [_vp, C.POINTER(RcclId), _i, _i, C.POINTER(_vp)]),
    "fv_comm_destroy": (_i, [_vp, _vp]),
    "fv_allreduce_grads": (_i, [_vp, _vp, _vp, _i64, _vp]),
    "fv_train_layout": (_i, [_vp, C.POINTER(TrainTensor), _i, C.POINTER(_i), C.POINTER(_i64), C.POINTER(_i)]),
    "fv_train_begin": (_i, [_vp]),
    "fv_train_export_params": (_i, [_vp, _vp, _vp]),
    "fv_train_commit": (_i, [_vp, _vp, _vp]),
    "fv_train_set_options": (_i, [_vp, _i, _i, _i]),
    "fv_train_loss_scale": (_i, [_vp, C.POINTER(_f)]),
    "fv_train_set_forward_f16": (_i, [_vp, _i]),
    "fv_train_workspace_bytes": (_i, [_vp, _i, _i, C.POINTER(C.c_size_t)]),
    "fv_train_forward_backward": (_i, [_vp, _vp, _vp, _vp, _vp, _vp, _vp, _i, _i, _i, _f, _u64, _u64, _vp, C.c_size_t, _vp, _vp, _vp, BUCKET_CB, _vp, _vp]),
    "fv_train_lora_begin": (_i, [_vp, _i, _f, _i]),
    "fv_train_lora_begin_ex": (_i, [_vp, _i, _f, _i, _i]),
    "fv_train_lora_init_magnitude": (_i, [_vp, _vp, _vp, _vp]),
    "fv_train_lora_layout": (_i, [_vp, C.POINTER(TrainTensor), _i, C.POINTER(_i), C.POINTER(_i64)]),
    "fv_train_lora_project": (_i, [_vp, _vp, _vp, _vp, _vp]),
    "fv_train_lora_commit": (_i, [_vp, _vp, _vp, _vp]),
    "fv_train_lora_merge": (_i, [_vp, _vp, _vp, _vp]),
    "fv_train_lora_forward_backward": (_i, [_vp, _vp, _vp, _vp, _vp, _vp, _vp, _vp, _i, _i, _i, _f, _u64, _u64, _vp, C.c_size_t, _vp, _vp, _vp, _vp]),
    "fv_train_tower_begin": (_i, [_vp]),
    "fv_train_tower_workspace_bytes": (_i, [_vp, _i, C.POINTER(C.c_size_t)]),
    "fv_train_tower_forward": (_i, [_vp, _vp, _i, _vp, C.c_size_t, _vp, _vp]),
    "fv_train_set_tower_grad": (_i, [_vp, _vp]),
    "fv_train_tower_backward": (_i, [_vp, _vp, _vp, _i, _vp, C.c_size_t, _vp, BUCKET_CB, _vp, _vp]),
    "fv_train_tower_read_unit": (_i, [_vp, _i, _i, _vp, C.c_size_t, _vp, _vp]),
    "fv_train_tower_unit": (_i, [_vp, _i, _vp, _vp, _f, _i, _vp, C.c_size_t, _vp, _vp, _vp, _vp]),
    "fv_profile": (_i, [_vp, _i]),
    "fv_profile_read": (_i, [_vp, C.POINTER(ProfileEntry), C.POINTER(GemmProfile), _i, C.POINTER(_i)]),
    "fv_adamw_clip_step": (_i, [_vp, _vp, _vp, _vp, _vp, _i64, C.POINTER(AdamWHParams), _i64, _vp, _vp]),
}

OPS_SIGNATURES = {
    "fv_op_gemm": (_i, [_vp, _i, _vp, _i, _i, _i, _vp, _vp, _vp, _i, _vp, _i, _i, _vp]),
    "fv_op_gemm_f16": (_i, [_vp, _i, _vp, _i, _i, _i, _vp, _vp, _i, _vp, _i, _i, _vp, C.c_size_t, _vp]),
    "fv_op_gemm_lo8": (_i, [_vp, _i, _vp, _vp, _i, _i, _i, _vp, _vp, _i, _vp, _i, _i, _vp, C.c_size_t, _vp]),
    "fv_op_lo8_pack": (_i, [_vp, _vp, _i, _vp, _vp, _i, _i, _i, _vp]),
    "fv_op_gemm_ksplit": (_i, [_vp, _i, _vp, _i, _i, _i, _vp, _vp, _i, _vp, _i, _i, _vp]),
    "fv_op_gemm_tn": (_i, [_vp, _i, _vp, _i, _i, _i, _i, _i, _vp, _vp, _i, _vp, C.c_size_t, _vp]),
    "fv_op_gemm_splitk": (_i, [_vp, _i, _vp, _i, _i, _i, _vp, _vp, _i, _vp, _i, _i, _i, _vp, C.c_size_t, _vp]),
    "fv_op_dwconv": (_i, [_vp, _vp, _vp, _vp, _i, _i, _i, _i, _i, _i, _i, _i, _vp]),
    "fv_op_stem_conv": (_i, [_vp, _vp, _vp, _vp, _i, _i, _i, _vp]),
    "fv_op_stem_mfma": (_i, [_vp, _vp, _vp, _vp, _i, _i, _i, _vp]),
    "fv_op_stem_fused": (_i, [_vp, _vp, _vp, _vp, _vp, _vp, _i, _i, _i, _vp]),
    "fv_op_stem_fused_images": (_i, [_vp, _i, _i, _i, _i, _i, _f, _i, _vp, _vp, _vp, _vp, _vp, _i, _i, _vp]),
    "fv_op_layernorm_rows": (_i, [_vp, _vp, _vp, _vp, _i, _i, _f, _vp]),
    "fv_op_attention": (_i, [_vp, _vp, _vp, _i, _i, _i, _vp, _i, _i, _i, _i, _i, _i, _i, _vp, _f, _vp]),
    "fv_op_rmsnorm": (_i, [_vp, _vp, _vp, _i, _i, _f, _vp]),
    "fv_op_rope": (_i, [_vp, _i, _i, _i, _i, _i, _i, _f, _vp]),
    "fv_op_dwconv_mfma": (_i, [_vp, _vp, _vp, _vp, _i, _i, _i, _i, _i, _i, _vp]),
    "fv_op_dwconv_s2_mfma": (_i, [_vp, _vp, _vp, _vp, _i, _i, _i, _i, _i, _vp]),
    "fv_op_dwconv_pair": (_i, [_vp, _vp, _vp, _vp, _vp, _vp, _vp, _i, _i, _i, _i, _vp]),
    "fv_op_convffn": (_i, [_vp, _vp, _vp, _vp, _vp, _vp, _vp, _vp, _i, _i, _vp]),
    "fv_op_convffn32": (_i, [_vp, _vp, _vp, _vp, _vp, _vp, _vp, _i, _i, _vp]),
    "fv_op_convffn32_stash": (_i, [_vp, _vp, _vp, _vp, _vp, _vp, _vp, _i, _i, _vp, _vp]),
    "fv_op_gemm_f16_gelup": (_i, [_vp, _i, _vp, _i, _i, _i, _vp, _i, _vp, _i, _vp, _vp]),
    "fv_op_dw_wgrad": (_i, [_vp, _vp, _vp, _vp, _vp, C.c_size_t, _i, _i, _i, _i, _i, _i, _i, _vp]),
    "fv_op_convffn32_split": (_i, [_vp, _vp, _vp, _vp, _vp, _vp, _vp, _i, _i, _vp, C.c_size_t, _vp]),
    "fv_op_lora_direct_scratch_floats": (_i, [_i, _i, _i, C.POINTER(C.c_size_t)]),
    "fv_op_lora_direct": (_i, [_i, _i, _i, _i, _i, _i, _i, _vp, _vp, _vp, _vp, _i, _i, _i, _i, _vp, _vp, _f, _vp, C.c_size_t, _vp]),
    "fv_op_attention_bwd": (_i, [_vp, _i, _vp, _vp, _vp, _vp, _i, _i, _i, _i, _i, _vp, _f, _vp]),
    "fv_op_rmsnorm_bwd": (_i, [_vp, _vp, _vp, _vp, _vp, _vp, _vp, _i, _i, _f, _vp]),
    "fv_op_se_gelu": (_i, [_vp, _vp, _vp, _vp, _vp, _vp, _vp, _i, _i, _i, _i, _vp]),
}

_LIB = None
_OPS = None


def library_path() -> Path:
    env = os.environ.get("FASTVLA_HIP_LIB")
    return Path(env) if env else Path(__file__).resolve().parent / "libfastvla_hip.so"


def load():
    global _LIB
    if _LIB is not None:
        return _LIB
    path = library_path()
    if not path.is_file():
        raise FastVLAHipError(f"{path} not found: build it with `python -c 'import __graft_entry__ as g; g.build()'` "
                              "(make -C vla-from-fastvlm_amd/csrc).  There is no CPU fallback.")
    try:
        lib = C.CDLL(str(path))
    except OSError as exc:
        raise FastVLAHipError(f"cannot load {path}: {exc}") from exc
    for name, (res, args) in SIGNATURES.items():
        fn = getattr(lib, name)
        fn.restype = res
        fn.argtypes = args
    _LIB = lib
    return lib


def testops_path() -> Path:
    env = os.environ.get("FASTVLA_HIP_TESTOPS_LIB")
    if env:
        return Path(env)
    if os.environ.get("FASTVLA_HIP_LIB"):
        lp = library_path()
        return lp.with_name(lp.stem + "_testops.so")
    return Path(__file__).resolve().parents[2] / "tests" / "_native" / "libfastvla_hip_testops.so"


class _WithTestOps:

    def __init__(self, product, ops):
        self._product, self._ops = product, ops

    def __getattr__(self, name):
        try:
            return getattr(self._product, name)
        except AttributeError:
            return getattr(self._ops, name)


def load_testops():
    global _OPS
    if _OPS is not None:
        return _OPS
    product = load()
    if hasattr(product, "fv_op_gemm"):
        for name, (res, args) in OPS_SIGNATURES.items():
            fn = getattr(product, name)
            fn.restype = res
            fn.argtypes = args
        _OPS = product
        return _OPS
    path = testops_path()
    if not path.is_file():
        raise FastVLAHipError(f"{path} not found: `make -C vla-from-fastvlm_amd/csrc` builds it beside the product library (test-only entry points)")
    try:
        C.CDLL(str(library_path()), mode=C.RTLD_GLOBAL)
        ops = C.CDLL(str(path))
    except OSError as exc:
        raise FastVLAHipError(f"cannot load {path}: {exc}") from exc
    for name, (res, args) in OPS_SIGNATURES.items():
        fn = getattr(ops, name)
        fn.restype = res
        fn.argtypes = args
    _OPS = _WithTestOps(product, ops)
    return _OPS


def check(rc: int, what: str = "", handle=None) -> None:
    if rc != 0:
        msg = load().fv_last_error(handle)
        err = FastVLAHipError(f"{what or 'libfastvla_hip'} failed (status {rc}): {msg.decode() if msg else '?'}")
        err.status = int(rc)
        raise err
```

Before: 18.99 steps/s.

## Stage letterbox source window in LDS and optionally fuse stem 1x1 conv

The fused stem kernel gains a mode that loads the small source-image window each tile needs into LDS, along with per-axis interpolation tables. Letterbox resampling then reads from shared memory instead of doing repeated bilinear global gathers. An opt-in path also fuses the following 1x1 conv with bias and GELU into the stem kernel via MFMA, skipping a separate GEMM and one intermediate round trip. The cost is more LDS, more template variants and extra sync points in the tile loop.

```diff
diff --git a/include/fastvla_hip_testops.h b/include/fastvla_hip_testops.h
--- a/include/fastvla_hip_testops.h
+++ b/include/fastvla_hip_testops.h
@@ -42,6 +42,11 @@
                      int S, int Cout, fv_stream s);
 int fv_op_stem_fused_images(const void* img, int dtype, int B, int C, int Hin, int Win, float pad_value, int resize_with_padding, const void* wp,
                             const float* b1, const float* w2, const float* b2, void* y, int S, int Cout, fv_stream s);
+int fv_op_stem_fused_pw(const void* pix, const void* wp, const float* b1, const float* w2, const float* b2, const void* w3, const float* b3, void* y,
+                        int B, int S, int Cout, fv_stream s);
+int fv_op_stem_fused_images_pw(const void* img, int dtype, int B, int C, int Hin, int Win, float pad_value, int resize_with_padding, const void* wp,
+                               const float* b1, const float* w2, const float* b2, const void* w3, const float* b3, void* y, int S, int Cout,
+                               fv_stream s);
 int fv_op_layernorm_rows(const void* x, const float* w, const float* b, void* y, int rows, int C, float eps,
                          fv_stream s);
 int fv_op_attention(const void* q, const void* k, const void* v, int ldq, int ldk, int ldv, void* out, int ldo, int B,
diff --git a/vla-from-fastvlm_amd/csrc/engine.hip b/vla-from-fastvlm_amd/csrc/engine.hip
--- a/vla-from-fastvlm_amd/csrc/engine.hip
+++ b/vla-from-fastvlm_amd/csrc/engine.hip
@@ -528,18 +528,27 @@
   float* se = reinterpret_cast<float*>(ws + wp.se);
   const int S = d.image_size, C0 = d.tower_dims[0];
   static const bool fuse_stem = !fv_ab_env("FASTVLA_NO_FUSED_STEM");
+  bool stem2_done = false;
+  static const bool stem_pw = fv_ab_env("FASTVLA_STEM_PW") != nullptr;
+  const bool pw_in = stem_pw && tw.stem2_w && tw.stem2_b;
+  const bf16_t* w3 = pw_in ? tw.stem2_w : nullptr;
+  const float* b3 = pw_in ? tw.stem2_b : nullptr;
+  bf16_t* stem_out = pw_in ? cur : oth;
+  const double pw_flops = pw_in ? 2.0 * mb * (S / 4) * (S / 4) * (double)C0 * C0 : 0.0;
   if (h->lbsrc) {
     const fv_handle::LbSrc& L = *h->lbsrc;
     if (!(tw.stem0_wp && fv::stem_fused_supported(S, C0))) return fv_fail(FV_ERR_UNSUPPORTED, "fv_vision_forward_images needs the fused stem (first stage width 96)");
     const size_t per = (size_t)L.C * L.Hin * L.Win * (L.dtype == FV_U8 ? 1 : 4);
-    FV_P(FV_FAM_STEM, 2.0 * mb * (S / 2) * (S / 2) * 27 * C0 + dw_flops(mb, S / 4, S / 4, C0, 3) + 30.0 * mb * S * S,
+    FV_P(FV_FAM_STEM, 2.0 * mb * (S / 2) * (S / 2) * 27 * C0 + dw_flops(mb, S / 4, S / 4, C0, 3) + 30.0 * mb * S * S + pw_flops,
          (double)mb * per + (double)mb * (S / 4) * (S / 4) * C0 * 2,
          fv::launch_stem_fused_lb(static_cast<const char*>(L.img) + (size_t)b0 * per, L.dtype, mb, L.C, L.Hin, L.Win, L.pad, L.letterbox, tw.stem0_wp,
-                                  tw.stem0_b, tw.stem1_w, tw.stem1_b, oth, S, C0, s));
+                                  tw.stem0_b, tw.stem1_w, tw.stem1_b, w3, b3, stem_out, S, C0, s));
+    stem2_done = pw_in;
   } else if (fuse_stem && tw.stem0_wp && fv::stem_fused_supported(S, C0)) {
-    FV_P(FV_FAM_STEM, 2.0 * mb * (S / 2) * (S / 2) * 27 * C0 + dw_flops(mb, S / 4, S / 4, C0, 3),
+    FV_P(FV_FAM_STEM, 2.0 * mb * (S / 2) * (S / 2) * 27 * C0 + dw_flops(mb, S / 4, S / 4, C0, 3) + pw_flops,
          (double)mb * S * S * 8 + (double)mb * (S / 4) * (S / 4) * C0 * 2,
-         fv::launch_stem_fused(pix, tw.stem0_wp, tw.stem0_b, tw.stem1_w, tw.stem1_b, oth, mb, S, C0, s));
+         fv::launch_stem_fused(pix, tw.stem0_wp, tw.stem0_b, tw.stem1_w, tw.stem1_b, w3, b3, stem_out, mb, S, C0, s));
+    stem2_done = pw_in;
   } else {
     FV_P(FV_FAM_STEM, 2.0 * mb * (S / 2) * (S / 2) * 27 * C0, (double)mb * S * S * 8 + (double)mb * (S / 2) * (S / 2) * C0 * 2,
          tw.stem0_wp ? fv::launch_stem_mfma(pix, tw.stem0_wp, tw.stem0_b, cur, mb, S, C0, s)
@@ -548,7 +557,7 @@
          fv::launch_dwconv(cur, tw.stem1_w, tw.stem1_b, oth, mb, S / 2, S / 2, C0, 3, 2, 1, 1, s));
   }
   int H = S / 4;
-  {
+  if (!stem2_done) {
     fv::GemmArgs g{oth, C0, tw.stem2_w, mb * H * H, C0, C0, tw.stem2_b, nullptr, nullptr, 0, cur, C0, FV_EPI_BIAS_GELU};
     FV_TRY(gemm_p(h, g, s));
   }
diff --git a/vla-from-fastvlm_amd/csrc/kernels.h b/vla-from-fastvlm_amd/csrc/kernels.h
--- a/vla-from-fastvlm_amd/csrc/kernels.h
+++ b/vla-from-fastvlm_amd/csrc/kernels.h
@@ -54,10 +54,11 @@
 void stem_mfma_pack(const float* w27, float* out, int Cout);
 int launch_stem_mfma(const bf16_t* pix, const bf16_t* wp, const float* bias, bf16_t* y, int B, int S, int Cout, hipStream_t s);
 bool stem_fused_supported(int S, int C0);
-int launch_stem_fused(const bf16_t* pix, const bf16_t* wp, const float* b1, const float* w2, const float* b2, bf16_t* y, int B,
-                      int S, int C0, hipStream_t s);
+int launch_stem_fused(const bf16_t* pix, const bf16_t* wp, const float* b1, const float* w2, const float* b2, const bf16_t* w3,
+                      const float* b3, bf16_t* y, int B, int S, int C0, hipStream_t s);
 int launch_stem_fused_lb(const void* img, int dtype, int B, int C, int Hin, int Win, float pad_value, int letterbox, const bf16_t* wp,
-                         const float* b1, const float* w2, const float* b2, bf16_t* y, int S, int C0, hipStream_t s);
+                         const float* b1, const float* w2, const float* b2, const bf16_t* w3, const float* b3, bf16_t* y, int S, int C0,
+                         hipStream_t s);
 int launch_dwconv(const bf16_t* x, const float* w, const float* bias, bf16_t* y, int B, int H, int W, int C, int k,
                   int stride, int mult, int gelu, hipStream_t s);
 bool dwconv_mfma_supported(int W, int C, int k, int stride, int mult);
diff --git a/vla-from-fastvlm_amd/csrc/ops_api.hip b/vla-from-fastvlm_amd/csrc/ops_api.hip
--- a/vla-from-fastvlm_amd/csrc/ops_api.hip
+++ b/vla-from-fastvlm_amd/csrc/ops_api.hip
@@ -76,14 +76,25 @@
 }
 int fv_op_stem_fused(const void* pix, const void* wp, const float* b1, const float* w2, const float* b2, void* y, int B, int S, int Cout,
                      fv_stream s) {
-  return fv::launch_stem_fused(static_cast<const bf16_t*>(pix), static_cast<const bf16_t*>(wp), b1, w2, b2, static_cast<bf16_t*>(y), B, S, Cout,
-                               static_cast<hipStream_t>(s));
+  return fv::launch_stem_fused(static_cast<const bf16_t*>(pix), static_cast<const bf16_t*>(wp), b1, w2, b2, nullptr, nullptr, static_cast<bf16_t*>(y), B, S,
+                               Cout, static_cast<hipStream_t>(s));
+}
+int fv_op_stem_fused_pw(const void* pix, const void* wp, const float* b1, const float* w2, const float* b2, const void* w3, const float* b3, void* y,
+                        int B, int S, int Cout, fv_stream s) {
+  return fv::launch_stem_fused(static_cast<const bf16_t*>(pix), static_cast<const bf16_t*>(wp), b1, w2, b2, static_cast<const bf16_t*>(w3), b3,
+                               static_cast<bf16_t*>(y), B, S, Cout, static_cast<hipStream_t>(s));
 }
 
 int fv_op_stem_fused_images(const void* img, int dtype, int B, int C, int Hin, int Win, float pad_value, int resize_with_padding, const void* wp,
                             const float* b1, const float* w2, const float* b2, void* y, int S, int Cout, fv_stream s) {
+  return fv::launch_stem_fused_lb(img, dtype, B, C, Hin, Win, pad_value, resize_with_padding, static_cast<const bf16_t*>(wp), b1, w2, b2, nullptr,
+                                  nullptr, static_cast<bf16_t*>(y), S, Cout, static_cast<hipStream_t>(s));
+}
+int fv_op_stem_fused_images_pw(const void* img, int dtype, int B, int C, int Hin, int Win, float pad_value, int resize_with_padding, const void* wp,
+                               const float* b1, const float* w2, const float* b2, const void* w3, const float* b3, void* y, int S, int Cout,
+                               fv_stream s) {
   return fv::launch_stem_fused_lb(img, dtype, B, C, Hin, Win, pad_value, resize_with_padding, static_cast<const bf16_t*>(wp), b1, w2, b2,
-                                  static_cast<bf16_t*>(y), S, Cout, static_cast<hipStream_t>(s));
+                                  static_cast<const bf16_t*>(w3), b3, static_cast<bf16_t*>(y), S, Cout, static_cast<hipStream_t>(s));
 }
 
 int fv_op_layernorm_rows(const void* x, const float* w, const float* b, void* y, int rows, int C, float eps, fv_stream s) {
diff --git a/vla-from-fastvlm_amd/csrc/tower_kernels.hip b/vla-from-fastvlm_amd/csrc/tower_kernels.hip
--- a/vla-from-fastvlm_amd/csrc/tower_kernels.hip
+++ b/vla-from-fastvlm_amd/csrc/tower_kernels.hip
@@ -1,4 +1,6 @@
 #include "kernels.h"
+#include <algorithm>
+#include <cmath>
 #include <cstdlib>
 
 namespace fv {
@@ -383,60 +385,185 @@
 constexpr int SF_PATCH = SF_PR * SF_PCH * 16 + 16;
 constexpr int SF_LDS = SF_S1 + 10 * SF_C * 4 + SF_PATCH;
 constexpr int SF_PLD = (SF_PR * SF_PCH + 511) / 512;
-template <bool LB>
+constexpr int SF_MODE_PIX = 0, SF_MODE_LB_DIRECT = 1, SF_MODE_LB_WINDOW = 2;
+constexpr int SF_WIN = 4032;
+constexpr int SF_OFF_B3 = SF_LDS, SF_OFF_XT = SF_OFF_B3 + 2 * SF_C * 4;
+constexpr int SF_OFF_YT = SF_OFF_XT + 2 * SF_PCH * 8;
+constexpr int SF_OFF_WIN = SF_OFF_YT + (SF_PR + 1) * 8;
+constexpr int sf_lds_bytes(int mode, bool pw) { return mode == SF_MODE_LB_WINDOW ? SF_OFF_WIN + SF_WIN * 4 : pw ? SF_OFF_XT : SF_LDS; }
+static_assert(sf_lds_bytes(SF_MODE_LB_WINDOW, true) <= 160 * 1024, "stem_fused_kernel: LDS");
+struct SfWin { int rows, pitch; float inv_pitch; };
+
+__device__ __forceinline__ void sf_axis_window(int o0, int n, int S, int pad0, int rsz, int nin, float scale, int& first, int& count) {
+  const int da = max(max(o0, 0), pad0) - pad0, db = min(min(o0 + n - 1, S - 1), pad0 + rsz - 1) - pad0;
+  first = 0; count = 0;
+  if (da > db) return;
+  first = min((int)lb_src(da, scale), nin - 1);
+  count = min(min((int)lb_src(db, scale), nin - 1) + 1, nin - 1) - first + 1;
+}
+__device__ __forceinline__ int2 sf_axis_entry(int o, int pad0, int rsz, int nin, float scale, int first) {
+  const int d = o - pad0;
+  if (d < 0 || d >= rsz) return make_int2(-1, 0);
+  const float sp = lb_src(d, scale);
+  const int i0 = min((int)sp, nin - 1), i1 = min(i0 + 1, nin - 1);
+  return make_int2((i0 - first) | ((i1 - first) << 16), __float_as_int(lb_frac(sp, i0)));
+}
+
+template <int MODE, bool PW>
 __global__ __launch_bounds__(512, 1) void stem_fused_kernel(const bf16_t* __restrict__ pix, const bf16_t* __restrict__ wp,
                                                              const float* __restrict__ b1, const float* __restrict__ w2,
-                                                             const float* __restrict__ b2, bf16_t* __restrict__ y, int B, int S,
-                                                             long ntiles, LbParams lb) {
+                                                             const float* __restrict__ b2, const bf16_t* __restrict__ w3,
+                                                             const float* __restrict__ b3, bf16_t* __restrict__ y, int B, int S,
+                                                             long ntiles, LbParams lb, SfWin lw) {
+  constexpr bool LB = MODE != SF_MODE_PIX, WIN = MODE == SF_MODE_LB_WINDOW;
   extern __shared__ __attribute__((aligned(16))) char sf_smem[];
   char* s1 = sf_smem;
   float* sw2 = reinterpret_cast<float*>(sf_smem + SF_S1);
   char* spx = sf_smem + SF_S1 + 10 * SF_C * 4;
+  float* sb3 = reinterpret_cast<float*>(sf_smem + SF_OFF_B3);
+  int2* sxt = reinterpret_cast<int2*>(sf_smem + SF_OFF_XT);
+  int2* syt = reinterpret_cast<int2*>(sf_smem + SF_OFF_YT);
+  float* swin = reinterpret_cast<float*>(sf_smem + SF_OFF_WIN);
   const int tid = threadIdx.x, lane = tid & 63, wid = tid >> 6, fr = lane & 15, fg = lane >> 4;
   const int S1 = S >> 1, S2 = S >> 2;
   const int tiles_x = (S2 + SF_TC - 1) / SF_TC, tiles_y = (S2 + SF_TR - 1) / SF_TR;
   for (int i = tid; i < 10 * SF_C; i += 512) sw2[i] = i < 9 * SF_C ? w2[i] : b2[i - 9 * SF_C];
+  if constexpr (PW) { if (tid < 2 * SF_C) sb3[tid] = tid < SF_C ? b3[tid] : b1[tid - SF_C]; }
   bf16x8 wf[6][2];
 #pragma unroll
   for (int nt = 0; nt < 6; ++nt)
 #pragma unroll
     for (int ks = 0; ks < 2; ++ks)
       wf[nt][ks] = __builtin_bit_cast(bf16x8, *reinterpret_cast<const uint4*>(wp + ((size_t)(nt * 16 + fr) * 64 + ks * 32 + fg * 8)));
-  float4 bv1[6];
-#pragma unroll
-  for (int nt = 0; nt < 6; ++nt) bv1[nt] = *reinterpret_cast<const float4*>(b1 + nt * 16 + fg * 4);
-
-  uint4 pre[SF_PLD];
+  float4 bv1[PW ? 1 : 6];
+  if constexpr (!PW) {
+#pragma unroll
+    for (int nt = 0; nt < 6; ++nt) bv1[nt] = *reinterpret_cast<const float4*>(b1 + nt * 16 + fg * 4);
+  }
+
+  constexpr int SF_W3P = SF_C * 2 + 16, SF_W3CH = SF_C * (SF_C / 8);
+  static_assert(SF_C * SF_W3P <= SF_PATCH, "stem_fused_kernel: the 1x1 weight image lives in the patch area");
+  char* sw3 = spx;
+  uint4 w3r[PW ? (SF_W3CH + 511) / 512 : 1];
+  if constexpr (PW) {
+#pragma unroll
+    for (int j = 0; j < (SF_W3CH + 511) / 512; ++j) {
+      const int c = tid + 512 * j;
+      w3r[j] = c < SF_W3CH ? *reinterpret_cast<const uint4*>(w3 + (size_t)c * 8) : make_uint4(0, 0, 0, 0);
+    }
+  }
+  auto w3_store = [&]() {
+#pragma unroll
+    for (int j = 0; j < (SF_W3CH + 511) / 512; ++j) {
+      const int c = tid + 512 * j;
+      if (c < SF_W3CH) *reinterpret_cast<uint4*>(sw3 + (c / (SF_C / 8)) * SF_W3P + (c % (SF_C / 8)) * 16) = w3r[j];
+    }
+  };
+
+  uint4 pre[WIN ? 1 : SF_PLD];
+  constexpr int SF_WLD = (SF_WIN + 511) / 512;
+  float wpre[WIN ? SF_WLD : 1];
   auto patch_fetch = [&](unsigned tile) {
     const unsigned r_ = tile / (unsigned)tiles_x;
     const int tx = (int)(tile - r_ * (unsigned)tiles_x), ty = (int)(r_ % (unsigned)tiles_y);
     const long b = r_ / (unsigned)tiles_y;
     const int iy0 = 4 * ty * SF_TR - 3, ix0 = 4 * tx * SF_TC - 4;
-#pragma unroll
-    for (int j = 0; j < SF_PLD; ++j) {
-      const int c = tid + 512 * j, r = c / SF_PCH, cc = c % SF_PCH;
-      const int iy = iy0 + r, ix = ix0 + 2 * cc;
-      const bool in_ = c < SF_PR * SF_PCH && iy >= 0 && iy < S && ix >= 0 && ix < S;
-      if constexpr (LB) {
-        pre[j] = make_uint4(0, 0, 0, 0);
-        if (in_) {
-          const uint2 p0 = lb_pixel(lb, (int)b, iy, ix), p1 = lb_pixel(lb, (int)b, iy, ix + 1);
-          pre[j] = make_uint4(p0.x, p0.y, p1.x, p1.y);
+    if constexpr (WIN) {
+      int wx0, nx, wy0, ny;
+      sf_axis_window(ix0, 2 * SF_PCH, S, lb.pl, lb.rw, lb.Win, lb.sw, wx0, nx);
+      sf_axis_window(iy0, SF_PR, S, lb.pt, lb.rh, lb.Hin, lb.sh, wy0, ny);
+      const int nc = lb.C >= 3 ? 3 : 1;
+      int t_ = tid;
+      asm volatile("" : "+v"(t_));
+      const bool u8 = lb.dtype == FV_U8;
+      const size_t plane = (size_t)lb.Hin * lb.Win, img0 = (size_t)b * lb.C * plane + (size_t)wy0 * lb.Win + wx0;
+#pragma unroll
+      for (int j = 0; j < SF_WLD; ++j) {
+        const int i = t_ + 512 * j, row = (int)(((float)i + 0.5f) * lw.inv_pitch), x = i - row * lw.pitch;
+        const int c = (row >= lw.rows) + (row >= 2 * lw.rows), r = row - c * lw.rows;
+        const size_t at = img0 + c * plane + (size_t)(r * lb.Win + x);
+        const bool ok = c < nc && r < ny && x < nx;
+        if (u8) { const uint8_t v = ok ? static_cast<const uint8_t*>(lb.img)[at] : (uint8_t)0; wpre[j] = (float)v; }
+        else wpre[j] = ok ? static_cast<const float*>(lb.img)[at] : 0.f;
+      }
+    } else {
+#pragma unroll
+      for (int j = 0; j < SF_PLD; ++j) {
+        const int c = tid + 512 * j, r = c / SF_PCH, cc = c % SF_PCH;
+        const int iy = iy0 + r, ix = ix0 + 2 * cc;
+        const bool in_ = c < SF_PR * SF_PCH && iy >= 0 && iy < S && ix >= 0 && ix < S;
+        if constexpr (LB) {
+          pre[j] = make_uint4(0, 0, 0, 0);
+          if (in_) {
+            const uint2 p0 = lb_pixel(lb, (int)b, iy, ix), p1 = lb_pixel(lb, (int)b, iy, ix + 1);
+            pre[j] = make_uint4(p0.x, p0.y, p1.x, p1.y);
+          }
+        } else {
+          pre[j] = in_ ? *reinterpret_cast<const uint4*>(pix + (((size_t)b * S + iy) * S + ix) * 4) : make_uint4(0, 0, 0, 0);
         }
-      } else {
-        pre[j] = in_ ? *reinterpret_cast<const uint4*>(pix + (((size_t)b * S + iy) * S + ix) * 4) : make_uint4(0, 0, 0, 0);
       }
     }
   };
-  auto patch_store = [&]() {
-#pragma unroll
-    for (int j = 0; j < SF_PLD; ++j) {
-      const int c = tid + 512 * j;
-      if (c < SF_PR * SF_PCH) *reinterpret_cast<uint4*>(spx + c * 16) = pre[j];
+  auto patch_store = [&](unsigned tile) {
+    if constexpr (WIN) {
+      const unsigned r_ = tile / (unsigned)tiles_x;
+      const int tx = (int)(tile - r_ * (unsigned)tiles_x), ty = (int)(r_ % (unsigned)tiles_y);
+      const int iy0 = 4 * ty * SF_TR - 3, ix0 = 4 * tx * SF_TC - 4;
+      int wx0, nx, wy0, ny;
+      sf_axis_window(ix0, 2 * SF_PCH, S, lb.pl, lb.rw, lb.Win, lb.sw, wx0, nx);
+      sf_axis_window(iy0, SF_PR, S, lb.pt, lb.rh, lb.Hin, lb.sh, wy0, ny);
+#pragma unroll
+      for (int j = 0; j < SF_WLD; ++j)
+        if (tid + 512 * j < SF_WIN) swin[tid + 512 * j] = wpre[j];
+      if (tid < 2 * SF_PCH) sxt[tid] = sf_axis_entry(ix0 + tid, lb.pl, lb.rw, lb.Win, lb.sw, wx0);
+      if (tid >= 192 && tid < 192 + SF_PR) syt[tid - 192] = sf_axis_entry(iy0 + tid - 192, lb.pt, lb.rh, lb.Hin, lb.sh, wy0);
+      __syncthreads();
+      const int nc = lb.C >= 3 ? 3 : 1;
+      int t_ = tid;
+      asm volatile("" : "+v"(t_));
+#pragma unroll
+      for (int j = 0; j < SF_PLD; ++j) {
+        const int c = t_ + 512 * j, r = c / SF_PCH, cc = c % SF_PCH;
+        const int iy = iy0 + r, ix = ix0 + 2 * cc;
+        if (c >= SF_PR * SF_PCH) continue;
+        uint4 o = make_uint4(0, 0, 0, 0);
+        if (iy >= 0 && iy < S && ix >= 0 && ix < S) {
+          const int2 ye = syt[r];
+          const float wy = __int_as_float(ye.y);
+          const int r0 = (ye.x & 0xffff) * lw.pitch, r1 = (int)((unsigned)ye.x >> 16) * lw.pitch;
+          unsigned w[4];
+#pragma unroll
+          for (int q = 0; q < 2; ++q) {
+            const int2 xe = sxt[2 * cc + q];
+            float v[3] = {lb.pad, lb.pad, lb.pad};
+            if (ye.x != -1 && xe.x != -1) {
+              const float wx = __int_as_float(xe.y);
+              const int x0 = xe.x & 0xffff, x1 = (int)((unsigned)xe.x >> 16);
+              for (int ch = 0; ch < nc; ++ch) {
+                const float* pl = swin + ch * lw.rows * lw.pitch;
+                const float t0 = lb_lerp(pl[r0 + x0], pl[r0 + x1], wx);
+                const float t1 = lb_lerp(pl[r1 + x0], pl[r1 + x1], wx);
+                v[ch] = lb_lerp(t0, t1, wy);
+              }
+              if (nc == 1) v[1] = v[2] = v[0];
+            }
+            w[2 * q] = pack_bf2(v[0], v[1]);
+            w[2 * q + 1] = pack_bf2(v[2], 0.0f);
+          }
+          o = make_uint4(w[0], w[1], w[2], w[3]);
+        }
+        *reinterpret_cast<uint4*>(spx + c * 16) = o;
+      }
+    } else {
+#pragma unroll
+      for (int j = 0; j < SF_PLD; ++j) {
+        const int c = tid + 512 * j;
+        if (c < SF_PR * SF_PCH) *reinterpret_cast<uint4*>(spx + c * 16) = pre[j];
+      }
     }
   };
   if (tid == 0) *reinterpret_cast<uint4*>(spx + SF_PR * SF_PCH * 16) = make_uint4(0, 0, 0, 0);
-  if ((long)blockIdx.x < ntiles) { patch_fetch(blockIdx.x); patch_store(); }
+  if ((long)blockIdx.x < ntiles) { patch_fetch(blockIdx.x); patch_store(blockIdx.x); }
 
   for (unsigned tile = blockIdx.x; tile < (unsigned)ntiles; tile += gridDim.x) {
     const unsigned r_ = tile / (unsigned)tiles_x;
@@ -475,8 +602,15 @@
 #pragma unroll
       for (int np = 0; np < 3; ++np) {
         const int n0 = 2 * np, n1 = 2 * np + 1;
-        f32x2 g[4] = {{acc[n0][0] + bv1[n0].x, acc[n0][1] + bv1[n0].y}, {acc[n0][2] + bv1[n0].z, acc[n0][3] + bv1[n0].w},
-                      {acc[n1][0] + bv1[n1].x, acc[n1][1] + bv1[n1].y}, {acc[n1][2] + bv1[n1].z, acc[n1][3] + bv1[n1].w}};
+        float4 c0, c1;
+        if constexpr (PW) {
+          c0 = *reinterpret_cast<const float4*>(sb3 + SF_C + n0 * 16 + fg * 4);
+          c1 = *reinterpret_cast<const float4*>(sb3 + SF_C + n1 * 16 + fg * 4);
+        } else {
+          c0 = bv1[n0]; c1 = bv1[n1];
+        }
+        f32x2 g[4] = {{acc[n0][0] + c0.x, acc[n0][1] + c0.y}, {acc[n0][2] + c0.z, acc[n0][3] + c0.w},
+                      {acc[n1][0] + c1.x, acc[n1][1] + c1.y}, {acc[n1][2] + c1.z, acc[n1][3] + c1.w}};
         gelu2_n<4>(g);
         uint2 o0, o1;
         o0.x = live ? pack_bf2(g[0].x, g[0].y) : 0u;
@@ -494,10 +628,11 @@
     __syncthreads();
     const unsigned tile_n = tile + gridDim.x;
     if (tile_n < (unsigned)ntiles) patch_fetch(tile_n);
-#pragma unroll 1
-    for (int it = 0; it < SF_TR * SF_TC * (SF_C / 8) / 512; ++it) {
-      const int item = tid + 512 * it;
-      const int cg = item % (SF_C / 8), p = item / (SF_C / 8), pr = p / SF_TC, pc = p % SF_TC;
+    if constexpr (PW) {
+      w3_store();
+      __syncthreads();
+    }
+    auto dw_item = [&](int pr, int pc, int cg) -> uint4 {
       float acc[8];
       {
         const float4 a0 = *reinterpret_cast<const float4*>(sw2 + 9 * SF_C + cg * 8), a1 = *reinterpret_cast<const float4*>(sw2 + 9 * SF_C + cg * 8 + 4);
@@ -516,14 +651,56 @@
         }
       f32x2 g[4] = {{acc[0], acc[1]}, {acc[2], acc[3]}, {acc[4], acc[5]}, {acc[6], acc[7]}};
       gelu2_n<4>(g);
+      uint4 o;
+      o.x = pack_bf2(g[0].x, g[0].y); o.y = pack_bf2(g[1].x, g[1].y); o.z = pack_bf2(g[2].x, g[2].y); o.w = pack_bf2(g[3].x, g[3].y);
+      return o;
+    };
+    if constexpr (PW) {
+      const int p = wid * 16 + fr, pr = p / SF_TC, pc = p % SF_TC;
+      const char* w3l = sw3 + fr * SF_W3P + fg * 16;
+      f32x4 a[6];
+#pragma unroll
+      for (int j = 0; j < 6; ++j) a[j] = f32x4{0.f, 0.f, 0.f, 0.f};
+#pragma unroll 1
+      for (int ks = 0; ks < 3; ++ks) {
+        uint4 wq[6];
+#pragma unroll
+        for (int j = 0; j < 6; ++j) wq[j] = *reinterpret_cast<const uint4*>(w3l + j * 16 * SF_W3P + ks * 64);
+        const bf16x8 xb = __builtin_bit_cast(bf16x8, dw_item(pr, pc, 4 * ks + fg));
+#pragma unroll
+        for (int j = 0; j < 6; ++j) a[j] = __builtin_amdgcn_mfma_f32_16x16x32_bf16(__builtin_bit_cast(bf16x8, wq[j]), xb, a[j], 0, 0, 0);
+      }
       const int oy = ty * SF_TR + pr, ox = tx * SF_TC + pc;
-      if (oy < S2 && ox < S2) {
-        uint4 o;
-        o.x = pack_bf2(g[0].x, g[0].y); o.y = pack_bf2(g[1].x, g[1].y); o.z = pack_bf2(g[2].x, g[2].y); o.w = pack_bf2(g[3].x, g[3].y);
-        *reinterpret_cast<uint4*>(y + (((size_t)b * S2 + oy) * S2 + ox) * SF_C + cg * 8) = o;
-      }
-    }
-    if (tile_n < (unsigned)ntiles) patch_store();
+      bf16_t* yp = y + (((size_t)b * S2 + oy) * S2 + ox) * SF_C;
+#pragma unroll
+      for (int jp = 0; jp < 3; ++jp) {
+        const f32x4 a0 = a[2 * jp], a1 = a[2 * jp + 1];
+        const float4 c0 = *reinterpret_cast<const float4*>(sb3 + 2 * jp * 16 + fg * 4), c1 = *reinterpret_cast<const float4*>(sb3 + (2 * jp + 1) * 16 + fg * 4);
+        f32x2 g[4] = {{a0[0] + c0.x, a0[1] + c0.y}, {a0[2] + c0.z, a0[3] + c0.w}, {a1[0] + c1.x, a1[1] + c1.y}, {a1[2] + c1.z, a1[3] + c1.w}};
+        gelu2_n<4>(g);
+        uint2 o0, o1;
+        o0.x = pack_bf2(g[0].x, g[0].y); o0.y = pack_bf2(g[1].x, g[1].y);
+        o1.x = pack_bf2(g[2].x, g[2].y); o1.y = pack_bf2(g[3].x, g[3].y);
+        if (oy < S2 && ox < S2) {
+          *reinterpret_cast<uint2*>(yp + 2 * jp * 16 + 4 * fg) = o0;
+          *reinterpret_cast<uint2*>(yp + (2 * jp + 1) * 16 + 4 * fg) = o1;
+        }
+      }
+    } else {
+#pragma unroll 1
+      for (int it = 0; it < SF_TR * SF_TC * (SF_C / 8) / 512; ++it) {
+        const int item = tid + 512 * it;
+        const int cg = item % (SF_C / 8), p = item / (SF_C / 8), pr = p / SF_TC, pc = p % SF_TC;
+        const uint4 o = dw_item(pr, pc, cg);
+        const int oy = ty * SF_TR + pr, ox = tx * SF_TC + pc;
+        if (oy < S2 && ox < S2) *reinterpret_cast<uint4*>(y + (((size_t)b * S2 + oy) * S2 + ox) * SF_C + cg * 8) = o;
+      }
+    }
+    if constexpr (PW) {
+      if (tid == 0) *reinterpret_cast<uint4*>(spx + SF_PR * SF_PCH * 16) = make_uint4(0, 0, 0, 0);
+      if (!WIN) __syncthreads();
+    }
+    if (tile_n < (unsigned)ntiles) patch_store(tile_n);
   }
 }
 
@@ -1684,13 +1861,14 @@
 }
 
 bool stem_fused_supported(int S, int C0) { return C0 == SF_C && S >= 8 && S % 4 == 0; }
-int launch_stem_fused(const bf16_t* pix, const bf16_t* wp, const float* b1, const float* w2, const float* b2, bf16_t* y, int B,
-                      int S, int C0, hipStream_t s) {
-  if (!pix || !wp || !b1 || !w2 || !b2 || !y) return fv_fail(FV_ERR_ARG, "stem_fused: null pointer");
-  if (B <= 0 || !stem_fused_supported(S, C0)) return fv_fail(FV_ERR_UNSUPPORTED, "stem_fused: bad shape S=%d C0=%d", S, C0);
+namespace {
+template <int MODE, bool PW>
+int stem_fused_launch(const bf16_t* pix, const bf16_t* wp, const float* b1, const float* w2, const float* b2, const bf16_t* w3, const float* b3,
+                      bf16_t* y, int B, int S, const LbParams& lb, SfWin lw, hipStream_t s) {
+  constexpr int lds = sf_lds_bytes(MODE, PW);
   static bool attr_set = false;
   if (!attr_set) {
-    FV_HIP_CHECK(hipFuncSetAttribute(reinterpret_cast<const void*>(&stem_fused_kernel<false>), hipFuncAttributeMaxDynamicSharedMemorySize, SF_LDS));
+    FV_HIP_CHECK(hipFuncSetAttribute(reinterpret_cast<const void*>(&stem_fused_kernel<MODE, PW>), hipFuncAttributeMaxDynamicSharedMemorySize, lds));
     attr_set = true;
   }
   const int S2 = S / 4;
@@ -1700,32 +1878,44 @@
   hipDeviceProp_t prop;
   if (hipGetDevice(&dev) == hipSuccess && hipGetDeviceProperties(&prop, dev) == hipSuccess && prop.multiProcessorCount > 0) cus = prop.multiProcessorCount;
   const long blocks = ntiles < cus ? ntiles : cus;
-  hipLaunchKernelGGL(stem_fused_kernel<false>, dim3((unsigned)blocks), dim3(512), SF_LDS, s, pix, wp, b1, w2, b2, y, B, S, ntiles, LbParams{});
+  hipLaunchKernelGGL((stem_fused_kernel<MODE, PW>), dim3((unsigned)blocks), dim3(512), lds, s, pix, wp, b1, w2, b2, w3, b3, y, B, S, ntiles, lb, lw);
   FV_HIP_CHECK(hipGetLastError());
   return FV_OK;
 }
 
+bool sf_window(const LbParams& p, SfWin& lw) {
+  const long wc = std::min((long)p.Win, (long)std::ceil((2 * SF_PCH - 1) * (double)p.sw) + 3), wr = std::min((long)p.Hin, (long)std::ceil((SF_PR - 1) * (double)p.sh) + 3);
+  if ((p.C >= 3 ? 3 : 1) * wr * wc > SF_WIN) return false;
+  lw.rows = (int)wr; lw.pitch = (int)wc; lw.inv_pitch = 1.0f / (float)wc;
+  return true;
+}
+}
+
+int launch_stem_fused(const bf16_t* pix, const bf16_t* wp, const float* b1, const float* w2, const float* b2, const bf16_t* w3,
+                      const float* b3, bf16_t* y, int B, int S, int C0, hipStream_t s) {
+  if (!pix || !wp || !b1 || !w2 || !b2 || !y) return fv_fail(FV_ERR_ARG, "stem_fused: null pointer");
+  if ((w3 == nullptr) != (b3 == nullptr)) return fv_fail(FV_ERR_ARG, "stem_fused: the 1x1 needs weight and bias");
+  if (B <= 0 || !stem_fused_supported(S, C0)) return fv_fail(FV_ERR_UNSUPPORTED, "stem_fused: bad shape S=%d C0=%d", S, C0);
+  return w3 ? stem_fused_launch<SF_MODE_PIX, true>(pix, wp, b1, w2, b2, w3, b3, y, B, S, LbParams{}, SfWin{}, s)
+            : stem_fused_launch<SF_MODE_PIX, false>(pix, wp, b1, w2, b2, w3, b3, y, B, S, LbParams{}, SfWin{}, s);
+}
+
 int launch_stem_fused_lb(const void* img, int dtype, int B, int C, int Hin, int Win, float pad_value, int letterbox, const bf16_t* wp,
-                         const float* b1, const float* w2, const float* b2, bf16_t* y, int S, int C0, hipStream_t s) {
+                         const float* b1, const float* w2, const float* b2, const bf16_t* w3, const float* b3, bf16_t* y, int S, int C0,
+                         hipStream_t s) {
   if (!img || !wp || !b1 || !w2 || !b2 || !y) return fv_fail(FV_ERR_ARG, "stem_fused_lb: null pointer");
+  if ((w3 == nullptr) != (b3 == nullptr)) return fv_fail(FV_ERR_ARG, "stem_fused_lb: the 1x1 needs weight and bias");
   if (B <= 0 || !stem_fused_supported(S, C0)) return fv_fail(FV_ERR_UNSUPPORTED, "stem_fused_lb: bad shape S=%d C0=%d", S, C0);
   LbParams p;
   FV_TRY_RC(lb_params(img, dtype, B, C, Hin, Win, S, pad_value, letterbox, nullptr, p));
-  static bool attr_set = false;
-  if (!attr_set) {
-    FV_HIP_CHECK(hipFuncSetAttribute(reinterpret_cast<const void*>(&stem_fused_kernel<true>), hipFuncAttributeMaxDynamicSharedMemorySize, SF_LDS));
-    attr_set = true;
-  }
-  const int S2 = S / 4;
-  const long ntiles = (long)B * ((S2 + SF_TC - 1) / SF_TC) * ((S2 + SF_TR - 1) / SF_TR);
-  if (ntiles > 0x3fffffffL) return fv_fail(FV_ERR_ARG, "stem_fused_lb: too many tiles");
-  int dev = 0, cus = 256;
-  hipDeviceProp_t prop;
-  if (hipGetDevice(&dev) == hipSuccess && hipGetDeviceProperties(&prop, dev) == hipSuccess && prop.multiProcessorCount > 0) cus = prop.multiProcessorCount;
-  const long blocks = ntiles < cus ? ntiles : cus;
-  hipLaunchKernelGGL(stem_fused_kernel<true>, dim3((unsigned)blocks), dim3(512), SF_LDS, s, nullptr, wp, b1, w2, b2, y, B, S, ntiles, p);
-  FV_HIP_CHECK(hipGetLastError());
-  return FV_OK;
+  SfWin lw{};
+  static const bool no_window = fv_ab_env("FASTVLA_STEM_LB_DIRECT") != nullptr;
+  const bool window = sf_window(p, lw) && !no_window;
+  if (window)
+    return w3 ? stem_fused_launch<SF_MODE_LB_WINDOW, true>(nullptr, wp, b1, w2, b2, w3, b3, y, B, S, p, lw, s)
+              : stem_fused_launch<SF_MODE_LB_WINDOW, false>(nullptr, wp, b1, w2, b2, w3, b3, y, B, S, p, lw, s);
+  return w3 ? stem_fused_launch<SF_MODE_LB_DIRECT, true>(nullptr, wp, b1, w2, b2, w3, b3, y, B, S, p, lw, s)
+            : stem_fused_launch<SF_MODE_LB_DIRECT, false>(nullptr, wp, b1, w2, b2, w3, b3, y, B, S, p, lw, s);
 }
 
 bool dwconv_pair_supported(int B, int H, int W, int C) {
diff --git a/vla-from-fastvlm_amd/fastvla_hip/_lib.py b/vla-from-fastvlm_amd/fastvla_hip/_lib.py
--- a/vla-from-fastvlm_amd/fastvla_hip/_lib.py
+++ b/vla-from-fastvlm_amd/fastvla_hip/_lib.py
@@ -146,6 +146,8 @@
     "fv_op_stem_mfma": (_i, [_vp, _vp, _vp, _vp, _i, _i, _i, _vp]),
     "fv_op_stem_fused": (_i, [_vp, _vp, _vp, _vp, _vp, _vp, _i, _i, _i, _vp]),
     "fv_op_stem_fused_images": (_i, [_vp, _i, _i, _i, _i, _i, _f, _i, _vp, _vp, _vp, _vp, _vp, _i, _i, _vp]),
+    "fv_op_stem_fused_pw": (_i, [_vp, _vp, _vp, _vp, _vp, _vp, _vp, _vp, _i, _i, _i, _vp]),
+    "fv_op_stem_fused_images_pw": (_i, [_vp, _i, _i, _i, _i, _i, _f, _i, _vp, _vp, _vp, _vp, _vp, _vp, _vp, _i, _i, _vp]),
     "fv_op_layernorm_rows": (_i, [_vp, _vp, _vp, _vp, _i, _i, _f, _vp]),
     "fv_op_attention": (_i, [_vp, _vp, _vp, _i, _i, _i, _vp, _i, _i, _i, _i, _i, _i, _i, _vp, _f, _vp]),
     "fv_op_rmsnorm": (_i, [_vp, _vp, _vp, _i, _i, _f, _vp]),
```

New measurement: 18.99 steps/s (median of 4 runs). No clear change (-0.0%).
